# jakepoz/rnnt

Hardware: AMD Instinct MI355X
Metric: RNN-T joint+loss fwd+bwd lattice cells/s (B*T*U/s) (higher is better)
Workload: dtype f32(f16x2); 1 GPU; cfg2: B=32,T=1000,U=200,H=512,V=1024 fp32-class (f16x2 arithmetic) joint+loss fwd+bwd; enc_layout=contiguous (B,T,H), global_batch=32, per_gpu_batch=32, parallelism=dp1, cells_BTU1=6432000

## Files before the change

rnnt_amd/csrc/engine.hip:

```cpp
#include "../../include/rnnt_engine.h"

#include <cfloat>
#include <cmath>
#include <cstdarg>
#include <cstddef>
#include <cstdio>
#include <dlfcn.h>
#include <string>

#include "kernels.hpp"

namespace {

thread_local std::string g_err;
#if defined(RNNT_ABLATE) || defined(RNNT_STAMPS)
int g_flags = 0;
unsigned long long *g_debug = nullptr;
#else
constexpr int g_flags = 0;
constexpr unsigned long long *g_debug = nullptr;
#endif

}

// ... 55 lines not shown
    return RNNT_OK;
}

int check_reg(float fastemit_lambda, float delay_penalty)
{
    if (!(fastemit_lambda >= 0.f && fastemit_lambda <= FLT_MAX))
        return fail(RNNT_ERR_INVALID_ARG, "fastemit_lambda=%g must be finite and >= 0", (double)fastemit_lambda);
    if (!(delay_penalty >= 0.f && delay_penalty <= FLT_MAX))
        return fail(RNNT_ERR_INVALID_ARG, "delay_penalty=%g must be finite and >= 0", (double)delay_penalty);
    return RNNT_OK;
}

int check_restrict(const int32_t *restrict_frames, int restrict_left, int restrict_right)
{
    if (!restrict_frames) return fail(RNNT_ERR_INVALID_ARG, "null pointer argument (restrict_frames)");
    if (restrict_left < 0 || restrict_right < 0)
        return fail(RNNT_ERR_INVALID_ARG, "restrict_left=%d and restrict_right=%d must be >= 0", restrict_left, restrict_right);
    return RNNT_OK;
}

int dw_splits(int B, int T, int H, int V, int dtype)
{
    const long tiles = dtype == RNNT_DTYPE_F32 ? dw_tiles(H, V) : dtype == RNNT_DTYPE_F32_F16X2 ? x2_dw_tiles(H, V) : (long)((V + 255) / 256) * ((H + 255) / 256);
    long s = 256 / tiles;
    if (s < 1) s = 1;
    if (s > (long)B * T) s = (long)B * T;
    return (int)s;
}

long bf16_rows_alloc(size_t rows_pad) { return (long)((rows_pad + 96 + 127) / 128 * 128); }

void layout(int B, int T, int U1, int H, int V, int dtype, rnnt_engine_ws_layout *L)
{
    const size_t D = (size_t)T + U1 - 1;
    const size_t cells = (size_t)B * T * U1;
    const bool bf = dtype == RNNT_DTYPE_BF16, x2 = dtype == RNNT_DTYPE_F32_F16X2, x3 = dtype == RNNT_DTYPE_F32_BF16X3 || x2;
    const size_t rows_pad = (bf || x3) ? (cells + 1 + 31) / 32 * 32 : (cells + 1 + 15) / 16 * 16;
    L->rows_pad = rows_pad;
    L->D = (int)D;
    L->n_ublk = bf ? (U1 + 15) / 16 : x3 ? (U1 + 7) / 8 : (U1 + dhidden_gen_bu(T, U1) - 1) / dhidden_gen_bu(T, U1);
    L->n_ttile = (T + 3) / 4;
    L->n_split = dw_splits(B, T, H, V, dtype);
    L->g_lo = 0; L->aux = 0; L->aux_bytes = 0; L->x2_live = 0;
    size_t o = 0;
    if (bf) {
        const size_t ra = (size_t)bf16_rows_alloc(rows_pad);
        L->logits = o;   o += align_up(ra * V * 2);
        L->hidden = o;   o += align_up(ra * H * 2);
    } else if (x3) {
        const size_t ra = (size_t)bf16_rows_alloc(rows_pad);
        L->logits = o;   o += align_up(ra * V * 4);
        L->hidden = o;   o += align_up((x2 ? 2 : 3) * ra * H * 2);
        if (!x2) { L->g_lo = o; o += align_up(ra * V * 2); }
    } else {
        L->logits = o;   o += align_up((rows_pad + 16) * V * 4);
        L->hidden = o;   o += align_up((rows_pad + 16) * H * 4);
    }
    const LossWs w = carve_loss_ws((void *)o, B, T, U1);
    L->denom_s = (size_t)w.denom_s; L->lpb_s = (size_t)w.lpb_s; L->lpe_s = (size_t)w.lpe_s;
    L->alpha_s = (size_t)w.alpha_s; L->beta_s = (size_t)w.beta_s; L->coef = (size_t)w.coef; o = (size_t)w.err;
    L->wpack = o;
    if (bf) o += align_up(bf16_wpack_fwd_bytes(H, V)) + align_up(bf16_wpack_dh_bytes(H, V));
    else if (x2) o += align_up(x2_wpack_fwd_bytes(H, V)) + align_up(x2_wpack_dh_bytes(H, V));
    else if (x3) o += align_up(x3_wpack_fwd_bytes(H, V)) + align_up(x3_wpack_dh_bytes(H, V));
    else o += align_up(wpack_floats(H, V) * 4);
    L->enc_copy = o; o += align_up((size_t)B * T * H * 4);
    L->ep = 0;
    if (x2) { L->ep = o; o += align_up(x2_ep_bytes(B, T, U1, H)); }
    L->slab_enc = o; o += align_up((size_t)L->n_ublk * B * T * H * 4);
    L->slab_pred = o; o += align_up((size_t)L->n_ttile * B * U1 * H * 4);
    L->slab_w = o;   o += align_up((size_t)L->n_split * V * H * 4);
    L->slab_b = o;   o += align_up((size_t)L->n_split * V * 4);
    const size_t tab = ControlBlock::dw_table_bytes(B), lst = (bf || x3) ? 0 : align_up(dw_list_bytes(B, T, U1, 16));
    L->counters = o; o += sizeof(ControlBlock) + (tab > lst ? tab : lst) + ((bf || x2) ? align_up((size_t)L->n_split * 64) : 0);
    if (x2) { L->x2_live = o; o += align_up(x2_live_bytes(B, T, U1, (long)rows_pad)); }
    L->total = o;
    if (x3) {
        L->aux = o; L->aux_bytes = align_up((rows_pad + 16) * H * 4) + align_up(wpack_floats(H, V) * 4);
    }
}

}

typedef unsigned u32x4 __attribute__((ext_vector_type(4)));

__global__ __launch_bounds__(256) void k_fill32(unsigned *__restrict__ p, unsigned value, size_t n_words, int vec)
{
    const size_t i = (size_t)blockIdx.x * 256 + threadIdx.x;
    if (vec) {
        if (i < n_words / 4) ((u32x4 *)p)[i] = u32x4{value, value, value, value};
    } else if (i < n_words) {
        p[i] = value;
    }
}

__global__ __launch_bounds__(256) void k_copy32(unsigned *__restrict__ d, const unsigned *__restrict__ s, size_t n_words, int vec)
{
    const size_t i = (size_t)blockIdx.x * 256 + threadIdx.x;
    if (vec) {
        if (i < n_words / 4) ((u32x4 *)d)[i] = ((const u32x4 *)s)[i];
    } else if (i < n_words) {
        d[i] = s[i];
    }
}

void launch_fill32(void *p, unsigned value, size_t bytes, hipStream_t st)
{
    const size_t n = bytes / 4;
    if (!n) return;
    const int vec = ((uintptr_t)p % 16 == 0) && (n % 4 == 0);
    const size_t thr = vec ? n / 4 : n;
    hipLaunchKernelGGL(k_fill32, dim3((unsigned)((thr + 255) / 256)), dim3(256), 0, st, (unsigned *)p, value, n, vec);
}

void launch_copy_bytes(void *dst, const void *src, size_t bytes, hipStream_t st)
{
    const size_t n = bytes / 4;
    if (!n) return;
    const int vec = ((uintptr_t)dst % 16 == 0) && ((uintptr_t)src % 16 == 0) && (n % 4 == 0);
    const size_t thr = vec ? n / 4 : n;
    hipLaunchKernelGGL(k_copy32, dim3((unsigned)((thr + 255) / 256)), dim3(256), 0, st, (unsigned *)dst, (const unsigned *)src, n, vec);
}

namespace {

int launch_status(const char *what)
{
    hipError_t e = hipGetLastError();
    if (e != hipSuccess) return fail(RNNT_ERR_LAUNCH, "%s: %s", what, hipGetErrorString(e));
    return RNNT_OK;
}

void resolve_enc(const void *enc, const int64_t s[3], int B, int T, int H, float *copy_buf,
                 hipStream_t st, const float **out, long *sb, long *st_)
{
    const bool direct = s[2] == 1 && (s[1] % 4) == 0 && (s[0] % 4) == 0 && aligned16(enc);
    if (direct) {
        *out = (const float *)enc; *sb = s[0]; *st_ = s[1];
    } else {
        launch_copy_enc((const float *)enc, s[0], s[1], s[2], copy_buf, B, T, H, st);
        *out = copy_buf; *sb = (long)T * H; *st_ = H;
    }
}

enum { ST_PROD = 1, ST_FWD = 2, ST_LATTICE = 4, ST_COEF = 8, ST_DH = 16, ST_DH_RED = 32, ST_DW = 64,
       ST_DW_RED = 128, ST_ALL = 255 };
enum { ABLATE_NO_HIDDEN = 8, ABLATE_SEPARATE_G = 32, ABLATE_SEPARATE_HIDDEN = 64, ABLATE_FWD_LDS_RING = 128, ABLATE_FWD_ONE_WG = 256 };

struct LossCall {
    LossWs w;
    const int32_t *targets, *logit_lens, *target_lens; float *costs;
    int B, T, U1, stages ; float grad_scale, fastemit, delay; hipStream_t st;
    const int32_t *restrict_frames; int restrict_left, restrict_right;
};

struct FusedCall : LossCall {
    int H, V, blank, n_cu;
    const float *enc, *pred, *W, *bias; long enc_sb, enc_st;
    float *grad_enc, *grad_pred, *grad_W, *grad_bias;
    rnnt_engine_ws_layout L;
    char *ws; ControlBlock *cb; float *logits;
    bool separate_g, separate_hidden, fwd_lds_ring, fwd_one_wg_per_tile, no_hidden;
    bool x3_fp32_fwd, x3_fp32_dh;
    bool x2_no_flush;
    int ablate; unsigned long long *debug;
};
float *f32_at(const FusedCall &c, size_t offset) { return (float *)(c.ws + offset); }

JointFwdArgs fwd_args(const FusedCall &c, const float *wpack, const float *hidden, int make_hidden)
{
    JointFwdArgs f{};
    f.enc = c.enc; f.enc_sb = c.enc_sb; f.enc_st = c.enc_st; f.pred = c.pred; f.logit_lens = c.logit_lens; f.target_lens = c.target_lens;
    f.B = c.B; f.T = c.T; f.U1 = c.U1; f.H = c.H; f.V = c.V; f.blank = c.blank; f.ablate = c.ablate; f.debug = c.debug;
    f.wpack = wpack; f.hidden = hidden; f.make_hidden = make_hidden; f.bias = c.bias; f.targets = c.targets; f.logits = c.logits;
    f.denom_s = c.w.denom_s; f.lpb_s = c.w.lpb_s; f.lpe_s = c.w.lpe_s; f.D = c.L.D; f.counter = c.cb ? c.cb->fwd_tile : nullptr; f.n_cu = c.n_cu;
    return f;
}

JointBwdArgs bwd_args(const FusedCall &c)
{
    JointBwdArgs g{};
    g.enc = c.enc; g.enc_sb = c.enc_sb; g.enc_st = c.enc_st; g.pred = c.pred; g.logit_lens = c.logit_lens; g.target_lens = c.target_lens;
    g.B = c.B; g.T = c.T; g.U1 = c.U1; g.H = c.H; g.V = c.V; g.blank = c.blank; g.ablate = c.ablate; g.debug = c.debug;
    g.W = c.W; g.logits = c.logits; g.coef = c.w.coef; g.hidden = f32_at(c, c.L.hidden); g.rows_pad = (long)c.L.rows_pad;
    g.slab_enc = f32_at(c, c.L.slab_enc); g.slab_pred = f32_at(c, c.L.slab_pred);
    g.slab_w = f32_at(c, c.L.slab_w); g.slab_b = f32_at(c, c.L.slab_b);
    g.grad_enc = c.grad_enc; g.grad_pred = c.grad_pred; g.grad_W = c.grad_W; g.grad_bias = c.grad_bias;
    g.n_ublk = c.L.n_ublk; g.n_ttile = c.L.n_ttile; g.n_split = c.L.n_split;
    g.counter = c.cb->queue; g.dw_tab = c.cb->dw_tab(); g.n_cu = c.n_cu;
    g.gen_bu = dhidden_gen_bu(c.T, c.U1);
    return g;
}

template <class Args> Args split_args(const FusedCall &c, size_t wpack_fwd_bytes)
{
    Args h{};
    h.enc = c.enc; h.enc_sb = c.enc_sb; h.enc_st = c.enc_st; h.pred = c.pred; h.logit_lens = c.logit_lens; h.target_lens = c.target_lens;
    h.B = c.B; h.T = c.T; h.U1 = c.U1; h.H = c.H; h.V = c.V; h.blank = c.blank; h.ablate = c.ablate; h.debug = c.debug;
    h.W = c.W; h.bias = c.bias; h.targets = c.targets; h.coef = c.w.coef; h.hidden = (unsigned short *)(c.ws + c.L.hidden);
    h.denom_s = c.w.denom_s; h.lpb_s = c.w.lpb_s; h.lpe_s = c.w.lpe_s; h.D = c.L.D;
    h.slab_enc = f32_at(c, c.L.slab_enc); h.slab_pred = f32_at(c, c.L.slab_pred);
    h.slab_w = f32_at(c, c.L.slab_w); h.slab_b = f32_at(c, c.L.slab_b);
    h.rows_pad = (long)c.L.rows_pad; h.rows_alloc = bf16_rows_alloc(c.L.rows_pad);
    h.n_ublk = c.L.n_ublk; h.n_split = c.L.n_split; h.dw_tab = c.cb->dw_tab();
    h.wpack_fwd = c.ws + c.L.wpack; h.wpack_dh = c.ws + c.L.wpack + align_up(wpack_fwd_bytes);
    return h;
}

Bf16Args bf16_args(const FusedCall &c)
{
    Bf16Args h = split_args<Bf16Args>(c, bf16_wpack_fwd_bytes(c.H, c.V));
    h.logits = (unsigned short *)c.logits; h.dw_prog = c.cb->dw_prog(c.B);
    return h;
}

struct OperandScales { float g_scale, dw_rescale, db_rescale; double flush_log2; float flush_lin; };
OperandScales operand_scales(float grad_scale, float fastemit)
{
    OperandScales s; int e = 0;
    (void)frexpf(grad_scale * (1.0f + fastemit), &e);
    const int k = 13 - e < -100 ? -100 : (13 - e > 100 ? 100 : 13 - e);
    s.g_scale = ldexpf(1.0f, k); s.flush_log2 = (double)(-26 - k); s.flush_lin = ldexpf(1.0f, -26 - k);
    s.dw_rescale = 1.0f / (s.g_scale * 16384.0f); s.db_rescale = 1.0f / s.g_scale;
    return s;
}

X3Args x3_args(const FusedCall &c, size_t wpack_fwd_bytes, const OperandScales &s)
{
    X3Args h = split_args<X3Args>(c, wpack_fwd_bytes);
    h.g_scale = s.g_scale; h.dw_rescale = s.dw_rescale; h.db_rescale = s.db_rescale; h.scales = c.cb->x2_scales;
    h.ep_enc = f32_at(c, c.L.ep); h.ep_pred = h.ep_enc + (size_t)c.B * c.T * c.H; h.ep_flag = c.cb->ep_flag;
    h.logits = c.logits; h.g_lo = (unsigned short *)(c.ws + c.L.g_lo); h.n_ublk16 = (c.U1 + 15) / 16;
    h.plane_stride = h.rows_alloc * (long)c.H; h.counter = c.cb->fwd_tile; h.n_cu = c.n_cu;
    return h;
}

void loss_stages(const LossCall &c, const double *flush_log2 = nullptr, float flush_lin = 0.f)
{
    const LossWs &w = c.w; const int D = c.T + c.U1 - 1;
    if (c.restrict_frames) {
        if (c.stages & ST_LATTICE) {
            launch_restrict(w.lpe_s, c.restrict_frames, c.logit_lens, c.target_lens, c.B, c.T, c.U1, D, c.restrict_left, c.restrict_right,
                            c.delay, c.st);
            launch_lattice(w.lpb_s, w.lpe_s, w.alpha_s, w.beta_s, c.logit_lens, c.target_lens, c.costs, c.B, c.U1, D, w.err, c.st, true);
            if (c.delay > 0.f) launch_delay_cost(w.beta_s, c.logit_lens, c.target_lens, c.costs, c.B, c.T, c.U1, D, c.delay, c.st);
        }
        if (c.stages & ST_COEF)
            launch_coef_restrict(w.alpha_s, w.beta_s, w.denom_s, w.lpb_s, w.lpe_s, c.targets, c.logit_lens, c.target_lens, w.coef,
                                 c.B, c.T, c.U1, D, c.grad_scale, c.fastemit, flush_log2, flush_lin, c.st);
        return;
    }
    if (c.stages & ST_LATTICE) {
        if (c.delay > 0.f) launch_delay_penalty(w.lpe_s, c.logit_lens, c.target_lens, c.B, c.T, c.U1, D, c.delay, c.st);
        launch_lattice(w.lpb_s, w.lpe_s, w.alpha_s, w.beta_s, c.logit_lens, c.target_lens, c.costs, c.B, c.U1, D, w.err, c.st);
        if (c.delay > 0.f) launch_delay_cost(w.beta_s, c.logit_lens, c.target_lens, c.costs, c.B, c.T, c.U1, D, c.delay, c.st);
    }
    if (c.stages & ST_COEF) {
        if (c.fastemit > 0.f)
            launch_coef_fastemit(w.alpha_s, w.beta_s, w.denom_s, w.lpb_s, w.lpe_s, c.targets, c.logit_lens, c.target_lens, w.coef,
                                 c.B, c.T, c.U1, D, c.grad_scale, c.fastemit, c.st);
        else if (flush_log2)
            launch_coef_flush(w.alpha_s, w.beta_s, w.denom_s, w.lpb_s, w.lpe_s, c.targets, c.logit_lens, c.target_lens, w.coef,
                              c.B, c.T, c.U1, D, c.grad_scale, *flush_log2, flush_lin, c.st);
        else
            launch_coef(w.alpha_s, w.beta_s, w.denom_s, w.lpb_s, w.lpe_s, c.targets, c.logit_lens, c.target_lens, w.coef,
                        c.B, c.T, c.U1, D, c.grad_scale, c.st);
    }
}

void zero_unwritten_hidden(const FusedCall &c, float *hidden)
{
    const size_t cells = (size_t)c.B * c.T * c.U1;
    launch_fill32(hidden + cells * c.H, 0u, (c.L.rows_pad + 16 - cells) * c.H * 4, c.st);
    launch_zero_dead_hidden(hidden, c.logit_lens, c.target_lens, c.B, c.T, c.U1, c.H, c.st);
}

int tile_kernel_cols(const FusedCall &c) { return dhidden_gen_ok(c.H, c.V, c.U1) ? 512 * dhidden_gen_groups(c.H) : 0; }

float *aux_hidden(const FusedCall &c) { return f32_at(c, c.L.aux); }
typedef void (*x3_launcher)(const X3Args &, hipStream_t);

void standin_forward(const FusedCall &c, const X3Args &h, x3_launcher make_hidden)
{
    float *wpack = (float *)(c.ws + c.L.aux + align_up((c.L.rows_pad + 16) * (size_t)c.H * 4));
    if (c.stages & ST_PROD) { zero_unwritten_hidden(c, aux_hidden(c)); launch_pack_w_fwd(c.W, wpack, c.H, c.V, c.st); }
    if (c.stages & ST_FWD) {
        JointFwdArgs f = fwd_args(c, wpack, aux_hidden(c), 1);
        f.ablate = 0; f.debug = nullptr;
        launch_joint_fwd(f, c.st); make_hidden(h, c.st);
    }
}

void standin_dhidden(const FusedCall &c, const JointBwdArgs &g, const X3Args &h, x3_launcher split_g)
{
    const bool tile = g.pred_split_col > 0;
    if (!tile) launch_make_g(g, c.st);
    launch_dhidden(g, tile, c.st);
    split_g(h, c.st);
}

int route_fp32(const FusedCall &c)
{
    JointBwdArgs g = bwd_args(c);
    const bool tile = (g.pred_split_col = tile_kernel_cols(c)) > 0, fuse_g = tile && !c.separate_g;
    g.g_ready = tile && !fuse_g;
    const bool fuse_hid = !c.separate_hidden && !c.no_hidden;
    float *wpack = (float *)(c.ws + c.L.wpack);
    if (c.stages & ST_PROD) {
        if (fuse_hid) zero_unwritten_hidden(c, g.hidden);
        else launch_make_hidden(g, c.st);
        launch_pack_w_fwd(c.W, wpack, c.H, c.V, c.st);
    }
    if (c.stages & ST_FWD)
        launch_joint_fwd(fwd_args(c, wpack, c.no_hidden ? nullptr : g.hidden, fuse_hid ? 1 : 0), c.st, c.fwd_lds_ring, c.fwd_one_wg_per_tile);
    loss_stages(c);
    if ((c.stages & ST_COEF) && !fuse_g) launch_make_g(g, c.st);
    if (c.stages & ST_DH) launch_dhidden(g, tile, c.st);
    if (c.stages & ST_DH_RED) launch_dhidden_reduce(g, c.st);
    if (c.stages & ST_DW) launch_dw(g, c.st);
    if (c.stages & ST_DW_RED) launch_dw_reduce(g, c.st);
    return launch_status("rnnt_engine fused pipeline");
}

int route_bf16(const FusedCall &c)
{
    const Bf16Args h = bf16_args(c);
    JointBwdArgs g = bwd_args(c); g.gen_bu = 16; g.pred_split_col = c.H;
    if (c.stages & ST_PROD) launch_bf16_producers(h, c.st);
    if (c.stages & ST_FWD) launch_joint_fwd_bf16(h, c.st);
    loss_stages(c);
    if (c.stages & ST_DH) launch_dhidden_bf16(h, c.st);
    if (c.stages & ST_DH_RED) launch_dhidden_reduce(g, c.st);
    if (c.stages & ST_DW) launch_dw_bf16(h, c.st);
    if (c.stages & ST_DW_RED) launch_dw_reduce(g, c.st);
    return launch_status("rnnt_engine fused pipeline (bf16)");
}

int route_bf16x3(const FusedCall &c)
{
    const X3Args h = x3_args(c, x3_wpack_fwd_bytes(c.H, c.V), operand_scales(c.grad_scale, c.fastemit));
    JointBwdArgs g = bwd_args(c); g.hidden = aux_hidden(c);
    if (c.x3_fp32_dh) g.pred_split_col = tile_kernel_cols(c);
    else { g.gen_bu = 16; g.pred_split_col = c.H; }
    if (c.stages & ST_PROD) { launch_x3_zero_padding(h, 1, c.st); launch_x3_pack_w(h, c.st); }
    if (c.x3_fp32_fwd) standin_forward(c, h, launch_x3_make_hidden);
    else if (c.stages & ST_FWD) launch_joint_fwd_x3(h, c.st);
    loss_stages(c);
    if (c.stages & ST_DH) {
        launch_x3_zero_padding(h, 2, c.st);
        if (c.x3_fp32_dh) standin_dhidden(c, g, h, launch_x3_split_g);
        else launch_dhidden_x3(h, c.st);
    }
    if (c.stages & ST_DH_RED) launch_dhidden_reduce(g, c.st);
    if (c.stages & ST_DW) launch_dw_x3(h, c.st);
    if (c.stages & ST_DW_RED) launch_dw_reduce(g, c.st);
    return launch_status("rnnt_engine fused pipeline (bf16x3)");
}

int route_f16x2(const FusedCall &c)
{
    OperandScales s = operand_scales(c.grad_scale, c.fastemit);
    X3Args h = x3_args(c, x2_wpack_fwd_bytes(c.H, c.V), s);
    h.dw_prog = c.cb->dw_prog(c.B); h.dw_ksteps = x2_dw_walks_ksteps(c.H, c.V) ? 1 : 0;
    x2_live_carve(c.ws + c.L.x2_live, c.B, c.T, c.U1, (long)c.L.rows_pad, h);
    JointBwdArgs g = bwd_args(c); g.hidden = aux_hidden(c);
    if (c.x3_fp32_dh) g.pred_split_col = tile_kernel_cols(c);
    else { g.gen_bu = 16; g.pred_split_col = c.H; }
    if (!c.x3_fp32_dh) { g.tile_flag = h.tile_live; g.flag_ntt = (c.T + 7) / 8; g.flag_nub = h.n_ublk16; }
    if (c.x2_no_flush || c.x3_fp32_dh) { s.flush_log2 = -HUGE_VAL; s.flush_lin = 0.f; }
    if (c.stages & ST_PROD) { launch_x2_zero_padding(h, 1, c.st); launch_x2_pack_w(h, c.cb->x2_scales, c.st); launch_x2_make_ep(h, c.st); }
    if (c.x3_fp32_fwd) standin_forward(c, h, launch_x2_make_hidden);
    else if (c.stages & ST_FWD) launch_joint_fwd_x2(h, c.st);
    loss_stages(c, &s.flush_log2, s.flush_lin);
    if (c.stages & ST_COEF) launch_x2_live(h, c.st);
    if (c.stages & ST_DH) {
        launch_x2_zero_padding(h, 2, c.st);
        if (c.x3_fp32_dh) standin_dhidden(c, g, h, launch_x2_split_g);
        else { launch_x2_dead_rows(h, c.st); launch_dhidden_x2(h, c.st); }
    }
    if (c.stages & ST_DH_RED) launch_dhidden_reduce(g, c.st);
    if (c.stages & ST_DW) launch_dw_x2(h, c.st);
    if (c.stages & ST_DW_RED) launch_dw_reduce_x2(h, c.grad_W, c.grad_bias, c.st);
    return launch_status("rnnt_engine fused pipeline (f16x2)");
}

int run_fused(int stages, int variant, const void *enc, const int64_t enc_strides[3], const void *pred,
              const void *W, const void *bias, const int32_t *targets, const int32_t *logit_lens,
              const int32_t *target_lens, int B, int T, int U1, int H, int V, int blank,
              float clamp, float grad_scale, float fastemit, float delay, int dtype, float *costs,
              void *grad_enc, void *grad_pred, void *grad_W, void *grad_bias, void *workspace,
              size_t ws_bytes, void *stream, const int32_t *restrict_frames = nullptr, int restrict_left = 0,
              int restrict_right = 0)
{
    if (int rc = check_dims(B, T, U1, H, V, dtype, true)) return rc;
    if (!enc || !enc_strides || !pred || !W || !bias || !targets || !logit_lens || !target_lens ||
        !costs || !workspace)
        return fail(RNNT_ERR_INVALID_ARG, "null pointer argument");
    const bool backward = (stages & (ST_DH | ST_DH_RED | ST_DW | ST_DW_RED)) != 0;
    if (backward && (!grad_enc || !grad_pred || !grad_W || !grad_bias))
        return fail(RNNT_ERR_INVALID_ARG, "null gradient pointer");
    if (blank < 0 || blank >= V) return fail(RNNT_ERR_INVALID_ARG, "blank=%d outside [0,%d)", blank, V);
    if (clamp > 0.f) return fail(RNNT_ERR_UNSUPPORTED, "clamp>0 is only supported by rnnt_engine_loss_fwd_bwd");
    if (!(grad_scale > 0.f)) return fail(RNNT_ERR_INVALID_ARG, "grad_scale must be > 0");
    if (!aligned16(pred) || !aligned16(W) || !aligned16(bias) || !aligned16(grad_enc) ||
        !aligned16(grad_pred) || !aligned16(grad_W) || !aligned16(grad_bias) ||
        ((uintptr_t)workspace & 255))
        return fail(RNNT_ERR_INVALID_ARG, "pointers must be 16-byte aligned (workspace 256)");
    if (variant & RNNT_VARIANT_LAB_MASK)
        return fail(RNNT_ERR_UNSUPPORTED, "variant bits 0x%x are reserved: no kernel of librnnt_engine.so answers to them",
                    variant & RNNT_VARIANT_LAB_MASK);
    FusedCall c{};
    layout(B, T, U1, H, V, dtype, &c.L);
    if (ws_bytes < c.L.total)
        return fail(RNNT_ERR_WORKSPACE, "workspace %zu < required %zu bytes", ws_bytes, c.L.total);
    c.ablate = g_flags; c.debug = g_debug;
    const int xp = dtype == RNNT_DTYPE_F32 ? c.ablate : 0;
    c.separate_g = (variant & RNNT_VARIANT_SEPARATE_G) != 0 || (xp & ABLATE_SEPARATE_G) != 0;
    c.separate_hidden = (variant & RNNT_VARIANT_SEPARATE_HIDDEN) != 0 || (xp & ABLATE_SEPARATE_HIDDEN) != 0;
    c.fwd_lds_ring = (variant & RNNT_VARIANT_FWD_LDS_RING) != 0 || (xp & ABLATE_FWD_LDS_RING) != 0;
    c.fwd_one_wg_per_tile = (variant & RNNT_VARIANT_FWD_ONE_WG_PER_TILE) != 0 || (xp & ABLATE_FWD_ONE_WG) != 0;
    c.no_hidden = (xp & ABLATE_NO_HIDDEN) != 0;
    c.x2_no_flush = (variant & RNNT_VARIANT_X2_NO_FLUSH_SKIP) != 0 || fastemit > 0.f || delay > 0.f;
    if (dtype == RNNT_DTYPE_F32_BF16X3 || dtype == RNNT_DTYPE_F32_F16X2) {
        const bool x2 = dtype == RNNT_DTYPE_F32_F16X2;
        c.x3_fp32_dh = (variant & RNNT_VARIANT_X3_FP32_DH) != 0 || !(x2 ? x2_dhidden_ok(U1, H, V) : x3_dhidden_ok(U1, H, V));
        c.x3_fp32_fwd = (variant & RNNT_VARIANT_X3_FP32_FWD) != 0 || !(x2 ? x2_fwd_ok(U1, H, V) : x3_fwd_ok(U1, H, V)) || c.x3_fp32_dh;
        if (c.x3_fp32_fwd && ws_bytes < c.L.total + c.L.aux_bytes)
            return fail(RNNT_ERR_WORKSPACE, "workspace %zu < %zu bytes: a stage on the fp32 route's kernels (RNNT_VARIANT_X3_FP32_*, or a "
                        "shape k_joint_fwd_x3 / k_dhidden_x3 do not cover) needs total + aux_bytes of rnnt_engine_workspace_layout",
                        ws_bytes, c.L.total + c.L.aux_bytes);
    }
    c.B = B; c.T = T; c.U1 = U1; c.H = H; c.V = V; c.blank = blank; c.pred = (const float *)pred; c.W = (const float *)W;
    c.bias = (const float *)bias; c.targets = targets; c.logit_lens = logit_lens; c.target_lens = target_lens; c.costs = costs;
    c.grad_enc = (float *)grad_enc; c.grad_pred = (float *)grad_pred; c.grad_W = (float *)grad_W; c.grad_bias = (float *)grad_bias;
    c.stages = stages; c.grad_scale = grad_scale; c.fastemit = fastemit; c.delay = delay; c.n_cu = device_cus(); c.st = (hipStream_t)stream;
    c.restrict_frames = restrict_frames; c.restrict_left = restrict_left; c.restrict_right = restrict_right;
    c.ws = (char *)workspace; c.cb = (ControlBlock *)(c.ws + c.L.counters); c.logits = f32_at(c, c.L.logits);
    c.w = carve_loss_ws(c.ws + c.L.denom_s, B, T, U1); c.w.err = c.cb->lattice_err;
    resolve_enc(enc, enc_strides, B, T, H, f32_at(c, c.L.enc_copy), c.st, &c.enc, &c.enc_sb, &c.enc_st);
    if (dtype == RNNT_DTYPE_BF16) return route_bf16(c);
    if (dtype == RNNT_DTYPE_F32_BF16X3) return route_bf16x3(c);
    return dtype == RNNT_DTYPE_F32_F16X2 ? route_f16x2(c) : route_fp32(c);
}

}

extern "C" {

int rnnt_engine_version(void) { return RNNT_ENGINE_VERSION; }

#if defined(RNNT_ABLATE) || defined(RNNT_STAMPS)
int rnnt_engine_set_flags(int flags) { int o = g_flags; g_flags = flags; return o; }
void rnnt_engine_set_debug(void *buf) { g_debug = (unsigned long long *)buf; }
#else
int rnnt_engine_set_flags(int) { return 0; }
void rnnt_engine_set_debug(void *) {}
#endif

int rnnt_engine_debug_query(int what) { return fwd_occupancy(what); }

const char *rnnt_engine_last_error(void) { return g_err.c_str(); }

int rnnt_engine_allreduce(void *buf, size_t count, void *comm, void *stream)
{
    if (!buf || !comm) return fail(RNNT_ERR_INVALID_ARG, "null buffer / communicator");
    if (count == 0) return RNNT_OK;
    typedef int (*allreduce_fn)(const void *, void *, size_t, int, int, void *, hipStream_t);
    typedef const char *(*errstr_fn)(int);
    void *sym = dlsym(RTLD_DEFAULT, "ncclAllReduce");
    void *lib = nullptr;
    if (!sym) {
        lib = dlopen("librccl.so.1", RTLD_NOW | RTLD_NOLOAD);
        if (!lib) lib = dlopen("librccl.so.1", RTLD_NOW);
        if (!lib) lib = dlopen("librccl.so", RTLD_NOW);
        if (lib) sym = dlsym(lib, "ncclAllReduce");
    }
    if (!sym) return fail(RNNT_ERR_UNSUPPORTED, "RCCL (librccl.so.1: ncclAllReduce) not found in this process");
    const int ncclFloat32_ = 7, ncclSum_ = 0;
    const int rc = ((allreduce_fn)sym)(buf, buf, count, ncclFloat32_, ncclSum_, comm, (hipStream_t)stream);
    if (rc != 0) {
        void *es = lib ? dlsym(lib, "ncclGetErrorString") : dlsym(RTLD_DEFAULT, "ncclGetErrorString");
        return fail(RNNT_ERR_LAUNCH, "ncclAllReduce failed (%d): %s", rc, es ? ((errstr_fn)es)(rc) : "?");
    }
    return RNNT_OK;
}

int rnnt_engine_workspace_layout(int B, int T, int U1, int H, int V, int dtype,
                                 rnnt_engine_ws_layout *out)
{
    if (!out) return fail(RNNT_ERR_INVALID_ARG, "null layout pointer");
    if (int rc = check_dims(B, T, U1, H, V, dtype, true)) return rc;
    layout(B, T, U1, H, V, dtype, out);
    return RNNT_OK;
}

int rnnt_engine_workspace_bytes(int B, int T, int U1, int H, int V, int dtype, size_t *out)
{
    if (!out) return fail(RNNT_ERR_INVALID_ARG, "null size pointer");
    rnnt_engine_ws_layout L;
    if (int rc = rnnt_engine_workspace_layout(B, T, U1, H, V, dtype, &L)) return rc;
    *out = L.total;
    return RNNT_OK;
}

int rnnt_engine_loss_workspace_bytes(int B, int T, int U1, int V, int dtype, size_t *out)
{
    if (!out) return fail(RNNT_ERR_INVALID_ARG, "null size pointer");
    if (int rc = check_dims(B, T, U1, 4, V, dtype, false)) return rc;
    *out = carve_loss_ws(nullptr, B, T, U1).bytes;
    return RNNT_OK;
}

int rnnt_engine_joint_fwd_workspace_bytes(int B, int T, int U1, int H, int V, int dtype,
                                          size_t *out)
{
    if (!out) return fail(RNNT_ERR_INVALID_ARG, "null size pointer");
    if (int rc = check_dims(B, T, U1, H, V, dtype, true)) return rc;
    *out = align_up(wpack_floats(H, V) * 4) + align_up((size_t)B * T * H * 4);
    return RNNT_OK;
}

int rnnt_engine_joint_fwd(const void *enc, const int64_t enc_strides[3], const void *pred,
                          const void *W, const void *bias, int B, int T, int U1, int H, int V,
                          int dtype, void *logits, void *workspace, size_t ws_bytes, void *stream)
{
    if (int rc = check_dims(B, T, U1, H, V, dtype, true)) return rc;
    if (!enc || !enc_strides || !pred || !W || !bias || !logits || !workspace)
        return fail(RNNT_ERR_INVALID_ARG, "null pointer argument");
    if (!aligned16(pred) || !aligned16(W) || !aligned16(bias) || !aligned16(logits) ||
        ((uintptr_t)workspace & 255))
        return fail(RNNT_ERR_INVALID_ARG, "pointers must be 16-byte aligned (workspace 256)");
    size_t need;
    rnnt_engine_joint_fwd_workspace_bytes(B, T, U1, H, V, dtype, &need);
    if (ws_bytes < need) return fail(RNNT_ERR_WORKSPACE, "workspace %zu < required %zu bytes", ws_bytes, need);
// ... 752 lines not shown
```

rnnt_amd/csrc/joint_bwd.hip:

```cpp
#include "common.hpp"
#include "kernels.hpp"

typedef __attribute__((address_space(3))) void *lds_void_ptr;

#define DH_BT 8
#define DW_KC 16
#define DW_ZERO_SPAN 32
#define DH_BU 16

#define PW_BT 4
struct PwChunk {
    f32x4 x[2];
    f32x4 w[4];
};

template <int BU>
__global__ __launch_bounds__(512, 2) void k_dhidden(JointBwdArgs a, int cb0)
{
    constexpr int IT = 64 / BU;
    const int lane = threadIdx.x & 63;
    const int i = lane & 31, half = lane >> 5;
    const int T = a.T, U1 = a.U1, H = a.H, V = a.V;
    const int n_cb = (H + 127) / 128 - cb0, n_ub = (U1 + BU - 1) / BU, n_tt = (T + IT - 1) / IT;
    const long zero_row = (long)a.B * T * U1;
// ... 377 lines not shown
                }
            }
#pragma unroll
            for (int m = 8; m < 16; ++m) mf(2, m);
#pragma unroll
            for (int m = 0; m < 16; ++m) mf(3, m);
            PIN();
            if (!(j & 1)) {
                asm volatile("s_waitcnt lgkmcnt(0)" ::: "memory");
                __builtin_amdgcn_s_barrier();
            }
            PIN();
            a0 = an0;
            a1 = an1;
        }
    }
#undef PIN
    GSTAMP(2);

    if (RNNT_XP(a.ablate, 8192)) return;
    constexpr int TPM = 32 / BU;
    constexpr int NU = BU / 2;
    constexpr int TB = BU == 16 ? 1 : 2;
    float psum[NU][8];
#pragma unroll
    for (int k = 0; k < NU; ++k)
#pragma unroll
        for (int q = 0; q < 8; ++q) psum[k][q] = 0.f;
    const long BTH = (long)a.B * T * H, BUH = (long)a.B * U1 * H;
    const long rows_utt = (long)(T - t0) * U1 - u0;
    const long hspan = span_rows < rows_utt ? span_rows : rows_utt;
    const __amdgpu_buffer_rsrc_t hrsrc = __builtin_amdgcn_make_buffer_rsrc(
        (void *)(a.hidden + cell0 * H), 0, (int)(hspan * H * 4), 0x00020000);
    const unsigned hvoff[2] = {colok[0] ? (unsigned)(((4 * half) * H + colg[0]) * 4) : 0xfffffff0u,
                               colok[1] ? (unsigned)(((4 * half) * H + colg[1]) * 4) : 0xfffffff0u};
    auto t_of = [&](int mt, int rh, int r7) { return (2 * wm + mt) * TPM + (BU == 16 ? rh : 2 * rh + (r7 >> 2)); };
    auto us_of = [&](int r7) { return BU == 16 ? 8 * (r7 >> 2) + (r7 & 3) : (r7 & 3); };
    auto hload = [&](int k, f32x4 (&hb)[16]) {
        const int mt = k >> 1, rh = k & 1;
#pragma unroll
        for (int r7 = 0; r7 < 8; ++r7) {
            const unsigned soff = (unsigned)((t_of(mt, rh, r7) * U1 + us_of(r7)) * H) * 4u;
#pragma unroll
            for (int g = 0; g < 2; ++g)
                hb[r7 * 2 + g] = __builtin_bit_cast(f32x4, __builtin_amdgcn_raw_buffer_load_b128(hrsrc, hvoff[g], soff, 0));
        }
    };
    auto hcomp = [&](int k, const f32x4 (&hb)[16]) {
        const int mt = k >> 1, rh = k & 1;
        float esum[TB][8];
#pragma unroll
        for (int e = 0; e < TB; ++e)
#pragma unroll
            for (int q = 0; q < 8; ++q) esum[e][q] = 0.f;
#pragma unroll
        for (int r7 = 0; r7 < 8; ++r7)
#pragma unroll
            for (int g = 0; g < 2; ++g) {
                const f32x4 h4 = hb[r7 * 2 + g];
#pragma unroll
                for (int q = 0; q < 4; ++q) {
                    const float d = acc[mt][g * 4 + q][rh * 8 + r7] * (1.f - h4[q] * h4[q]);
                    esum[BU == 16 ? 0 : (r7 >> 2)][g * 4 + q] += d;
                    psum[BU == 16 ? r7 : (r7 & 3)][g * 4 + q] += d;
                }
            }
#pragma unroll
        for (int e = 0; e < TB; ++e) {
#pragma unroll
            for (int q = 0; q < 8; ++q) esum[e][q] += __shfl_xor(esum[e][q], 32, 64);
            const int t = t0 + t_of(mt, rh, 4 * e);
            if (half == 0 && t < Tb) {
#pragma unroll
                for (int g = 0; g < 2; ++g)
                    if (colok[g]) {
                        f32x4 o = {esum[e][g * 4], esum[e][g * 4 + 1], esum[e][g * 4 + 2], esum[e][g * 4 + 3]};
                        *(f32x4 *)(a.slab_enc + (long)ub * BTH + ((long)b * T + t) * H + colg[g]) = o;
                    }
            }
        }
    };
    {
        f32x4 hA[16], hB[16];
        hload(0, hA);
        hload(1, hB);
        __builtin_amdgcn_sched_barrier(0);
        hcomp(0, hA);
        __builtin_amdgcn_sched_barrier(0);
        hload(2, hA);
        __builtin_amdgcn_sched_barrier(0);
        hcomp(1, hB);
        __builtin_amdgcn_sched_barrier(0);
        hload(3, hB);
        __builtin_amdgcn_sched_barrier(0);
        hcomp(2, hA);
        hcomp(3, hB);
    }
    if (wm == 1) {
#pragma unroll
        for (int k = 0; k < NU; ++k)
#pragma unroll
            for (int q = 0; q < 8; ++q) s_red[wn][lane][k * 8 + q] = psum[k][q];
    }
    __syncthreads();
    if (wm == 0) {
#pragma unroll
        for (int k = 0; k < NU; ++k) {
            const int u = u0 + (BU == 16 ? 8 * (k >> 2) + (k & 3) : k) + 4 * half;
            if (u < U1) {
#pragma unroll
                for (int g = 0; g < 2; ++g)
                    if (colok[g]) {
                        f32x4 o;
#pragma unroll
                        for (int q = 0; q < 4; ++q)
                            o[q] = psum[k][g * 4 + q] + s_red[wn][lane][k * 8 + g * 4 + q];
                        *(f32x4 *)(a.slab_pred + (long)tt * BUH + ((long)b * U1 + u) * H + colg[g]) = o;
                    }
            }
        }
    }
    GSTAMP(3);
}

int dhidden_gen_bu(int T, int U1)
{
    const long c16 = (long)((U1 + 15) / 16 * 16) * ((T + 7) / 8 * 8);
    const long c8 = (long)((U1 + 7) / 8 * 8) * ((T + 15) / 16 * 16);
    return c8 < c16 ? 8 : 16;
}
bool dhidden_gen_ok(int H, int V, int U1)
{
    const long span_rows = (long)(16 - 1) * U1 + 16;
    const long wide = V > H ? V : H;
    return (V % 32) == 0 && (long)V * H * 4 < 0xffffffffL && span_rows * wide * 4 < 0x7fffffffL;
}
#define DG_COLS 512
int dhidden_gen_groups(int H) { return H <= DG_COLS ? 1 : H / DG_COLS; }

__device__ __forceinline__ void reduce_flagged(f32x4 &s, const f32x4 *__restrict__ p, long stride, int k0, unsigned m)
{
    const f32x4 z = {0.f, 0.f, 0.f, 0.f};
    while (m) {
        f32x4 v[8];
#pragma unroll
        for (int j = 0; j < 8; ++j) {
            v[j] = z;
            if (m) { v[j] = p[(long)(k0 + __builtin_ctz(m)) * stride]; m &= m - 1; }
        }
#pragma unroll
        for (int j = 0; j < 8; ++j) s += v[j];
    }
}
__global__ __launch_bounds__(256) void k_reduce_enc(const float *__restrict__ slab,
                                                    const int32_t *__restrict__ logit_lens,
                                                    const int32_t *__restrict__ target_lens,
                                                    float *__restrict__ out, int B, int T, int U1,
                                                    int H, int n_ublk, int bu_lo, int col_split,
                                                    const unsigned char *__restrict__ flag, int ntt, int nub_f)
{
    const long idx = (long)blockIdx.x * blockDim.x + threadIdx.x;
    const int H4 = H / 4;
    const long n = (long)B * T * H4;
    if (idx >= n) return;
    const long bt = idx / H4;
    const int t = (int)(bt % T), b = (int)(bt / T);
    f32x4 s = {0.f, 0.f, 0.f, 0.f};
    if (t < len_t(logit_lens, b, T)) {
        const int bu = bu_lo;
        int nub = len_u(target_lens, b, U1) / bu + 1;
        if (nub > n_ublk) nub = n_ublk;
        if (flag) {
            const unsigned char *f = flag + ((long)b * ntt + t / 8) * nub_f;
            for (int k0 = 0; k0 < nub; k0 += 32) {
                const int kn = nub - k0 < 32 ? nub - k0 : 32;
                unsigned m = 0;
                for (int k = 0; k < kn; ++k) m |= (f[k0 + k] ? 1u : 0u) << k;
                reduce_flagged(s, (const f32x4 *)slab + idx, n, k0, m);
            }
        } else {
            for (int k = 0; k < nub; ++k) s += ((const f32x4 *)slab)[(long)k * n + idx];
        }
    }
    ((f32x4 *)out)[idx] = s;
}

__global__ __launch_bounds__(256) void k_reduce_pred(const float *__restrict__ slab,
                                                     const int32_t *__restrict__ logit_lens,
                                                     const int32_t *__restrict__ target_lens,
                                                     float *__restrict__ out, int B, int T, int U1,
                                                     int H, int bt_lo, int bt_hi, int col_split,
                                                     const unsigned char *__restrict__ flag, int ntt_f, int nub_f)
{
    const long idx = (long)blockIdx.x * blockDim.x + threadIdx.x;
    const int H4 = H / 4;
    const long n = (long)B * U1 * H4;
    if (idx >= n) return;
    const int b = (int)(idx / ((long)U1 * H4));
    const int bt = 4 * (int)(idx % H4) < col_split ? bt_lo : bt_hi;
    const int ntt = (len_t(logit_lens, b, T) + bt - 1) / bt;
    const int u = (int)((idx / H4) % U1);
    f32x4 s = {0.f, 0.f, 0.f, 0.f};
    if (u <= len_u(target_lens, b, U1)) {
        if (flag) {
            const unsigned char *f = flag + (long)b * ntt_f * nub_f + u / 16;
            for (int k0 = 0; k0 < ntt; k0 += 32) {
                const int kn = ntt - k0 < 32 ? ntt - k0 : 32;
                unsigned m = 0;
                for (int k = 0; k < kn; ++k) m |= (f[(long)(k0 + k) * nub_f] ? 1u : 0u) << k;
                reduce_flagged(s, (const f32x4 *)slab + idx, n, k0, m);
            }
        } else {
            for (int k = 0; k < ntt; ++k) s += ((const f32x4 *)slab)[(long)k * n + idx];
        }
    }
    ((f32x4 *)out)[idx] = s;
}

void launch_dhidden(const JointBwdArgs &a, bool tile_kernel, hipStream_t st)
{
    int cb0 = 0;
    if (tile_kernel) {
        const long cells = (long)a.B * a.T * a.U1;
        launch_fill32((float *)a.logits + cells * a.V, 0u, (size_t)(a.rows_pad + 16 - cells) * a.V * 4, st);
        const int n_full = dhidden_gen_groups(a.H);
        if (a.gen_bu == 8) {
            dim3 grid((a.U1 + 7) / 8, (a.T + 15) / 16, a.B);
            if (a.g_ready) hipLaunchKernelGGL((k_dhidden_gen<8, false>), grid, dim3(256), 0, st, a, 0);
            else hipLaunchKernelGGL((k_dhidden_gen<8, true>), grid, dim3(256), 0, st, a, 0);
            for (int hp = 1; hp < n_full; ++hp) hipLaunchKernelGGL((k_dhidden_gen<8, false>), grid, dim3(256), 0, st, a, hp * DG_COLS);
        } else {
            dim3 grid((a.U1 + 15) / 16, (a.T + DG_BT - 1) / DG_BT, a.B);
            if (a.g_ready) hipLaunchKernelGGL((k_dhidden_gen<16, false>), grid, dim3(256), 0, st, a, 0);
            else hipLaunchKernelGGL((k_dhidden_gen<16, true>), grid, dim3(256), 0, st, a, 0);
            for (int hp = 1; hp < n_full; ++hp) hipLaunchKernelGGL((k_dhidden_gen<16, false>), grid, dim3(256), 0, st, a, hp * DG_COLS);
        }
        cb0 = n_full * (DG_COLS / 128);
        if (cb0 * 128 >= a.H) return;
    }
    launch_fill32(a.counter, 0u, 8 * 64, st);
    if (a.gen_bu == 8) hipLaunchKernelGGL(k_dhidden<8>, dim3(a.n_cu), dim3(512), 0, st, a, cb0);
    else hipLaunchKernelGGL(k_dhidden<16>, dim3(a.n_cu), dim3(512), 0, st, a, cb0);
}

void launch_dhidden_reduce(const JointBwdArgs &a, hipStream_t st)
{
    const long n4e = (long)a.B * a.T * (a.H / 4);
    hipLaunchKernelGGL(k_reduce_enc, dim3((unsigned)((n4e + 255) / 256)), dim3(256), 0, st,
                       a.slab_enc, a.logit_lens, a.target_lens, a.grad_enc, a.B, a.T, a.U1, a.H, a.n_ublk, a.gen_bu, a.pred_split_col,
                       a.tile_flag, a.flag_ntt, a.flag_nub);
    const long n4p = (long)a.B * a.U1 * (a.H / 4);
    hipLaunchKernelGGL(k_reduce_pred, dim3((unsigned)((n4p + 255) / 256)), dim3(256), 0, st,
                       a.slab_pred, a.logit_lens, a.target_lens, a.grad_pred, a.B, a.T, a.U1, a.H,
                       128 / a.gen_bu, 64 / a.gen_bu, a.pred_split_col, a.tile_flag, a.flag_ntt, a.flag_nub);
}

__global__ __launch_bounds__(256) void k_make_hidden(const float *__restrict__ enc, long sb,
                                                     long st_, const float *__restrict__ pred,
                                                     float *__restrict__ hid, int B, int T, int U1,
                                                     int H, long rows_pad)
{
    const int H4 = H / 4;
    const long idx = (long)blockIdx.x * blockDim.x + threadIdx.x;
    if (idx >= rows_pad * H4) return;
    const long c = idx / H4;
    const int h = (int)(idx - c * H4) * 4;
    f32x4 o = {0.f, 0.f, 0.f, 0.f};
    if (c < (long)B * T * U1) {
        const int u = (int)(c % U1);
        const long bt = c / U1;
        const int t = (int)(bt % T), b = (int)(bt / T);
        const f32x4 e = *(const f32x4 *)(enc + (long)b * sb + (long)t * st_ + h);
        const f32x4 p = *(const f32x4 *)(pred + ((long)b * U1 + u) * H + h);
#pragma unroll
        for (int q = 0; q < 4; ++q) o[q] = fast_tanh(e[q] + p[q]);
    }
    __builtin_nontemporal_store(o, (f32x4 *)(hid + c * H + h));
}

__global__ __launch_bounds__(256) void k_make_g(float *__restrict__ logits,
                                                const CellCoef *__restrict__ coef, long rows,
                                                long rows_pad, int V, int blank)
{
    const int lane = threadIdx.x & 63;
    const long row = (long)blockIdx.x * 4 + (threadIdx.x >> 6);
    if (row >= rows_pad) return;
    float *x = logits + row * V;
    CellCoef c;
    c.c1 = RNNT_NEG_INF; c.sb = 0.f; c.se = 0.f; c.y = -1;
    if (row < rows) c = coef[row];
    const bool live = c.c1 != RNNT_NEG_INF;
    for (int v = lane * 4; v < V; v += 256) {
        f32x4 o = {0.f, 0.f, 0.f, 0.f};
        if (live) {
            const f32x4 q = *(const f32x4 *)(x + v);
#pragma unroll
            for (int s = 0; s < 4; ++s) {
                float e = __builtin_amdgcn_exp2f(fmaf(q[s], RNNT_LOG2E, c.c1));
                if (v + s == blank) e -= c.sb;
                if (v + s == c.y) e -= c.se;
                o[s] = e;
            }
        }
        *(f32x4 *)(x + v) = o;
    }
}

void launch_make_hidden(const JointBwdArgs &a, hipStream_t st)
{
    const long n = a.rows_pad * (a.H / 4);
    hipLaunchKernelGGL(k_make_hidden, dim3((unsigned)((n + 255) / 256)), dim3(256), 0, st, a.enc,
                       a.enc_sb, a.enc_st, a.pred, a.hidden, a.B, a.T, a.U1, a.H, a.rows_pad);
}

void launch_make_g(const JointBwdArgs &a, hipStream_t st)
{
    hipLaunchKernelGGL(k_make_g, dim3((unsigned)((a.rows_pad + 3) / 4)), dim3(256), 0, st,
                       (float *)a.logits, a.coef, (long)a.B * a.T * a.U1, a.rows_pad, a.V, a.blank);
}

#define DW_RING 8

__global__ void k_dw_table(const int32_t *__restrict__ logit_lens, int B, int T, int U1, int gran, long *__restrict__ tab)
{
    if (threadIdx.x != 0 || blockIdx.x != 0) return;
    long prev_end = 0, cum = 0;
    for (int b = 0; b < B; ++b) {
        const long c0 = (long)b * T * U1;
        long s = c0 / gran, e = (c0 + (long)len_t(logit_lens, b, T) * U1 + gran - 1) / gran;
        if (s < prev_end) s = prev_end;
        if (e < s) e = s;
        tab[b] = s;
        tab[B + 1 + b] = cum;
        cum += e - s;
        prev_end = e;
    }
    tab[B] = prev_end;
    tab[2 * B + 1] = cum;
}

void launch_dw_table(const int32_t *logit_lens, int B, int T, int U1, int gran, long *tab, hipStream_t st)
{
    hipLaunchKernelGGL(k_dw_table, dim3(1), dim3(64), 0, st, logit_lens, B, T, U1, gran, tab);
}

__device__ __forceinline__ bool granule_live(long g, int gran, const int32_t *logit_lens,
                                             const int32_t *target_lens, int B, int T, int U1)
{
    const long cells = (long)B * T * U1;
    long c = g * gran;
    if (c >= cells) return false;
    long bt = c / U1;
    int u = (int)(c - bt * U1);
    int t = (int)(bt % T), b = (int)(bt / T);
    int left = gran;
    while (left > 0 && b < B) {
        if (t < len_t(logit_lens, b, T) && u <= len_u(target_lens, b, U1)) return true;
        left -= U1 - u;
        u = 0;
        if (++t == T) { t = 0; ++b; }
    }
    return false;
}
#define DWL_BLK 1024
__global__ __launch_bounds__(DWL_BLK) void k_dw_list_count(const int32_t *__restrict__ logit_lens,
                                                           const int32_t *__restrict__ target_lens, int B, int T,
                                                           int U1, int gran, long n_gran, int *__restrict__ blk)
{
    const long g = (long)blockIdx.x * DWL_BLK + threadIdx.x;
    const bool live = g < n_gran && granule_live(g, gran, logit_lens, target_lens, B, T, U1);
    const int cnt = __syncthreads_count(live);
    if (threadIdx.x == 0) blk[blockIdx.x] = cnt;
}
__global__ __launch_bounds__(1024) void k_dw_list_scan(int *__restrict__ blk, int nblk, long *__restrict__ head,
                                                       const long *__restrict__ tab, int B)
{
    __shared__ int s_w[16];
    __shared__ int s_carry;
    if (threadIdx.x == 0) s_carry = 0;
    __syncthreads();
    for (int base = 0; base < nblk; base += 1024) {
        const int i = base + threadIdx.x;
        const int v = i < nblk ? blk[i] : 0;
        int x = v;
#pragma unroll
        for (int d = 1; d < 64; d <<= 1) { const int y = __shfl_up(x, d, 64); if ((threadIdx.x & 63) >= d) x += y; }
        if ((threadIdx.x & 63) == 63) s_w[threadIdx.x >> 6] = x;
        __syncthreads();
        int off = s_carry;
        for (int w = 0; w < (int)(threadIdx.x >> 6); ++w) off += s_w[w];
        if (i < nblk) blk[i] = off + x - v;
        __syncthreads();
        if (threadIdx.x == 1023) s_carry = off + x;
        __syncthreads();
    }
    if (threadIdx.x == 0) { head[0] = s_carry; head[1] = s_carry < tab[2 * B + 1] ? 1 : 0; }
}
__global__ __launch_bounds__(DWL_BLK) void k_dw_list_write(const int32_t *__restrict__ logit_lens,
                                                           const int32_t *__restrict__ target_lens, int B, int T,
                                                           int U1, int gran, long n_gran, const int *__restrict__ blk,
                                                           int *__restrict__ list)
{
    __shared__ int s_w[DWL_BLK / 64];
    const long g = (long)blockIdx.x * DWL_BLK + threadIdx.x;
    const bool live = g < n_gran && granule_live(g, gran, logit_lens, target_lens, B, T, U1);
    const unsigned long long bal = __ballot(live);
    const int lane = threadIdx.x & 63, wave = threadIdx.x >> 6;
// ... 243 lines not shown
```

rnnt_amd/csrc/kernels.hpp:

```cpp
#pragma once
#include "common.hpp"
#include "../../include/rnnt_engine.h"

int engine_fail(int code, const char *fmt, ...);
void launch_fill32(void *p, unsigned value, size_t bytes, hipStream_t st);
void launch_copy_bytes(void *dst, const void *src, size_t bytes, hipStream_t st);
int device_cus();

void launch_logsoftmax_gather(const float *logits, const int32_t *targets,
                              const int32_t *logit_lens, const int32_t *target_lens,
                              float *denom_s, float *lpb_s, float *lpe_s, int B, int T, int U1,
                              int V, int D, int blank, hipStream_t st);
void launch_lattice(const float *lpb_s, const float *lpe_s, double *alpha_s, double *beta_s,
                    const int32_t *logit_lens, const int32_t *target_lens, float *costs, int B,
                    int U1, int D, unsigned *err , hipStream_t st,
                    bool restricted = false );
void launch_coef(const double *alpha_s, const double *beta_s, const float *denom_s,
                 const float *lpb_s, const float *lpe_s, const int32_t *targets,
                 const int32_t *logit_lens, const int32_t *target_lens, CellCoef *coef, int B,
                 int T, int U1, int D, float scale, hipStream_t st);
void launch_coef_flush(const double *alpha_s, const double *beta_s, const float *denom_s,
                       const float *lpb_s, const float *lpe_s, const int32_t *targets,
                       const int32_t *logit_lens, const int32_t *target_lens, CellCoef *coef, int B,
                       int T, int U1, int D, float scale, double flush_log2, float flush_lin, hipStream_t st);
void launch_coef_fastemit(const double *alpha_s, const double *beta_s, const float *denom_s,
                          const float *lpb_s, const float *lpe_s, const int32_t *targets,
                          const int32_t *logit_lens, const int32_t *target_lens, CellCoef *coef, int B,
                          int T, int U1, int D, float scale, float lambda, hipStream_t st);
void launch_delay_penalty(float *lpe_s, const int32_t *logit_lens, const int32_t *target_lens, int B,
                          int T, int U1, int D, float delay, hipStream_t st);
void launch_delay_cost(const double *beta_s, const int32_t *logit_lens, const int32_t *target_lens,
                       float *costs, int B, int T, int U1, int D, float delay, hipStream_t st);
void launch_restrict(float *lpe_s, const int32_t *frames , const int32_t *logit_lens,
                     const int32_t *target_lens, int B, int T, int U1, int D, int left, int right, float delay,
                     hipStream_t st);
void launch_coef_restrict(const double *alpha_s, const double *beta_s, const float *denom_s,
                          const float *lpb_s, const float *lpe_s, const int32_t *targets,
                          const int32_t *logit_lens, const int32_t *target_lens, CellCoef *coef, int B,
                          int T, int U1, int D, float scale, float lambda, const double *flush_log2, float flush_lin,
                          hipStream_t st);
void launch_grad_logits(const float *logits, const CellCoef *coef, float *grad, long nrows,
                        int V, int blank, float clamp, hipStream_t st);

void launch_align(const float *lpb_s, const float *lpe_s, void *bp, const int32_t *logit_lens,
                  const int32_t *target_lens, float *scores, int32_t *frames, int B, int U1, int D,
                  hipStream_t st);

struct JointFwdArgs {
    const float *enc;
    long enc_sb, enc_st;
    const float *pred;
    const float *wpack;
    const float *hidden;
    int make_hidden;
    const float *bias;
    const int32_t *targets, *logit_lens, *target_lens;
    float *logits;
    float *denom_s, *lpb_s, *lpe_s;
    int B, T, U1, H, V, D, blank;
    int ablate;
    unsigned *counter;
    int n_cu;
    unsigned long long *debug;
};
size_t wpack_floats(int H, int V);
void launch_pack_w_fwd(const float *W, float *wpack, int H, int V, hipStream_t st);
void launch_joint_fwd(const JointFwdArgs &a, hipStream_t st, bool lds_ring = false, bool one_wg_per_tile = false);
int fwd_occupancy(int with_loss);
void launch_zero_dead_hidden(float *hidden, const int32_t *logit_lens, const int32_t *target_lens, int B, int T,
                             int U1, int H, hipStream_t st);
void launch_copy_enc(const float *enc, long sb, long st_, long sh, float *dst, int B, int T, int H,
                     hipStream_t st);

struct JointBwdArgs {
    const float *enc; long enc_sb, enc_st;
    const float *pred;
    const float *W;
    const float *logits;
    float *hidden;
    long rows_pad;
    const CellCoef *coef;
    const int32_t *logit_lens, *target_lens;
    float *slab_enc;
    float *slab_pred;
    float *slab_w;
    float *slab_b;
    float *grad_enc, *grad_pred, *grad_W, *grad_bias;
    int B, T, U1, H, V, blank;
    int n_ublk, n_ttile, n_split;
    unsigned *counter;
    long *dw_tab;
    const int *dw_list;
    int n_cu;
    int ablate;
    int g_ready;
    int gen_bu;
    int pred_split_col;
    const unsigned char *tile_flag;
    int flag_ntt, flag_nub;
    unsigned long long *debug;
};
void launch_dhidden(const JointBwdArgs &a, bool tile_kernel, hipStream_t st);
void launch_dw(const JointBwdArgs &a, hipStream_t st);
int dw_tiles(int H, int V);
void launch_dw_table(const int32_t *logit_lens, int B, int T, int U1, int gran, long *tab, hipStream_t st);
size_t dw_list_bytes(int B, int T, int U1, int gran);
void launch_dhidden_reduce(const JointBwdArgs &a, hipStream_t st);
void launch_dw_reduce(const JointBwdArgs &a, hipStream_t st);
void launch_make_hidden(const JointBwdArgs &a, hipStream_t st);
void launch_make_g(const JointBwdArgs &a, hipStream_t st);
bool dhidden_gen_ok(int H, int V, int U1);
int dhidden_gen_groups(int H);
int dhidden_gen_bu(int T, int U1);

struct Bf16Args {
    const float *enc; long enc_sb, enc_st;
    const float *pred;
    const float *W;
    const float *bias;
    unsigned short *hidden;
    void *wpack_fwd, *wpack_dh;
    unsigned short *logits;
    const CellCoef *coef;
    const int32_t *targets, *logit_lens, *target_lens;
    float *denom_s, *lpb_s, *lpe_s;
    int D;
    float *slab_enc, *slab_pred, *slab_w, *slab_b;
    long rows_alloc;
    long rows_pad;
    int B, T, U1, H, V, blank;
    int n_ublk, n_split;
    int ablate;
    long *dw_tab;
    unsigned long long *debug;
    int *dw_prog;
};
size_t bf16_wpack_fwd_bytes(int H, int V);
size_t bf16_wpack_dh_bytes(int H, int V);
void launch_bf16_producers(const Bf16Args &a, hipStream_t st);
void launch_joint_fwd_bf16(const Bf16Args &a, hipStream_t st);
void launch_dhidden_bf16(const Bf16Args &a, hipStream_t st);
void launch_dw_bf16(const Bf16Args &a, hipStream_t st);

struct X3Args {
    const float *enc; long enc_sb, enc_st;
    const float *pred;
    const float *W;
    const float *bias;
    unsigned short *hidden;
    long plane_stride;
    void *wpack_fwd, *wpack_dh;
    float *logits;
    unsigned short *g_lo;
    const CellCoef *coef;
    const int32_t *targets, *logit_lens, *target_lens;
    float *denom_s, *lpb_s, *lpe_s;
    int D;
    float *slab_enc, *slab_pred, *slab_w, *slab_b;
    long rows_alloc;
    long rows_pad;
    int B, T, U1, H, V, blank;
    int n_ublk, n_split;
    int n_ublk16;
    int ablate;
    long *dw_tab;
    unsigned *counter;
    int n_cu;
    unsigned long long *debug;
    float g_scale;
    float dw_rescale, db_rescale;
    const float *scales;
    int *dw_prog;
    float *ep_enc, *ep_pred;
    unsigned *ep_flag;
    const unsigned char *tile_live;
    const unsigned *ks_bitmap;
    int *ks_list;
    const unsigned *grp_bitmap;
    int *grp_list;
    int *live_stats;
    const int *tile_list;
    int dw_ksteps;
};
size_t x2_live_bytes(int B, int T, int U1, long rows_pad);
void x2_live_carve(void *region, int B, int T, int U1, long rows_pad, X3Args &a);
void launch_x2_live(const X3Args &a, hipStream_t st);
bool x3_fwd_ok(int U1, int H, int V);
bool x3_dhidden_ok(int U1, int H, int V);
size_t x3_wpack_fwd_bytes(int H, int V);
size_t x3_wpack_dh_bytes(int H, int V);
void launch_x3_make_hidden(const X3Args &a, hipStream_t st);
void launch_x3_split_g(const X3Args &a, hipStream_t st);
void launch_x3_zero_padding(const X3Args &a, int what, hipStream_t st);
void launch_x3_pack_w(const X3Args &a, hipStream_t st);
void launch_joint_fwd_x3(const X3Args &a, hipStream_t st);
void launch_dhidden_x3(const X3Args &a, hipStream_t st);
void launch_dw_x3(const X3Args &a, hipStream_t st);
bool x2_fwd_ok(int U1, int H, int V);
bool x2_dhidden_ok(int U1, int H, int V);
size_t x2_wpack_fwd_bytes(int H, int V);
size_t x2_wpack_dh_bytes(int H, int V);
void launch_x2_make_hidden(const X3Args &a, hipStream_t st);
void launch_x2_split_g(const X3Args &a, hipStream_t st);
void launch_x2_zero_padding(const X3Args &a, int what, hipStream_t st);
void launch_x2_pack_w(const X3Args &a, float *scales, hipStream_t st);
void launch_x2_make_ep(const X3Args &a, hipStream_t st);
size_t x2_ep_bytes(int B, int T, int U1, int H);
void launch_joint_fwd_x2(const X3Args &a, hipStream_t st, bool plain_gemm = false);
void launch_x2_dead_rows(const X3Args &a, hipStream_t st);
void launch_dhidden_x2(const X3Args &a, hipStream_t st);
size_t x2_linear_ws_bytes(int M, int K, int N, bool bwd);
bool x2_linear_ok(int M, int K, int N);
void launch_linear_x2_fwd(const float *x, long ldx, const float *W, const float *bias, int M, int K, int N, float *y, void *ws, hipStream_t st);
void launch_linear_x2_bwd(const float *x, long ldx, const float *W, const float *dy, int M, int K, int N, float *dx, float *dW, float *db, void *ws,
                          hipStream_t st);
int x2_dw_tiles(int H, int V);
void launch_dw_reduce_x2(const X3Args &a, float *grad_W, float *grad_bias, hipStream_t st);
bool x2_dw_walks_ksteps(int H, int V);
void launch_dw_x2(const X3Args &a, hipStream_t st, bool zero_prog = true);

void launch_scan_logits(const float *enc, long enc_st, const float *pred, const float *W, const float *bias,
                        float *logits, int K, int H, int V, hipStream_t st);
void launch_argmax_scan(const float *logits, int K, int V, int blank, int t0, int32_t *out, hipStream_t st);

struct DecLoopArgs {
    const float *frames; long frame_stride; int T;
    rnnt_conv_predictor_params p; int S, E, O; float ln_in_eps, ln_eps;
    const float *text_W, *text_b;
    const float *W, *bias; int H, V, blank;
    int max_length, max_per_frame, scan_frames, iterations;
    int init;
    int32_t *host_flag;
    int32_t *state, *tokens;
    void *workspace;
    const void *tables = nullptr;
    const int32_t *sstate = nullptr;
    int stream_cap = 0;
};
size_t dec_loop_workspace_floats(int H, int V, int E, int O, int nframes);
void launch_dec_loop(const DecLoopArgs &a, hipStream_t st);
struct DecPersistArgs {
    unsigned long long *g2g, *zg, *sg, *cg;
    const float *Eenc; int T;
    const float *A0, *A1, *A2, *conv1_b;
    const float *wp2, *conv2_b;
    const float *Wl, *bl;
    const float *M, *dvec, *rvec, *cvec;
    const float *gamma, *beta; float eps;
    const float *W, *bias;
    int S, E, O, H, V, blank, max_length, max_per_frame, has_text, max_iters;
    int32_t *state, *tokens, *host_flag;
    const int32_t *sstate;
    int tok0, lds_toks;
};
int dec_persist_groups(int V);
const char *dec_persist_refusal(int T, int S, int E, int O, int H, int V, int has_text);
size_t dec_persist_workspace_floats(int T, int S, int E, int O, int H, int V, int has_text);
size_t dec_persist_lds_bytes(int E);
int launch_dec_persist(const DecLoopArgs &a, hipStream_t st);
size_t dec_tables_floats(int S, int E, int O, int H, int has_text);
void launch_dec_build_tables(const rnnt_conv_predictor_params &p, int S, int E, int O, float ln_in_eps, const float *text_W, const float *text_b, int H,
                             float *tables, hipStream_t st);
void dec_tables_offsets(int S, int E, int O, int H, int has_text, size_t *tab, size_t *wp2);
void launch_stream_init(int32_t *state, int blank, hipStream_t st);
size_t dec_stream_workspace_bytes(int n, int S, int E, int O, int H, int V, int has_text, int cap, int persistent);
int launch_dec_stream(const DecLoopArgs &a, int persistent, hipStream_t st);

struct BeamArgs {
    DecLoopArgs d;
    int beam;
    double *scores;
    const int32_t *utt = nullptr;
    int n_utt = 1, rows = 0;
    bool streaming = false;
    const rnnt_beam_context *ctx = nullptr;
};
size_t beam_workspace_bytes(int S, int E, int O, int H, int V, int has_text, int max_length, bool ctx = false);
size_t beam_batch_workspace_bytes(int S, int E, int O, int H, int V, int has_text, int max_length, int n_utt, bool ctx = false);
void launch_beam_decode(const BeamArgs &a, hipStream_t st);
size_t beam_stream_block_bytes(int S, int E, int O, int H, int V, int has_text, int max_length, int n_streams);
void launch_beam_stream_init(void *block, int32_t *state, double *scores, int S, int E, int O, int H, int V, int has_text, int max_length,
                             int beam, int blank, int n_streams, int first, int count, hipStream_t st);

enum { BEAM_ST_DONE = 3, BEAM_ST_NEW = 4, BEAM_ST_CUR = 6 };
struct BeamLstmStep {
    const int32_t *state;
    const int *need, *len, *tok;
    float *pvec;
    size_t stride; int n_utt, max_length;
    const int *own, *par; float *pool;
    rnnt_lstm_predictor_params p; int S, E, Hd, O, L, ln; float eps_in, eps_lstm, eps_out;
    const float *text_W, *text_b; int H;
    float *scratch;
};
size_t beam_lstm_step_floats(int n_utt, int E, int Hd, int O, int H);
void launch_beam_lstm_step(const BeamLstmStep &a, hipStream_t st);
struct BeamLstmArgs {
    BeamLstmStep s;
    const float *frames; long frame_stride; int rows; const int32_t *utt;
    const float *W, *bias; int V, blank, max_per_frame, beam, iterations, init;
    int32_t *host_flag, *state, *tokens; double *scores; void *workspace;
};
size_t beam_lstm_workspace_bytes(int n_utt, int E, int Hd, int O, int L, int H, int V, int max_length);
void launch_beam_decode_lstm(const BeamLstmArgs &a, hipStream_t st);
```

rnnt_amd/csrc/lattice.hip:

```cpp
#include "common.hpp"
#include "kernels.hpp"

typedef unsigned u32x2_t __attribute__((ext_vector_type(2)));

__global__ __launch_bounds__(256) void k_logsoftmax_gather(
    const float *__restrict__ logits, const int32_t *__restrict__ targets,
    const int32_t *__restrict__ logit_lens, const int32_t *__restrict__ target_lens,
    float *__restrict__ denom_s, float *__restrict__ lpb_s, float *__restrict__ lpe_s, int B,
    int T, int U1, int V, int D, int blank)
{
    const int lane = threadIdx.x & 63;
    const long row = (long)blockIdx.x * 4 + (threadIdx.x >> 6);
    const long nrows = (long)B * T * U1;
    if (row >= nrows) return;
    const int u = (int)(row % U1);
    const long bt = row / U1;
    const int t = (int)(bt % T);
    const int b = (int)(bt / T);
    if (t >= len_t(logit_lens, b, T) || u > len_u(target_lens, b, U1)) return;
    const float *x = logits + row * V;
    float m = RNNT_NEG_INF;
    for (int v = lane * 4; v < V; v += 256) {
        f32x4 q = *(const f32x4 *)(x + v);
        m = fmaxf(m, fmaxf(fmaxf(q[0], q[1]), fmaxf(q[2], q[3])));
// ... 341 lines not shown
    const int32_t *__restrict__ logit_lens, const int32_t *__restrict__ target_lens,
    CellCoef *__restrict__ coef, int B, int T, int U1, int D, float scale)
{
    coef_cell<false>(alpha_s, beta_s, denom_s, lpb_s, lpe_s, targets, logit_lens, target_lens, coef, B, T, U1, D,
                     scale, 0.f);
}

__global__ __launch_bounds__(256) void k_coef_restrict(
    const double *__restrict__ alpha_s, const double *__restrict__ beta_s,
    const float *__restrict__ denom_s, const float *__restrict__ lpb_s,
    const float *__restrict__ lpe_s, const int32_t *__restrict__ targets,
    const int32_t *__restrict__ logit_lens, const int32_t *__restrict__ target_lens,
    CellCoef *__restrict__ coef, int B, int T, int U1, int D, float scale)
{
    coef_cell<false, false, true>(alpha_s, beta_s, denom_s, lpb_s, lpe_s, targets, logit_lens, target_lens, coef, B, T, U1, D,
                                  scale, 0.f);
}

__global__ __launch_bounds__(256) void k_coef_restrict_flush(
    const double *__restrict__ alpha_s, const double *__restrict__ beta_s,
    const float *__restrict__ denom_s, const float *__restrict__ lpb_s,
    const float *__restrict__ lpe_s, const int32_t *__restrict__ targets,
    const int32_t *__restrict__ logit_lens, const int32_t *__restrict__ target_lens,
    CellCoef *__restrict__ coef, int B, int T, int U1, int D, float scale, double flush_log2, float flush_lin)
{
    coef_cell<false, true, true>(alpha_s, beta_s, denom_s, lpb_s, lpe_s, targets, logit_lens, target_lens, coef, B, T, U1, D,
                                 scale, 0.f, flush_log2, flush_lin);
}

__global__ __launch_bounds__(256) void k_coef_restrict_fastemit(
    const double *__restrict__ alpha_s, const double *__restrict__ beta_s,
    const float *__restrict__ denom_s, const float *__restrict__ lpb_s,
    const float *__restrict__ lpe_s, const int32_t *__restrict__ targets,
    const int32_t *__restrict__ logit_lens, const int32_t *__restrict__ target_lens,
    CellCoef *__restrict__ coef, int B, int T, int U1, int D, float scale, float lambda)
{
    coef_cell<true, false, true>(alpha_s, beta_s, denom_s, lpb_s, lpe_s, targets, logit_lens, target_lens, coef, B, T, U1, D,
                                 scale, lambda);
}

__global__ __launch_bounds__(256) void k_coef_fastemit(
    const double *__restrict__ alpha_s, const double *__restrict__ beta_s,
    const float *__restrict__ denom_s, const float *__restrict__ lpb_s,
    const float *__restrict__ lpe_s, const int32_t *__restrict__ targets,
    const int32_t *__restrict__ logit_lens, const int32_t *__restrict__ target_lens,
    CellCoef *__restrict__ coef, int B, int T, int U1, int D, float scale, float lambda)
{
    coef_cell<true>(alpha_s, beta_s, denom_s, lpb_s, lpe_s, targets, logit_lens, target_lens, coef, B, T, U1, D,
                    scale, lambda);
}

__global__ __launch_bounds__(256) void k_delay_penalty(float *__restrict__ lpe_s,
                                                       const int32_t *__restrict__ logit_lens,
                                                       const int32_t *__restrict__ target_lens,
                                                       int B, int T, int U1, int D, float delay)
{
    const long idx = (long)blockIdx.x * blockDim.x + threadIdx.x;
    const long per = (long)D * U1;
    if (idx >= per * B) return;
    const int b = (int)(idx / per);
    const long rem = idx - (long)b * per;
    const int d = (int)(rem / U1);
    const int u = (int)(rem - (long)d * U1);
    const int t = d - u;
    if (t < 0 || t >= len_t(logit_lens, b, T) || u >= len_u(target_lens, b, U1)) return;
    lpe_s[idx] -= delay * (float)t;
}

__global__ __launch_bounds__(256) void k_restrict(float *__restrict__ lpe_s, const int32_t *__restrict__ frames,
                                                  const int32_t *__restrict__ logit_lens,
                                                  const int32_t *__restrict__ target_lens, int B, int T, int U1,
                                                  int D, int left, int right, float delay)
{
    const long idx = (long)blockIdx.x * blockDim.x + threadIdx.x;
    const long per = (long)D * U1;
    if (idx >= per * B) return;
    const int b = (int)(idx / per);
    const long rem = idx - (long)b * per;
    const int d = (int)(rem / U1);
    const int u = (int)(rem - (long)d * U1);
    const int t = d - u;
    if (t < 0 || t >= len_t(logit_lens, b, T) || u >= len_u(target_lens, b, U1)) return;
    const long f = frames[(long)b * (U1 - 1) + u];
    if (t < f - left || t > f + right) lpe_s[idx] = RNNT_NEG_INF;
    else if (delay > 0.f) lpe_s[idx] -= delay * (float)t;
}

__global__ void k_delay_cost(const double *__restrict__ beta_s, const int32_t *__restrict__ logit_lens,
                             const int32_t *__restrict__ target_lens, float *__restrict__ costs, int B,
                             int T, int U1, int D, float delay)
{
    for (int b = threadIdx.x; b < B; b += blockDim.x) {
        const float c = costs[b];
        if (c != c) continue;
        const int Tb = len_t(logit_lens, b, T), Ub = len_u(target_lens, b, U1);
        costs[b] = (float)(-beta_s[(long)b * D * U1] - (double)Ub * (double)delay * 0.5 * (double)(Tb - 1));
    }
}

__global__ __launch_bounds__(256) void k_grad_logits(const float *__restrict__ logits,
                                                     const CellCoef *__restrict__ coef,
                                                     float *__restrict__ grad, long nrows, int V,
                                                     int blank, float clamp)
{
    const int lane = threadIdx.x & 63;
    const long row = (long)blockIdx.x * 4 + (threadIdx.x >> 6);
    if (row >= nrows) return;
    const CellCoef c = coef[row];
    const float *x = logits + row * V;
    float *g = grad + row * V;
    const bool live = c.c1 != RNNT_NEG_INF;
    for (int v = lane * 4; v < V; v += 256) {
        f32x4 o = {0.f, 0.f, 0.f, 0.f};
        if (live) {
            const f32x4 q = *(const f32x4 *)(x + v);
#pragma unroll
            for (int s = 0; s < 4; ++s) {
                float e = __builtin_amdgcn_exp2f(fmaf(q[s], RNNT_LOG2E, c.c1));
                if (v + s == blank) e -= c.sb;
                if (v + s == c.y) e -= c.se;
                if (clamp > 0.f) e = fminf(fmaxf(e, -clamp), clamp);
                o[s] = e;
            }
        }
        *(f32x4 *)(g + v) = o;
    }
}

void launch_logsoftmax_gather(const float *logits, const int32_t *targets,
                              const int32_t *logit_lens, const int32_t *target_lens,
                              float *denom_s, float *lpb_s, float *lpe_s, int B, int T, int U1,
                              int V, int D, int blank, hipStream_t st)
{
    const long nrows = (long)B * T * U1;
    hipLaunchKernelGGL(k_logsoftmax_gather, dim3((unsigned)((nrows + 3) / 4)), dim3(256), 0, st,
                       logits, targets, logit_lens, target_lens, denom_s, lpb_s, lpe_s, B, T, U1,
                       V, D, blank);
}

__global__ __launch_bounds__(1024) void k_lattice(
    const float *__restrict__ lpb_s, const float *__restrict__ lpe_s,
    double *__restrict__ alpha_s, double *__restrict__ beta_s,
    const int32_t *__restrict__ logit_lens, const int32_t *__restrict__ target_lens,
    float *__restrict__ costs, int U1, int D)
{
    if (blockIdx.y == 0)
        lattice_sweep<0>(lpb_s, lpe_s, alpha_s, logit_lens, target_lens, costs, U1, D);
    else
        lattice_sweep<1>(lpb_s, lpe_s, beta_s, logit_lens, target_lens, costs, U1, D);
}

void launch_lattice(const float *lpb_s, const float *lpe_s, double *alpha_s, double *beta_s,
                    const int32_t *logit_lens, const int32_t *target_lens, float *costs, int B,
                    int U1, int D, unsigned *err, hipStream_t st, bool restricted)
{
    const int NW = (U1 + 63) / 64;
    const size_t mbox = (size_t)(NW - 1) * D * 12;
    if (mbox <= 64 * 1024) {
        if (NW > 1) launch_fill32(err, 0u, 4, st);
        if (restricted)
            hipLaunchKernelGGL(k_lattice_chain_restrict, dim3(B, 2), dim3(64 * NW), (mbox + 15) / 16 * 16, st, lpb_s, lpe_s,
                               alpha_s, beta_s, logit_lens, target_lens, costs, U1, D, err);
        else
            hipLaunchKernelGGL(k_lattice_chain, dim3(B, 2), dim3(64 * NW), (mbox + 15) / 16 * 16, st, lpb_s, lpe_s, alpha_s,
                               beta_s, logit_lens, target_lens, costs, U1, D, err);
        if (NW > 1) hipLaunchKernelGGL(k_lattice_status, dim3(1), dim3(64), 0, st, err, costs, B);
        return;
    }
    const int NT = ((U1 + 63) / 64) * 64;
    const size_t lds = 2 * (size_t)(NT + 2) * sizeof(double);
    hipLaunchKernelGGL(k_lattice, dim3(B, 2), dim3(NT), lds, st, lpb_s, lpe_s, alpha_s, beta_s,
                       logit_lens, target_lens, costs, U1, D);
}

void launch_coef(const double *alpha_s, const double *beta_s, const float *denom_s,
                 const float *lpb_s, const float *lpe_s, const int32_t *targets,
                 const int32_t *logit_lens, const int32_t *target_lens, CellCoef *coef, int B,
                 int T, int U1, int D, float scale, hipStream_t st)
{
    const long n = (long)B * D * U1;
    hipLaunchKernelGGL(k_coef, dim3((unsigned)((n + 255) / 256)), dim3(256), 0, st, alpha_s,
                       beta_s, denom_s, lpb_s, lpe_s, targets, logit_lens, target_lens, coef, B,
                       T, U1, D, scale);
}

void launch_coef_flush(const double *alpha_s, const double *beta_s, const float *denom_s,
                       const float *lpb_s, const float *lpe_s, const int32_t *targets,
                       const int32_t *logit_lens, const int32_t *target_lens, CellCoef *coef, int B,
                       int T, int U1, int D, float scale, double flush_log2, float flush_lin, hipStream_t st)
{
    const long n = (long)B * D * U1;
    hipLaunchKernelGGL(k_coef_flush, dim3((unsigned)((n + 255) / 256)), dim3(256), 0, st, alpha_s,
                       beta_s, denom_s, lpb_s, lpe_s, targets, logit_lens, target_lens, coef, B,
                       T, U1, D, scale, flush_log2, flush_lin);
}

void launch_coef_fastemit(const double *alpha_s, const double *beta_s, const float *denom_s,
                          const float *lpb_s, const float *lpe_s, const int32_t *targets,
                          const int32_t *logit_lens, const int32_t *target_lens, CellCoef *coef, int B,
                          int T, int U1, int D, float scale, float lambda, hipStream_t st)
{
    const long n = (long)B * D * U1;
    hipLaunchKernelGGL(k_coef_fastemit, dim3((unsigned)((n + 255) / 256)), dim3(256), 0, st, alpha_s,
                       beta_s, denom_s, lpb_s, lpe_s, targets, logit_lens, target_lens, coef, B,
                       T, U1, D, scale, lambda);
}

void launch_coef_restrict(const double *alpha_s, const double *beta_s, const float *denom_s,
                          const float *lpb_s, const float *lpe_s, const int32_t *targets,
                          const int32_t *logit_lens, const int32_t *target_lens, CellCoef *coef, int B,
                          int T, int U1, int D, float scale, float lambda, const double *flush_log2, float flush_lin,
                          hipStream_t st)
{
    const long n = (long)B * D * U1;
    const dim3 grid((unsigned)((n + 255) / 256));
    if (lambda > 0.f)
        hipLaunchKernelGGL(k_coef_restrict_fastemit, grid, dim3(256), 0, st, alpha_s, beta_s, denom_s, lpb_s, lpe_s, targets,
                           logit_lens, target_lens, coef, B, T, U1, D, scale, lambda);
    else if (flush_log2)
        hipLaunchKernelGGL(k_coef_restrict_flush, grid, dim3(256), 0, st, alpha_s, beta_s, denom_s, lpb_s, lpe_s, targets,
                           logit_lens, target_lens, coef, B, T, U1, D, scale, *flush_log2, flush_lin);
    else
        hipLaunchKernelGGL(k_coef_restrict, grid, dim3(256), 0, st, alpha_s, beta_s, denom_s, lpb_s, lpe_s, targets,
                           logit_lens, target_lens, coef, B, T, U1, D, scale);
}

void launch_restrict(float *lpe_s, const int32_t *frames, const int32_t *logit_lens, const int32_t *target_lens, int B,
                     int T, int U1, int D, int left, int right, float delay, hipStream_t st)
{
    const long n = (long)B * D * U1;
    hipLaunchKernelGGL(k_restrict, dim3((unsigned)((n + 255) / 256)), dim3(256), 0, st, lpe_s, frames, logit_lens,
                       target_lens, B, T, U1, D, left, right, delay);
}

void launch_delay_penalty(float *lpe_s, const int32_t *logit_lens, const int32_t *target_lens, int B,
                          int T, int U1, int D, float delay, hipStream_t st)
{
    const long n = (long)B * D * U1;
    hipLaunchKernelGGL(k_delay_penalty, dim3((unsigned)((n + 255) / 256)), dim3(256), 0, st, lpe_s,
                       logit_lens, target_lens, B, T, U1, D, delay);
}

void launch_delay_cost(const double *beta_s, const int32_t *logit_lens, const int32_t *target_lens,
                       float *costs, int B, int T, int U1, int D, float delay, hipStream_t st)
{
    hipLaunchKernelGGL(k_delay_cost, dim3(1), dim3(256), 0, st, beta_s, logit_lens, target_lens, costs,
                       B, T, U1, D, delay);
}

void launch_grad_logits(const float *logits, const CellCoef *coef, float *grad, long nrows,
                        int V, int blank, float clamp, hipStream_t st)
{
    hipLaunchKernelGGL(k_grad_logits, dim3((unsigned)((nrows + 3) / 4)), dim3(256), 0, st, logits,
                       coef, grad, nrows, V, blank, clamp);
}
```

rnnt_amd/csrc/x2.hip:

```cpp
#include "kernels.hpp"

typedef __attribute__((ext_vector_type(8))) _Float16 f16x8;
typedef __attribute__((ext_vector_type(2))) _Float16 f16x2;
typedef __attribute__((ext_vector_type(4))) unsigned u32x4;
typedef __attribute__((ext_vector_type(2))) unsigned u32x2;
typedef __attribute__((ext_vector_type(4))) int i32x4;
typedef __attribute__((address_space(3))) void *lds_vptr;
typedef float f2 __attribute__((ext_vector_type(2)));

#ifdef RNNT_STAMPS
#define X2_CLOCK_STAMP(SLOT)                                                                                               \
    do {                                                                                                                   \
        if (a.debug && blockIdx.x == 0 && blockIdx.y == 0 && blockIdx.z == 0 && threadIdx.x == 0) {                        \
            unsigned long long t_, r_;                                                                                     \
            asm volatile("s_memtime %0\n\ts_memrealtime %1\n\ts_waitcnt lgkmcnt(0)" : "=s"(t_), "=s"(r_)::"memory");      \
            a.debug[SLOT] = t_; a.debug[(SLOT) + 1] = r_;                                                                  \
        }                                                                                                                  \
    } while (0)
#else
#define X2_CLOCK_STAMP(SLOT) do {} while (0)
#endif

#define X2_SH 16384.0f
#define X2_INV_SH (1.0f / 16384.0f)
#define X2_F16_MAX 65504.0f

__device__ __forceinline__ unsigned x2_pack(float lo, float hi)
{
    f16x2 v = {(_Float16)lo, (_Float16)hi};
    return __builtin_bit_cast(unsigned, v);
}
struct X2Pieces { unsigned h, m; };
__device__ __forceinline__ X2Pieces x2_split2(float a, float b)
{
    X2Pieces p;
    p.h = x2_pack(a, b);
    float ra, rb;
    asm("v_fma_mix_f32 %0, %1, -1.0, %2 op_sel_hi:[1,0,0]" : "=v"(ra) : "v"(p.h), "v"(a));
    asm("v_fma_mix_f32 %0, %1, -1.0, %2 op_sel:[1,0,0] op_sel_hi:[1,0,0]" : "=v"(rb) : "v"(p.h), "v"(b));
    p.m = x2_pack(ra, rb);
    return p;
}
__device__ __forceinline__ float x2_clamp(float x) { return __builtin_amdgcn_fmed3f(x, -X2_F16_MAX, X2_F16_MAX); }
#define X2_SPLIT4(x4, ph, pm, d)                                      \
    do {                                                              \
        const X2Pieces p0_ = x2_split2((x4)[0], (x4)[1]);             \
        const X2Pieces p1_ = x2_split2((x4)[2], (x4)[3]);             \
        (ph)[d] = p0_.h; (pm)[d] = p0_.m;                             \
        (ph)[(d) + 1] = p1_.h; (pm)[(d) + 1] = p1_.m;                 \
    } while (0)
__device__ __forceinline__ f32x16 x2_mfma(u32x4 a, u32x4 b, f32x16 c)
{
    return __builtin_amdgcn_mfma_f32_32x32x16_f16(__builtin_bit_cast(f16x8, a), __builtin_bit_cast(f16x8, b), c, 0, 0, 0);
}
__device__ __forceinline__ void x2_lds_barrier()
{
    __builtin_amdgcn_sched_barrier(0);
    asm volatile("s_waitcnt lgkmcnt(0)" ::: "memory");
    __builtin_amdgcn_s_barrier();
    __builtin_amdgcn_sched_barrier(0);
}
template <int N> struct X2Int { static constexpr int value = N; };
#define XW2_ROWS 16
#define XG2_BT 8
#define XG2_BU 16

#define X2_F32_MAX 3.4028234663852886e38f
__global__ __launch_bounds__(1024) void k_x2_wscale(const float *__restrict__ W, long n4, float *__restrict__ scales)
{
    __shared__ float s_m[16];
    float m = 0.f;
    bool bad = false;
    long i = threadIdx.x;
    for (; i + 7 * 1024 < n4; i += 8 * 1024) {
        f32x4 w[8];
#pragma unroll
        for (int k = 0; k < 8; ++k) w[k] = ((const f32x4 *)W)[i + 1024 * k];
#pragma unroll
        for (int k = 0; k < 8; ++k) {
            const float mw = fmaxf(fmaxf(fabsf(w[k][0]), fabsf(w[k][1])), fmaxf(fabsf(w[k][2]), fabsf(w[k][3])));
            bad |= (w[k][0] != w[k][0]) | (w[k][1] != w[k][1]) | (w[k][2] != w[k][2]) | (w[k][3] != w[k][3]);
            m = fmaxf(m, mw);
        }
    }
    for (; i < n4; i += 1024) {
        const f32x4 w = ((const f32x4 *)W)[i];
        bad |= (w[0] != w[0]) | (w[1] != w[1]) | (w[2] != w[2]) | (w[3] != w[3]);
        m = fmaxf(fmaxf(m, fmaxf(fabsf(w[0]), fabsf(w[1]))), fmaxf(fabsf(w[2]), fabsf(w[3])));
    }
#pragma unroll
    for (int o = 32; o > 0; o >>= 1) m = fmaxf(m, __shfl_xor(m, o, 64));
    const int any_bad = __syncthreads_or(bad ? 1 : 0);
    if ((threadIdx.x & 63) == 0) s_m[threadIdx.x >> 6] = m;
    __syncthreads();
    if (threadIdx.x == 0) {
        for (int k = 1; k < 16; ++k) m = fmaxf(m, s_m[k]);
        float s = 1.0f;
        const unsigned bits = __float_as_uint(m);
        const int e = (int)(bits >> 23) & 0xff;
        if (e > 0 && e < 255) {
            int k = 14 - (e - 126);
            k = k > 100 ? 100 : (k < -100 ? -100 : k);
            s = __uint_as_float((unsigned)(127 + k) << 23);
        }
        scales[0] = s;
        scales[1] = (any_bad || e == 255) ? __uint_as_float(0x7fc00000u) : 1.0f / s;
    }
}

__global__ __launch_bounds__(256) void k_x2_make_hidden(X3Args a)
{
    const int H8 = a.H / 8;
    const long cells = (long)a.B * a.T * a.U1;
    const long idx = (long)blockIdx.x * 256 + threadIdx.x;
    if (idx >= cells * H8) return;
    const long c = idx / H8;
    const int h = (int)(idx - c * H8) * 8;
    const int u = (int)(c % a.U1);
    const long bt = c / a.U1;
    const int t = (int)(bt % a.T), b = (int)(bt / a.T);
    const float *ep = a.enc + (long)b * a.enc_sb + (long)t * a.enc_st + h;
    const float *pp = a.pred + ((long)b * a.U1 + u) * a.H + h;
    f32x4 t0 = fast_tanh_sum4(*(const f32x4 *)ep, *(const f32x4 *)pp);
    f32x4 t1 = fast_tanh_sum4(*(const f32x4 *)(ep + 4), *(const f32x4 *)(pp + 4));
#pragma unroll
    for (int k = 0; k < 4; ++k) { t0[k] = x2_clamp(t0[k] * X2_SH); t1[k] = x2_clamp(t1[k] * X2_SH); }
    u32x4 ph, pm;
    X2_SPLIT4(t0, ph, pm, 0);
    X2_SPLIT4(t1, ph, pm, 2);
    u32x4 *o = (u32x4 *)(a.hidden + c * a.H + h);
    const long ps = a.plane_stride / 8;
    o[0] = ph; o[ps] = pm;
}

__global__ __launch_bounds__(256) void k_x2_split_g(X3Args a, long rows)
{
    const int VC = a.V / 32;
    const long idx = (long)blockIdx.x * 256 + threadIdx.x;
    if (idx >= rows * VC) return;
    const long r = idx / VC;
    const int c = (int)(idx - r * VC);
    f32x4 *p = (f32x4 *)(a.logits + r * a.V + 32 * c);
    f32x4 x[8];
#pragma unroll
    for (int i = 0; i < 8; ++i) {
        x[i] = p[i];
#pragma unroll
        for (int k = 0; k < 4; ++k) x[i][k] = x2_clamp(x[i][k] * a.g_scale);
    }
    u32x4 ph[4], pm[4];
#pragma unroll
    for (int i = 0; i < 8; ++i) X2_SPLIT4(x[i], ph[i >> 1], pm[i >> 1], 2 * (i & 1));
    u32x4 *o = (u32x4 *)p;
#pragma unroll
    for (int i = 0; i < 4; ++i) { o[i] = ph[i]; o[4 + i] = pm[i]; }
}

void launch_x2_make_hidden(const X3Args &a, hipStream_t st)
{
    const long n = (long)a.B * a.T * a.U1 * (a.H / 8);
    hipLaunchKernelGGL(k_x2_make_hidden, dim3((unsigned)((n + 255) / 256)), dim3(256), 0, st, a);
}
void launch_x2_split_g(const X3Args &a, hipStream_t st)
{
    const long rows = (long)a.B * a.T * a.U1;
    const long n = rows * (a.V / 32);
    hipLaunchKernelGGL(k_x2_split_g, dim3((unsigned)((n + 255) / 256)), dim3(256), 0, st, a, rows);
}
void launch_x2_zero_padding(const X3Args &a, int what, hipStream_t st)
{
    const long cells = (long)a.B * a.T * a.U1;
    const size_t pad = (size_t)(a.rows_alloc - cells);
    if (what & 1)
        for (int p = 0; p < 2; ++p) launch_fill32(a.hidden + p * a.plane_stride + cells * a.H, 0u, pad * a.H * 2, st);
    if (what & 2) launch_fill32(a.logits + cells * a.V, 0u, pad * a.V * 4, st);
}

#define XL2_BLK 1024
__device__ __forceinline__ bool x2_coef_live(const CellCoef &c) { return !(c.c1 == RNNT_NEG_INF && c.sb == 0.f && c.se == 0.f); }
namespace {
#define XL2_GPAD 32
struct X2LiveWs { size_t tiles, bitmap, blk, list, tlist, gbitmap, gblk, glist, total; long nks, ntile; int nblk; };
X2LiveWs x2_live_layout(int B, int T, int U1, long rows_pad)
{
    auto al = [](size_t x) { return (x + 255) & ~(size_t)255; };
    X2LiveWs L{};
    L.nks = rows_pad / XW2_ROWS;
    L.ntile = (long)B * ((T + 7) / 8) * ((U1 + 15) / 16);
    L.nblk = (int)((L.nks + XL2_BLK - 1) / XL2_BLK);
    size_t o = 256;
    L.tiles = o; o += al((size_t)L.ntile);
    L.bitmap = o; o += al((size_t)L.nblk * (XL2_BLK / 8));
    L.blk = o; o += al((size_t)L.nblk * 4);
    L.list = o; o += al((size_t)(L.nks + 8) * 4);
    L.tlist = o; o += al((size_t)L.ntile * 4);
    L.gbitmap = o; o += al((size_t)L.nblk * (XL2_BLK / 2));
    L.gblk = o; o += al((size_t)L.nblk * 16);
    L.glist = o; o += al((size_t)(4 * L.nks + XL2_GPAD) * 4);
    L.total = o;
    return L;
}
}
size_t x2_live_bytes(int B, int T, int U1, long rows_pad) { return x2_live_layout(B, T, U1, rows_pad).total; }
void x2_live_carve(void *region, int B, int T, int U1, long rows_pad, X3Args &a)
{
    const X2LiveWs L = x2_live_layout(B, T, U1, rows_pad);
    char *r = (char *)region;
    a.live_stats = (int *)r; a.tile_live = (const unsigned char *)(r + L.tiles); a.ks_bitmap = (const unsigned *)(r + L.bitmap);
    a.ks_list = (int *)(r + L.list); a.tile_list = (const int *)(r + L.tlist);
    a.grp_bitmap = (const unsigned *)(r + L.gbitmap); a.grp_list = (int *)(r + L.glist);
}
__global__ __launch_bounds__(XL2_BLK) void k_x2_live_count(const CellCoef *__restrict__ coef, long cells,
                                                           unsigned long long *__restrict__ bitmap, int *__restrict__ blk,
                                                           unsigned long long *__restrict__ gbitmap, int *__restrict__ gblk)
{
    __shared__ unsigned short s_nib[16][16];
    __shared__ unsigned short s_grp[16][16];
    const int lane = threadIdx.x & 63, wave = threadIdx.x >> 6;
    const long base = (long)blockIdx.x * XL2_BLK * XW2_ROWS;
    for (int it = 0; it < 16; ++it) {
        const long c = base + (long)it * XL2_BLK + threadIdx.x;
        const bool live = c < cells && x2_coef_live(coef[c]);
        const unsigned long long bal = __ballot(live);
        if (lane == 0)
            s_nib[it][wave] = (unsigned short)(((bal & 0xffffull) ? 1 : 0) | ((bal & 0xffff0000ull) ? 2 : 0) |
                                               ((bal & 0xffff00000000ull) ? 4 : 0) | ((bal & 0xffff000000000000ull) ? 8 : 0));
        unsigned long long x = bal | (bal >> 1);
        x = (x | (x >> 2)) & 0x1111111111111111ull;
        x = (x | (x >> 3)) & 0x0303030303030303ull;
        x = (x | (x >> 6)) & 0x000f000f000f000full;
        x = (x | (x >> 12)) & 0x000000ff000000ffull;
        x = (x | (x >> 24)) & 0xffffull;
        if (lane == 0) s_grp[it][wave] = (unsigned short)x;
    }
    __syncthreads();
    int cnt = 0;
    if (threadIdx.x < 16) {
        unsigned long long w = 0;
        for (int k = 0; k < 16; ++k) w |= (unsigned long long)s_nib[threadIdx.x][k] << (4 * k);
        bitmap[(long)blockIdx.x * 16 + threadIdx.x] = w;
        cnt = __popcll(w);
    }
    if (wave == 0) {
#pragma unroll
        for (int o = 8; o > 0; o >>= 1) cnt += __shfl_xor(cnt, o, 64);
        if (lane == 0) blk[blockIdx.x] = cnt;
        unsigned long long w = 0;
#pragma unroll
        for (int k = 0; k < 4; ++k) w |= (unsigned long long)s_grp[lane >> 2][4 * (lane & 3) + k] << (16 * k);
        gbitmap[(long)blockIdx.x * 64 + lane] = w;
        int gcnt = __popcll(w);
#pragma unroll
        for (int o = 8; o > 0; o >>= 1) gcnt += __shfl_xor(gcnt, o, 64);
        if ((lane & 15) == 0) gblk[(long)blockIdx.x * 4 + (lane >> 4)] = gcnt;
    }
}
#define XL2_TPT 64
__global__ __launch_bounds__(1024) void k_x2_live_scan(int *__restrict__ blk, int nblk, int *__restrict__ stats, int *__restrict__ list,
                                                       long cells, long nks, long ntile, const unsigned char *__restrict__ tile_live,
                                                       int *__restrict__ tile_list, int *__restrict__ gblk, int *__restrict__ glist)
{
    __shared__ int s_w[16];
    __shared__ int s_carry;
    auto scan_counts = [&](int *cnt, int n) {
        if (threadIdx.x == 0) s_carry = 0;
        __syncthreads();
        for (int base = 0; base < n; base += 1024) {
            const int i = base + threadIdx.x;
            const int v = i < n ? cnt[i] : 0;
            int x = v;
#pragma unroll
            for (int d = 1; d < 64; d <<= 1) { const int y = __shfl_up(x, d, 64); if ((threadIdx.x & 63) >= d) x += y; }
            if ((threadIdx.x & 63) == 63) s_w[threadIdx.x >> 6] = x;
            __syncthreads();
            int off = s_carry;
            for (int w = 0; w < (int)(threadIdx.x >> 6); ++w) off += s_w[w];
            if (i < n) cnt[i] = off + x - v;
            __syncthreads();
            if (threadIdx.x == 1023) s_carry = off + x;
            __syncthreads();
        }
        const int sum = s_carry;
        __syncthreads();
        return sum;
    };
    const int total = scan_counts(blk, nblk);
    const int gtotal = scan_counts(gblk, 4 * nblk);
    if (threadIdx.x == 0) s_carry = 0;
    __syncthreads();
    for (long base = 0; base < ntile; base += 1024L * XL2_TPT) {
        const long k0 = base + (long)threadIdx.x * XL2_TPT;
        unsigned long long m = 0;
        if (k0 < ntile) {
            u32x4 f[XL2_TPT / 16];
#pragma unroll
            for (int q = 0; q < XL2_TPT / 16; ++q) f[q] = ((const u32x4 *)(tile_live + k0))[q];
#pragma unroll
            for (int q = 0; q < XL2_TPT / 16; ++q)
#pragma unroll
                for (int j = 0; j < 16; ++j)
                    if ((f[q][j >> 2] >> (8 * (j & 3))) & 0xffu) m |= 1ull << (16 * q + j);
            if (ntile - k0 < XL2_TPT) m &= (1ull << (ntile - k0)) - 1ull;
        }
        const int v = __popcll(m);
        int x = v;
#pragma unroll
        for (int d = 1; d < 64; d <<= 1) { const int y = __shfl_up(x, d, 64); if ((threadIdx.x & 63) >= d) x += y; }
        if ((threadIdx.x & 63) == 63) s_w[threadIdx.x >> 6] = x;
        __syncthreads();
        int off = s_carry;
        for (int w = 0; w < (int)(threadIdx.x >> 6); ++w) off += s_w[w];
        off += x - v;
        for (; m; m &= m - 1) tile_list[off++] = (int)(k0 + __builtin_ctzll(m));
        __syncthreads();
        if (threadIdx.x == 1023) s_carry = off;
        __syncthreads();
    }
    if (threadIdx.x == 0) {
        stats[0] = total; stats[1] = (int)((cells + XW2_ROWS - 1) / XW2_ROWS); stats[2] = s_carry; stats[3] = (int)ntile;
        stats[4] = gtotal; stats[5] = (int)((cells + 3) / 4);
    }
    if (threadIdx.x < 8) list[total + threadIdx.x] = (int)nks;
    if (threadIdx.x < XL2_GPAD) glist[gtotal + threadIdx.x] = (int)(4 * nks);
}
__global__ __launch_bounds__(XL2_BLK) void k_x2_live_write(const unsigned long long *__restrict__ bitmap, int nblk, const int *__restrict__ blk,
                                                           int *__restrict__ list, const unsigned long long *__restrict__ gbitmap,
                                                           const int *__restrict__ gblk, int *__restrict__ glist)
{
    __shared__ int s_w[XL2_BLK / 64];
    int bid = blockIdx.x;
    if (bid >= nblk) { bid -= nblk; bitmap = gbitmap; blk = gblk; list = glist; }
    const long k = (long)bid * XL2_BLK + threadIdx.x;
    const int lane = threadIdx.x & 63, wave = threadIdx.x >> 6;
    const unsigned long long bal = bitmap[k >> 6];
    if (lane == 0) s_w[wave] = __popcll(bal);
    __syncthreads();
    int off = blk[bid];
    for (int w = 0; w < wave; ++w) off += s_w[w];
    if ((bal >> lane) & 1ull) list[off + __popcll(bal & ((1ull << lane) - 1ull))] = (int)k;
}
__global__ __launch_bounds__(256) void k_x2_live_tiles(const CellCoef *__restrict__ coef, int T, int U1, int ntt, int nub, long ntile,
                                                       unsigned char *__restrict__ tile_live)
{
    const int lane = threadIdx.x & 63;
    const long tile = (long)blockIdx.x * 4 + (threadIdx.x >> 6);
    if (tile >= ntile) return;
    const int ub = (int)(tile % nub), tt = (int)((tile / nub) % ntt);
    const long b = tile / ((long)nub * ntt);
    bool live = false;
#pragma unroll
    for (int it = 0; it < 2; ++it) {
        const int r = it * 64 + lane;
        const int t = tt * XG2_BT + (r >> 4), u = ub * XG2_BU + (r & 15);
        if (t < T && u < U1) live = live || x2_coef_live(coef[(b * T + t) * U1 + u]);
    }
    const bool any = __any(live ? 1 : 0) != 0;
    if (lane == 0) tile_live[tile] = any ? 1 : 0;
}
void launch_x2_live(const X3Args &a, hipStream_t st)
{
    const X2LiveWs L = x2_live_layout(a.B, a.T, a.U1, a.rows_pad);
    const long cells = (long)a.B * a.T * a.U1;
    int *blk = (int *)((char *)a.live_stats + L.blk);
    int *gblk = (int *)((char *)a.live_stats + L.gblk);
    unsigned long long *bitmap = (unsigned long long *)a.ks_bitmap, *gbitmap = (unsigned long long *)a.grp_bitmap;
    const int ntt = (a.T + XG2_BT - 1) / XG2_BT, nub = (a.U1 + XG2_BU - 1) / XG2_BU;
    hipLaunchKernelGGL(k_x2_live_tiles, dim3((unsigned)((L.ntile + 3) / 4)), dim3(256), 0, st, a.coef, a.T, a.U1, ntt, nub, L.ntile, (unsigned char *)a.tile_live);
    hipLaunchKernelGGL(k_x2_live_count, dim3(L.nblk), dim3(XL2_BLK), 0, st, a.coef, cells, bitmap, blk, gbitmap, gblk);
    hipLaunchKernelGGL(k_x2_live_scan, dim3(1), dim3(1024), 0, st, blk, L.nblk, a.live_stats, a.ks_list, cells, L.nks, L.ntile, a.tile_live, (int *)a.tile_list, gblk, a.grp_list);
    hipLaunchKernelGGL(k_x2_live_write, dim3(5 * L.nblk), dim3(XL2_BLK), 0, st, bitmap, L.nblk, blk, a.ks_list, gbitmap, gblk, a.grp_list);
}

__global__ __launch_bounds__(256) void k_x2_reduce_slabs(const float *__restrict__ slab, float *__restrict__ out, long n4, int ns)
{
    const long idx = (long)blockIdx.x * blockDim.x + threadIdx.x;
    if (idx >= n4) return;
    double s0 = 0.0, s1 = 0.0, s2 = 0.0, s3 = 0.0;
    for (int k = 0; k < ns; ++k) {
        const f32x4 v = ((const f32x4 *)slab)[(long)k * n4 + idx];
        s0 += (double)v[0]; s1 += (double)v[1]; s2 += (double)v[2]; s3 += (double)v[3];
    }
    ((f32x4 *)out)[idx] = f32x4{(float)s0, (float)s1, (float)s2, (float)s3};
}
void launch_dw_reduce_x2(const X3Args &a, float *grad_W, float *grad_bias, hipStream_t st)
{
    const long n4w = (long)a.V * a.H / 4, n4b = a.V / 4;
    hipLaunchKernelGGL(k_x2_reduce_slabs, dim3((unsigned)((n4w + 255) / 256)), dim3(256), 0, st, a.slab_w, grad_W, n4w, a.n_split);
    hipLaunchKernelGGL(k_x2_reduce_slabs, dim3((unsigned)((n4b + 255) / 256)), dim3(256), 0, st, a.slab_b, grad_bias, n4b, a.n_split);
}

#define XW2_NST 4
#define XW2_PLANE 4096
#define XW2_STAGE (2 * XW2_PLANE)
#define XW2_TILE (XW2_NST * XW2_STAGE)

#define XW2_LOAD_ENT4(ent, ep, WAIT) asm volatile("s_load_dwordx4 %0, %1, 0x0\n\t" WAIT "s_waitcnt lgkmcnt(0)" : "=s"(ent) : "s"(ep) : "memory")
__device__ __forceinline__ __amdgpu_buffer_rsrc_t x2_piece_rsrc(const char *base, int ent, unsigned gbytes, int imm)
{
    return __builtin_amdgcn_make_buffer_rsrc((void *)(base + (unsigned long long)(unsigned)ent * gbytes - imm), 0, (int)gbytes + imm, 0x00020000);
}
struct X2Frag { u32x2 lo[4], hi[4]; };
#define X2_LANDED(f, N)                                                                                          \
    asm volatile("s_waitcnt lgkmcnt(" #N ")"                                                                     \
                 : "+v"(f.lo[0]), "+v"(f.lo[1]), "+v"(f.lo[2]), "+v"(f.lo[3]), "+v"(f.hi[0]), "+v"(f.hi[1]),     \
                   "+v"(f.hi[2]), "+v"(f.hi[3])                                                                  \
                 :: "memory")

__device__ inline int x2_dw_xcd_remap(int id, int total)
{
    const int q8 = total / 8, r8 = total % 8, x = id % 8;
    return (x < r8 ? x * (q8 + 1) : r8 * (q8 + 1) + (x - r8) * q8) + id / 8;
}
__device__ inline int x2_dw_frag_addr(int lds0, int otile, int m, int sec, int lane)
{
    const int g = lane >> 4, q = (lane & 15) >> 2, pp = lane & 3, hh = g >> 1;
    const int row = 8 * hh + 4 * sec + q;
    const int swz = ((row & 3) << 2) | ((row >> 2) & 3);
    const int ch = 4 * m + 2 * (g & 1) + (pp >> 1);
    return lds0 + otile * XW2_TILE + 256 * row + 16 * (ch ^ swz) + 8 * (pp & 1);
}
template <int ST, int P, int NT>
__device__ inline void x2_dw_reads(X2Frag &f, const int (&base)[4][2])
{
    constexpr int off = ST * XW2_STAGE + P * XW2_PLANE;
#pragma unroll
    for (int m = 0; m < NT; ++m) {
        asm volatile("ds_read_b64_tr_b16 %0, %1 offset:%2" : "=v"(f.lo[m]) : "v"(base[m][0]), "n"(off));
        asm volatile("ds_read_b64_tr_b16 %0, %1 offset:%2" : "=v"(f.hi[m]) : "v"(base[m][1]), "n"(off));
    }
}
template <int N0, int CNT, class Piece>
__device__ inline void x2_dw_product(f32x16 (&acc)[4][4], const X2Frag &fa_, const X2Frag &fb_, bool live_n, const Piece &dma_piece)
{
    u32x4 fa[4], fb[4];
#pragma unroll
    for (int m = 0; m < 4; ++m) {
        fa[m] = u32x4{fa_.lo[m][0], fa_.lo[m][1], fa_.hi[m][0], fa_.hi[m][1]};
        fb[m] = u32x4{fb_.lo[m][0], fb_.lo[m][1], fb_.hi[m][0], fb_.hi[m][1]};
    }
#pragma unroll
    for (int qm = 0; qm < 4; ++qm) {
        if (live_n) {
#pragma unroll
            for (int qn = 0; qn < 4; ++qn) acc[qm][qn] = x2_mfma(fa[qm], fb[qn], acc[qm][qn]);
        }
        if (qm == 0 && CNT >= 1) dma_piece(X2Int<N0>{});
        if (qm == 1 && CNT >= 2) dma_piece(X2Int<N0 + (CNT >= 2 ? 1 : 0)>{});
        if (qm == 2 && CNT >= 4) dma_piece(X2Int<N0 + (CNT >= 4 ? 2 : 0)>{});
        if (qm == 3 && CNT >= 3) dma_piece(X2Int<N0 + (CNT >= 3 ? CNT - 1 : 0)>{});
        __builtin_amdgcn_sched_barrier(0);
    }
}
template <int ST, int P>
__device__ inline void x2_dw_bias_read(u32x2 &lo, u32x2 &hi, const int (&sbase)[2])
{
    constexpr int off = ST * XW2_STAGE + P * XW2_PLANE;
    asm volatile("ds_read_b64_tr_b16 %0, %1 offset:%2" : "=v"(lo) : "v"(sbase[0]), "n"(off));
    asm volatile("ds_read_b64_tr_b16 %0, %1 offset:%2" : "=v"(hi) : "v"(sbase[1]), "n"(off));
}
__device__ inline void x2_dw_bias_mfma(u32x2 &lo, u32x2 &hi, f32x16 &dacc, unsigned sv)
{
    asm volatile("s_waitcnt lgkmcnt(0)" : "+v"(lo), "+v"(hi) :: "memory");
    const u32x4 fa = {lo[0], lo[1], hi[0], hi[1]};
    const u32x4 sel = {sv, sv, sv, sv};
    asm volatile("v_mfma_f32_32x32x16_f16 %0, %1, %2, %0" : "+v"(dacc) : "v"(fa), "v"(sel));
}
struct X2DwBias { bool do_b, two_b; unsigned sel0, sel1; int sbase[2][2]; };
template <int ST, int C0, int C1, int C2, class Piece>
__device__ inline void x2_dw_kstep(f32x16 (&acc)[4][4], f32x16 &dacc, const int (&abase)[4][2], const int (&bbase)[4][2], const X2DwBias &b,
                                            bool live_n, const Piece &dma_piece)
{
    x2_lds_barrier();
    X2Frag Ah, Bh, Am, Bm;
    u32x2 dl[2], dh[2];
    x2_dw_reads<ST, 0, 4>(Ah, abase);
    x2_dw_reads<ST, 0, 4>(Bh, bbase);
    x2_dw_reads<ST, 1, 4>(Am, abase);
    X2_LANDED(Ah, 8);
    X2_LANDED(Bh, 8);
    x2_dw_product<0, C0>(acc, Ah, Bh, live_n, dma_piece);
    x2_dw_reads<ST, 1, 4>(Bm, bbase);
    X2_LANDED(Am, 8);
    x2_dw_product<C0, C1>(acc, Am, Bh, live_n, dma_piece);
    X2_LANDED(Bm, 0);
    if (b.do_b) { x2_dw_bias_read<ST, 0>(dl[0], dh[0], b.sbase[0]); x2_dw_bias_read<ST, 1>(dl[1], dh[1], b.sbase[0]); }
    x2_dw_product<C0 + C1, C2>(acc, Ah, Bm, live_n, dma_piece);
    if (b.do_b) {
        x2_dw_bias_mfma(dl[0], dh[0], dacc, b.sel0); x2_dw_bias_mfma(dl[1], dh[1], dacc, b.sel0);
        if (b.two_b) {
            x2_dw_bias_read<ST, 0>(dl[0], dh[0], b.sbase[1]); x2_dw_bias_read<ST, 1>(dl[1], dh[1], b.sbase[1]);
            x2_dw_bias_mfma(dl[0], dh[0], dacc, b.sel1); x2_dw_bias_mfma(dl[1], dh[1], dacc, b.sel1);
        }
    }
}
struct X2DwLockstep {
    int *prog;
    const int *nb;
    int nb_at;
    bool sync_on;
};
__device__ inline X2DwLockstep x2_dw_lockstep_init(int *dw_prog, int split, int tile, int tiles)
{
    X2DwLockstep s;
    s.prog = dw_prog ? dw_prog + split * 16 : nullptr;
    s.sync_on = s.prog != nullptr && tiles > 1 && tiles <= 16;
    s.nb = s.prog ? s.prog + (tile + 1 < tiles ? tile + 1 : 0) : nullptr;
    s.nb_at = 0x7fffffff;
    return s;
}
__device__ inline void x2_dw_lockstep(X2DwLockstep &s, int mine, int tile, int tid)
{
    constexpr int DW_LAG = 6, DW_NAPS = 256;
    asm volatile("s_waitcnt lgkmcnt(0)" : "+s"(s.nb_at) :: "memory");
    int naps = 0;
    while (s.sync_on && s.nb_at + DW_LAG + XW2_NST < mine) {
        if (++naps > DW_NAPS) { s.sync_on = false; break; }
        __builtin_amdgcn_s_sleep(4);
        asm volatile("s_load_dword %0, %1, 0x0 glc\n\ts_waitcnt lgkmcnt(0)" : "=s"(s.nb_at) : "s"(s.nb) : "memory");
    }
    if (s.sync_on) {
        if (tid == 0) __hip_atomic_store(s.prog + tile, mine, __ATOMIC_RELAXED, __HIP_MEMORY_SCOPE_AGENT);
        asm volatile("s_load_dword %0, %1, 0x0 glc" : "=s"(s.nb_at) : "s"(s.nb) : "memory");
    }
}
template <class KStep, class DmaStage>
__device__ inline void x2_dw_ring(int nks, X2DwLockstep &ls, int tile, int tid, const KStep &kstep, const DmaStage &dma_stage)
{
    static_assert(XW2_NST == 4, "prologue and unrolling below");
    int runs = 1;
    asm volatile("" : "+s"(runs));
    for (int run = 0; run < runs; ++run) {
        dma_stage(0, 0);
        dma_stage(1, 1);
        dma_stage(2, 2);
        for (int ks = 0;;) {
            if (ks >= nks) break;
            x2_dw_lockstep(ls, ks, tile, tid);
            kstep(X2Int<0>{}, ks); ++ks;
            if (ks >= nks) break;
            kstep(X2Int<1>{}, ks); ++ks;
            if (ks >= nks) break;
// ... 170 lines not shown
    const int g_lo = __builtin_amdgcn_readfirstlane((int)(nlive * split / a.n_split));
    const int g_hi = __builtin_amdgcn_readfirstlane((int)(nlive * (split + 1) / a.n_split));

    auto body = [&](auto tall_c) {
        constexpr bool TALL = decltype(tall_c)::value != 0;
        const int vb = TALL ? 0 : tile / n_fh, hb = TALL ? n_fh : tile % n_fh, vt = TALL ? tile - n_full : 0;
        const int wm = TALL ? wave : wave >> 1, wn = TALL ? 0 : wave & 1;
        const int v0 = TALL ? vt * 512 + wave * 128 : vb * 256 + wm * 128;
        const int h0 = TALL ? n_fh * 256 : hb * 256 + wn * 128;

        f32x16 acc[4][4];
#pragma unroll
        for (int qm = 0; qm < 4; ++qm)
#pragma unroll
            for (int qn = 0; qn < 4; ++qn)
#pragma unroll
                for (int r = 0; r < 16; ++r) acc[qm][qn][r] = 0.f;
        X2DwBias bias;
        bias.do_b = !TALL && hb < 2;
        bias.two_b = false;
        const int bsel0 = (hb & 1) * 2 + wn;
        f32x16 dacc;
#pragma unroll
        for (int r = 0; r < 16; ++r) dacc[r] = 0.f;
        bias.sel0 = (lane & 31) == 0 ? 0x3c003c00u : 0u; bias.sel1 = 0u;

        if (g_hi > g_lo) {
            const bool is_g = TALL || wave < 2;
            const int col0 = TALL ? v0 : (is_g ? vb : hb) * 256 + 128 * (wave & 1);
            const char *pbase[2];
            long rstride;
            if (is_g) {
                pbase[0] = (const char *)a.logits + 4L * col0;
                pbase[1] = (const char *)a.logits + 4L * col0 + 64;
                rstride = 4L * V;
            } else {
#pragma unroll
                for (int p = 0; p < 2; ++p) pbase[p] = (const char *)(a.hidden + p * a.plane_stride) + 2L * col0;
                rstride = 2L * H;
            }
            int soff[4];
#pragma unroll
            for (int i = 0; i < 4; ++i) {
                const int jg = (lane & 15) ^ (((lane >> 4) << 2) | (i & 3));
                const int cb = is_g ? 128 * (jg >> 2) + 16 * (jg & 3) : 16 * jg;
                soff[i] = (int)((4 * i + (lane >> 4)) * rstride) + cb - 1024 * i;
            }
            const int xp = wave >> 1, xi0 = 2 * (wave & 1);
            const char *xbase = (const char *)(a.hidden + xp * a.plane_stride) + 2L * h0;
            const long xstride = 2L * H;
            int xoff[2];
#pragma unroll
            for (int k = 0; k < 2; ++k) {
                const int i = xi0 + k;
                const int jg = (lane & 15) ^ (((lane >> 4) << 2) | (i & 3));
                xoff[k] = (int)((4 * i + (lane >> 4)) * xstride) + 16 * jg;
            }
            const int *lptr = a.ks_list + g_lo;
            const int lds0 = (int)(size_t)(lds_vptr)s_ring;
            const int own_tile = wave;
            int abase[4][2], bbase[4][2];
#pragma unroll
            for (int m = 0; m < 4; ++m)
#pragma unroll
                for (int sec = 0; sec < 2; ++sec) {
                    abase[m][sec] = x2_dw_frag_addr(lds0, wm, m, sec, lane);
                    bbase[m][sec] = x2_dw_frag_addr(lds0, TALL ? 4 : 2 + wn, m, sec, lane);
                    bias.sbase[1][sec] = bias.sbase[0][sec] = x2_dw_frag_addr(lds0, wm, bsel0 & 3, sec, lane);
                }

            auto kstep = [&](auto st_c, long ks) {
                constexpr int ST = decltype(st_c)::value, DST = (ST + XW2_NST - 1) % XW2_NST;
                int ent;
                const int *ep = lptr + ks + (XW2_NST - 1);
                if (TALL) asm volatile("s_load_dword %0, %1, 0x0\n\t" RNNT_VMCNT(20) "\n\ts_waitcnt lgkmcnt(0)" : "=s"(ent) : "s"(ep) : "memory");
                else asm volatile("s_load_dword %0, %1, 0x0\n\t" RNNT_VMCNT(16) "\n\ts_waitcnt lgkmcnt(0)" : "=s"(ent) : "s"(ep) : "memory");
                __amdgpu_buffer_rsrc_t rs[2];
#pragma unroll
                for (int p = 0; p < 2; ++p)
                    rs[p] = __builtin_amdgcn_make_buffer_rsrc((void *)(pbase[p] + ((long)ent * XW2_ROWS) * rstride), 0,
                                                              (int)(XW2_ROWS * rstride), 0x00020000);
                const __amdgpu_buffer_rsrc_t xrs = __builtin_amdgcn_make_buffer_rsrc(
                    (void *)(xbase + ((long)ent * XW2_ROWS) * xstride), 0, (int)(XW2_ROWS * xstride), 0x00020000);
                auto dma_piece = [&](auto n_c) {
                    constexpr int n = decltype(n_c)::value;
                    if constexpr (n < 8) {
                        constexpr int i = n & 3, p = (n >> 2) & 1;
                        __builtin_amdgcn_raw_ptr_buffer_load_lds(rs[p], (lds_vptr)(s_ring + own_tile * XW2_TILE + DST * XW2_STAGE + p * XW2_PLANE),
                                                                 16, soff[i], 0, 1024 * i, 0);
                    } else {
                        constexpr int k = n - 8;
                        __builtin_amdgcn_raw_ptr_buffer_load_lds(xrs, (lds_vptr)(s_ring + 4 * XW2_TILE + DST * XW2_STAGE + xp * XW2_PLANE + 1024 * (xi0 + k)),
                                                                 16, xoff[k], 0, 0, 0);
                    }
                };
                x2_dw_kstep<ST, (TALL ? 4 : 3), 3, (TALL ? 3 : 2)>(acc, dacc, abase, bbase, bias, true, dma_piece);
            };
            auto dma_stage = [&](long ks, int st) {
                int ent;
                const int *ep = lptr + ks;
                asm volatile("s_load_dword %0, %1, 0x0\n\ts_waitcnt lgkmcnt(0)" : "=s"(ent) : "s"(ep) : "memory");
#pragma unroll
                for (int n = 0; n < 8; ++n) {
                    const int p = n >> 2, i = n & 3;
                    const __amdgpu_buffer_rsrc_t r = __builtin_amdgcn_make_buffer_rsrc(
                        (void *)(pbase[p] + ((long)ent * XW2_ROWS) * rstride), 0, (int)(XW2_ROWS * rstride), 0x00020000);
                    lds_vptr d = (lds_vptr)(s_ring + own_tile * XW2_TILE + st * XW2_STAGE + p * XW2_PLANE);
                    if (i == 0) __builtin_amdgcn_raw_ptr_buffer_load_lds(r, d, 16, soff[i], 0, 0, 0);
                    if (i == 1) __builtin_amdgcn_raw_ptr_buffer_load_lds(r, d, 16, soff[i], 0, 1024, 0);
                    if (i == 2) __builtin_amdgcn_raw_ptr_buffer_load_lds(r, d, 16, soff[i], 0, 2048, 0);
                    if (i == 3) __builtin_amdgcn_raw_ptr_buffer_load_lds(r, d, 16, soff[i], 0, 3072, 0);
                }
                if (TALL) {
                    const __amdgpu_buffer_rsrc_t r = __builtin_amdgcn_make_buffer_rsrc(
                        (void *)(xbase + ((long)ent * XW2_ROWS) * xstride), 0, (int)(XW2_ROWS * xstride), 0x00020000);
#pragma unroll
                    for (int k = 0; k < 2; ++k)
                        __builtin_amdgcn_raw_ptr_buffer_load_lds(r, (lds_vptr)(s_ring + 4 * XW2_TILE + st * XW2_STAGE + xp * XW2_PLANE + 1024 * (xi0 + k)),
                                                                 16, xoff[k], 0, 0, 0);
                }
            };
            X2DwLockstep ls = x2_dw_lockstep_init(a.dw_prog, split, tile, tiles);
            x2_dw_ring(g_hi - g_lo, ls, tile, tid, kstep, dma_stage);
        }
        x2_dw_store<false>(a, split, v0, h0, lane, acc, dacc, bias.do_b, false, bsel0);
    };
    if (tile >= n_full) body(X2Int<1>{});
    else body(X2Int<0>{});
}

bool x2_dw_walks_ksteps(int H, int V) { return x2_dw_mixed_ok(H, V) != 0; }

void launch_dw_x2(const X3Args &a, hipStream_t st, bool zero_prog)
{
    if (a.dw_prog && zero_prog) launch_fill32(a.dw_prog, 0u, (size_t)a.n_split * 64, st);
    const int tiles = x2_dw_tiles(a.H, a.V);
    static bool attr_set[16] = {false};
    int dev = -1;
    if (hipGetDevice(&dev) != hipSuccess || dev < 0 || dev >= 16) dev = -1;
    if (dev < 0 || !attr_set[dev]) {
        (void)hipFuncSetAttribute((const void *)k_dw_x2<4>, hipFuncAttributeMaxDynamicSharedMemorySize, 4 * XW2_TILE);
        (void)hipFuncSetAttribute((const void *)k_dw_x2<4, true>, hipFuncAttributeMaxDynamicSharedMemorySize, 4 * XW2_TILE);
        (void)hipFuncSetAttribute((const void *)k_dw_x2m, hipFuncAttributeMaxDynamicSharedMemorySize, 5 * XW2_TILE);
        if (dev >= 0) attr_set[dev] = true;
    }
    if (x2_dw_mixed_ok(a.H, a.V)) hipLaunchKernelGGL(k_dw_x2m, dim3(tiles * a.n_split), dim3(256), 5 * XW2_TILE, st, a);
    else if (a.H % 256 != 0) hipLaunchKernelGGL((k_dw_x2<4, true>), dim3(((a.V + 255) / 256) * ((a.H + 255) / 256) * a.n_split), dim3(256), 4 * XW2_TILE, st, a);
    else hipLaunchKernelGGL(k_dw_x2<4>, dim3(tiles * a.n_split), dim3(256), 4 * XW2_TILE, st, a);
}

#define XG2_WAIT8(b) asm volatile("s_waitcnt lgkmcnt(0)" : "+v"(b[0]), "+v"(b[1]), "+v"(b[2]), "+v"(b[3]), "+v"(b[4]), "+v"(b[5]), "+v"(b[6]), "+v"(b[7]) :: "memory")
#define XG2_WAIT8_BUT(b, N) asm volatile("s_waitcnt lgkmcnt(" #N ")" : "+v"(b[0]), "+v"(b[1]), "+v"(b[2]), "+v"(b[3]), "+v"(b[4]), "+v"(b[5]), "+v"(b[6]), "+v"(b[7]) :: "memory")

__global__ __launch_bounds__(256) void k_x2_pack_w_dh(const float *__restrict__ W, const float *__restrict__ scales, u32x4 *__restrict__ out, int H, int V, long n)
{
    const long idx = (long)blockIdx.x * 256 + threadIdx.x;
    if (idx >= n) return;
    const int lane = (int)(idx & 63), tile = (int)(idx >> 6) & 15;
    const int VC = V / 16;
    const int c = (int)((idx >> 10) % VC), hp = (int)((idx >> 10) / VC);
    const int h = 512 * hp + 128 * (tile >> 2) + 4 * (lane & 31) + (tile & 3);
    const int v0 = 16 * c + 8 * (lane >> 5);
    const float sw = scales[0];
    u32x4 ph = {0u, 0u, 0u, 0u}, pm = ph;
    if (h < H) {
        const float *w = W + (long)v0 * H + h;
#pragma unroll
        for (int j = 0; j < 4; ++j) {
            const X2Pieces q = x2_split2(x2_clamp(w[(long)(2 * j) * H] * sw), x2_clamp(w[(long)(2 * j + 1) * H] * sw));
            ph[j] = q.h; pm[j] = q.m;
        }
    }
    u32x4 *o = out + ((long)hp * VC + c) * 2048 + tile * 64 + lane;
    o[0] = ph; o[1024] = pm;
}
size_t x2_wpack_dh_bytes(int H, int V) { return (size_t)((H + 511) / 512) * (V / 16) * 2 * 16 * 64 * 16; }

#define XG2_WSLOT 32768
#define XG2_XSLOT 8192
#define XG2_NW 3
template <bool FIRST, bool PART>
__global__ __launch_bounds__(256, 1) void k_dhidden_x2(X3Args a, const int hp)
{
    extern __shared__ __attribute__((aligned(1024))) char s_dh[];
    const int tid = threadIdx.x, lane = tid & 63;
    const int wave = __builtin_amdgcn_readfirstlane(tid >> 6);
    const int wm = wave >> 1, wn = wave & 1;
    const int i = lane & 31, half = lane >> 5;
    const int T = a.T, U1 = a.U1, H = a.H, V = a.V;
    if ((int)blockIdx.x >= a.live_stats[2]) return;
    const int tile = __builtin_amdgcn_readfirstlane(a.tile_list[blockIdx.x]);
    const int nub = a.n_ublk16, ntt = (T + XG2_BT - 1) / XG2_BT;
    const int ub = __builtin_amdgcn_readfirstlane(tile % nub), tt = __builtin_amdgcn_readfirstlane((tile / nub) % ntt);
    const int b = __builtin_amdgcn_readfirstlane(tile / (nub * ntt));
    int Tb, Ub;
    len_tu_uniform(a.logit_lens, a.target_lens, b, a.T, a.U1, Tb, Ub);
    const int t0 = tt * XG2_BT, u0 = ub * XG2_BU;
    const int VC = V / 16;
    const int ngrp = PART ? (H - 512 * hp) / 128 : 4;
    if (FIRST) X2_CLOCK_STAMP(128 + 108);

    const int prow = wave * 32 + i;
    const int pt = t0 + (prow >> 4), pu = u0 + (prow & 15);
    const bool pexists = pt < T && pu < U1;
    const long zrow = (long)a.B * T * U1;
    const long pcell = pexists ? ((long)b * T + pt) * U1 + pu : zrow;


    CellCoef cf = a.coef[pexists ? pcell : 0];
    const bool live = pexists && pt < Tb && cf.c1 != RNNT_NEG_INF;
    if (!live) { cf.c1 = RNNT_NEG_INF; cf.sb = 0.f; cf.se = 0.f; cf.y = -1; }
    const float gs = a.g_scale;
    const float *xsrc = a.logits + ((FIRST ? live : pexists) ? pcell : zrow) * V;
    const int blank = a.blank;
    const int lds0 = (int)(size_t)(lds_vptr)s_dh;
    const int lpiece = lane & 7, lrow = lane >> 3;
    const int xl = lds0 + XG2_NW * XG2_WSLOT + ((lpiece >> 1) & 1) * XG2_XSLOT + wave * 2048 + (lpiece >> 2) * 1024 + 16 * (lrow + 32 * (lpiece & 1));
    const long tile_cell0 = ((long)b * T + t0) * U1 + u0;
    const __amdgpu_buffer_rsrc_t grs = __builtin_amdgcn_make_buffer_rsrc(
        (void *)(a.logits + tile_cell0 * V), 0, (int)((((long)(XG2_BT - 1) * U1 + XG2_BU) * V) * 4), 0x00020000);
    int lvo[4];
#pragma unroll
    for (int n = 0; n < 4; ++n) {
        const int lt = 2 * wave + (n >> 1), lu = 8 * (n & 1) + lrow;
        const bool ex = t0 + lt < T && u0 + lu < U1;
        lvo[n] = ex ? (int)(((long)lt * U1 + lu) * V * 4) + 64 * (lpiece >> 2) + 16 * (lpiece & 3) : 0x7ffffff0;
    }

    f32x16 acc[2][8];
#pragma unroll
    for (int mt = 0; mt < 2; ++mt)
#pragma unroll
        for (int q = 0; q < 8; ++q)
#pragma unroll
            for (int r = 0; r < 16; ++r) acc[mt][q][r] = 0.f;

    const int xw = lds0 + XG2_NW * XG2_WSLOT + wave * 2048 + 16 * lane;
    const int xa = lds0 + XG2_NW * XG2_WSLOT + (2 * wm) * 2048 + 16 * lane;
    const int wb = lds0 + (8 * wn) * 1024 + 16 * lane;
    const __amdgpu_buffer_rsrc_t wrs = __builtin_amdgcn_make_buffer_rsrc((char *)a.wpack_dh + (long)hp * VC * XG2_WSLOT, 0, VC * XG2_WSLOT, 0x00020000);
    const int wvo = lane * 16;

    struct Raw { f32x4 x0, x1; };
    auto xload = [&](Raw &r, int c, int part = 3) {
        const int cc = c < VC ? c : VC - 1;
        if (FIRST) {
            const f32x4 *p = (const f32x4 *)xsrc + 4 * cc + 2 * half;
            if (part & 1) r.x0 = p[0];
            if (part & 2) r.x1 = p[1];
        } else {
            const u32x4 *p = (const u32x4 *)xsrc + 8 * (cc >> 1) + 2 * (cc & 1) + half;
            if (part & 1) r.x0 = __builtin_bit_cast(f32x4, p[0]);
            if (part & 2) r.x1 = __builtin_bit_cast(f32x4, p[4]);
        }
    };
    struct Prod { f32x4 g0, g1; u32x4 ph, pm; };
    auto produce_slice = [&](Prod &P, const Raw &r, int c, int sl) {
        if (!FIRST) {
            if (sl == 0) { P.ph = __builtin_bit_cast(u32x4, r.x0); P.pm = __builtin_bit_cast(u32x4, r.x1); }
        } else if (sl < 4) {
            P.g0[sl] = __builtin_amdgcn_exp2f(fmaf(r.x0[sl], RNNT_LOG2E, cf.c1));
            P.g1[sl] = __builtin_amdgcn_exp2f(fmaf(r.x1[sl], RNNT_LOG2E, cf.c1));
        } else if (sl == 4) {
            const int vb = 16 * c + 8 * half;
            const unsigned dy = (unsigned)(cf.y - vb);
            if (__any(dy < 8u)) {
#pragma unroll
                for (int e = 0; e < 4; ++e) {
                    P.g0[e] = (dy == (unsigned)e) ? P.g0[e] - cf.se : P.g0[e];
                    P.g1[e] = (dy == (unsigned)(e + 4)) ? P.g1[e] - cf.se : P.g1[e];
                }
            }
        } else if (sl == 5) {
            const int vb = 16 * c + 8 * half;
            if ((unsigned)(blank - 16 * c) < 16u) {
#pragma unroll
                for (int e = 0; e < 4; ++e) {
                    P.g0[e] = (vb + e == blank) ? P.g0[e] - cf.sb : P.g0[e];
                    P.g1[e] = (vb + e + 4 == blank) ? P.g1[e] - cf.sb : P.g1[e];
                }
            }
        } else if (sl == 6) {
            const f32x4 s4 = P.g0 * gs;
            X2_SPLIT4(s4, P.ph, P.pm, 0);
        } else if (sl == 7) {
            const f32x4 s4 = P.g1 * gs;
            X2_SPLIT4(s4, P.ph, P.pm, 2);
        }
        if (sl == 8) {
            const int dst = xw + (c & 1) * XG2_XSLOT;
            asm volatile("ds_write_b128 %0, %1" :: "v"(dst), "v"(P.ph) : "memory");
            asm volatile("ds_write_b128 %0, %1 offset:1024" :: "v"(dst), "v"(P.pm) : "memory");
        }
    };
    auto produce = [&](const Raw &r, int c) {
        Prod P;
#pragma unroll
        for (int sl = 0; sl < 9; ++sl) produce_slice(P, r, c, sl);
    };
    auto wdma = [&](int c, int slot, int n) {
        const int cc = c < VC ? c : VC - 1;
        const int vo = (!PART || (((wave * 8 + n) & 15) >> 2) < ngrp) ? wvo : 0x7ffffff0;
        const int g4 = n & 4;
        lds_vptr dst = (lds_vptr)(s_dh + slot * XG2_WSLOT + (wave * 8 + g4) * 1024);
        const int so = (cc * 32 + wave * 8 + g4) * 1024;
        if ((n & 3) == 0) __builtin_amdgcn_raw_ptr_buffer_load_lds(wrs, dst, 16, vo, so, 0, 0);
        if ((n & 3) == 1) __builtin_amdgcn_raw_ptr_buffer_load_lds(wrs, dst, 16, vo, so, 1024, 0);
        if ((n & 3) == 2) __builtin_amdgcn_raw_ptr_buffer_load_lds(wrs, dst, 16, vo, so, 2048, 0);
        if ((n & 3) == 3) __builtin_amdgcn_raw_ptr_buffer_load_lds(wrs, dst, 16, vo, so, 3072, 0);
    };

    Raw xr[4];
    xload(xr[0], 0); xload(xr[1], 1); xload(xr[2], 2); xload(xr[3], 3);
#pragma unroll
    for (int n = 0; n < 8; ++n) wdma(0, 0, n);
#pragma unroll
// ... 214 lines not shown
        lds_vptr dst = (lds_vptr)(s_dr + slot * XR2_WSLOT + (wp * 4 + wt2) * 1024);
        const int so = ((cc * 2 + wp) * 16 + wt2) * 1024;
        __builtin_amdgcn_raw_ptr_buffer_load_lds(wrs, dst, 16, wvo, so, 0, 0);
        __builtin_amdgcn_raw_ptr_buffer_load_lds(wrs, dst, 16, wvo, so, 1024, 0);
    };
    const int lds0 = (int)(size_t)(lds_vptr)s_dr;
    const int wb = lds0 + 16 * lane;

    f32x16 acc[4][4];
#pragma unroll
    for (int m = 0; m < 4; ++m)
#pragma unroll
        for (int n = 0; n < 4; ++n)
#pragma unroll
            for (int r = 0; r < 16; ++r) acc[m][n][r] = 0.f;

    AFrag ar[4];
    aload(ar[0], 0); aload(ar[1], 1); aload(ar[2], 2);
    wdma(0, 0); wdma(1, 1);
    int wsl = 0;
    for (int c0 = 0; c0 < VC; c0 += 4) {
#pragma unroll
        for (int j = 0; j < 4; ++j) {
            const int c = c0 + j;
            asm volatile(RNNT_VMCNT(10) ::: "memory");
            x2_lds_barrier();
            const int ws = wb + wsl * XR2_WSLOT;
            u32x4 bh[4], bm[4];
#pragma unroll
            for (int n = 0; n < 4; ++n) asm volatile("ds_read_b128 %0, %1 offset:%2" : "=v"(bh[n]) : "v"(ws), "n"(n * 1024));
            asm volatile("s_waitcnt lgkmcnt(0)" : "+v"(bh[0]), "+v"(bh[1]), "+v"(bh[2]), "+v"(bh[3]) :: "memory");
            AFrag &ac = ar[j], &an = ar[(j + 3) & 3];
            const int cn = c + 3;
            const int o = 8 * ((cn < VC ? cn : VC - 1) >> 1) + 2 * ((cn < VC ? cn : VC - 1) & 1);
#pragma unroll
            for (int m = 0; m < 4; ++m) {
#pragma unroll
                for (int n = 0; n < 4; ++n) {
                    acc[m][n] = x2_mfma(ac.h[m], bh[n], acc[m][n]);
                    if (m == 0) asm volatile("ds_read_b128 %0, %1 offset:%2" : "=v"(bm[n]) : "v"(ws), "n"(4096 + n * 1024));
                    if (n == 1) an.h[m] = arow[m][o];
                    if (n == 3) an.m[m] = arow[m][o + 4];
                    __builtin_amdgcn_sched_barrier(0);
                }
            }
#pragma unroll
            for (int m = 0; m < 4; ++m)
#pragma unroll
                for (int n = 0; n < 4; ++n) {
                    acc[m][n] = x2_mfma(ac.m[m], bh[n], acc[m][n]);
                    __builtin_amdgcn_sched_barrier(0);
                }
            asm volatile("s_waitcnt lgkmcnt(0)" : "+v"(bm[0]), "+v"(bm[1]), "+v"(bm[2]), "+v"(bm[3]) :: "memory");
#pragma unroll
            for (int m = 0; m < 4; ++m)
#pragma unroll
                for (int n = 0; n < 4; ++n) {
                    acc[m][n] = x2_mfma(ac.h[m], bm[n], acc[m][n]);
                    if (m == 3 && n == 0) wdma(c + 2, (wsl + 2) & 3);
                    __builtin_amdgcn_sched_barrier(0);
                }
            wsl = (wsl + 1) & 3;
        }
    }
    asm volatile("s_waitcnt vmcnt(0)" ::: "memory");
    if (!wlive) return;

    const int colg = 512 * hp + 4 * i;
    const bool colok = colg < H;
    f32x4 pr[8];
#pragma unroll
    for (int r7 = 0; r7 < 8; ++r7) {
        const int u = u0 + 8 * (r7 >> 2) + (r7 & 3) + 4 * half;
        pr[r7] = (u < U1 && colok) ? *(const f32x4 *)(a.pred + ((long)b * U1 + u) * H + colg) : f32x4{0.f, 0.f, 0.f, 0.f};
    }
    const float unscale = 4.0f * a.db_rescale * a.scales[1];
    const long BTH = (long)a.B * T * H, BUH = (long)a.B * U1 * H;
    auto dfac_q = [](f2 x) {
        const f2 av = x * (2.0f * RNNT_LOG2E);
        const f2 w = {__builtin_amdgcn_exp2f(-__builtin_fabsf(av[0])), __builtin_amdgcn_exp2f(-__builtin_fabsf(av[1]))};
        const f2 e1 = w + 1.0f;
        const f2 r = {__builtin_amdgcn_rcpf(e1[0]), __builtin_amdgcn_rcpf(e1[1])};
        return (w * r) * r;
    };
    f2 psum2[8][2];
#pragma unroll
    for (int k = 0; k < 8; ++k) { psum2[k][0] = f2{0.f, 0.f}; psum2[k][1] = f2{0.f, 0.f}; }
#pragma unroll
    for (int m = 0; m < 4; ++m)
#pragma unroll
        for (int rh = 0; rh < 2; ++rh) {
            const int t = t0 + 2 * m + rh;
            const f32x4 er = (t < T && colok) ? *(const f32x4 *)(a.enc + (long)b * a.enc_sb + (long)t * a.enc_st + colg) : f32x4{0.f, 0.f, 0.f, 0.f};
            f2 esum2[2] = {f2{0.f, 0.f}, f2{0.f, 0.f}};
#pragma unroll
            for (int r7 = 0; r7 < 8; ++r7)
#pragma unroll
                for (int qq = 0; qq < 2; ++qq) {
                    const f2 x = {er[2 * qq] + pr[r7][2 * qq], er[2 * qq + 1] + pr[r7][2 * qq + 1]};
                    const f2 av = {acc[m][2 * qq][rh * 8 + r7], acc[m][2 * qq + 1][rh * 8 + r7]};
                    const f2 d = av * dfac_q(x);
                    esum2[qq] += d;
                    psum2[r7][qq] += d;
                }
            f32x4 es = {unscale * esum2[0][0], unscale * esum2[0][1], unscale * esum2[1][0], unscale * esum2[1][1]};
#pragma unroll
            for (int q = 0; q < 4; ++q) es[q] += __shfl_xor(es[q], 32, 64);
            if (half == 0 && t < Tb && colok) *(f32x4 *)(a.slab_enc + (long)ub * BTH + ((long)b * T + t) * H + colg) = es;
        }
#pragma unroll
    for (int k = 0; k < 8; ++k) {
        const int u = u0 + 8 * (k >> 2) + (k & 3) + 4 * half;
        if (u < U1 && colok) {
            const f32x4 o = {unscale * psum2[k][0][0], unscale * psum2[k][0][1], unscale * psum2[k][1][0], unscale * psum2[k][1][1]};
            *(f32x4 *)(a.slab_pred + (long)tt * BUH + ((long)b * U1 + u) * H + colg) = o;
        }
    }
}

#define XZ2_WG_WAVES 4
__global__ __launch_bounds__(64 * XZ2_WG_WAVES) void k_x2_dead_rows(X3Args a, int ntt, int nub)
{
    const int lane = threadIdx.x & 63;
    const long wave = (long)blockIdx.x * XZ2_WG_WAVES + (threadIdx.x >> 6), nwave = (long)gridDim.x * XZ2_WG_WAVES;
    const long cells = (long)a.B * a.T * a.U1;
    const bool by_ks = a.dw_ksteps;
    const int sh = by_ks ? 4 : 2, per = 64 >> sh;
    const int *list = by_ks ? a.ks_list : a.grp_list;
    const long n = a.live_stats[by_ks ? 0 : 4];
    const int V4 = a.V / 4;
    const u32x4 z = {0u, 0u, 0u, 0u};
    for (long k = per * wave; k < n; k += per * nwave) {
        const long kk = k + (lane >> sh);
        int e = 0;
        bool dead = false;
        if (kk < n) {
            e = list[kk];
            const long c = ((long)e << sh) + (lane & ((1 << sh) - 1));
            if (c < cells) {
                const int u = (int)(c % a.U1);
                const long bt = c / a.U1;
                const int t = (int)(bt % a.T);
                const long b = bt / a.T;
                dead = a.tile_live[(b * ntt + t / XG2_BT) * nub + u / XG2_BU] == 0;
            }
        }
        unsigned long long m = __ballot(dead);
        for (; m; m &= m - 1) {
            const int r = __builtin_ctzll(m);
            u32x4 *row = (u32x4 *)(a.logits + (((long)__shfl(e, r, 64) << sh) + (r & ((1 << sh) - 1))) * a.V);
            for (int q = lane; q < V4; q += 64) row[q] = z;
        }
    }
}
void launch_x2_dead_rows(const X3Args &a, hipStream_t st)
{
    const long rounds = ((long)a.B * a.T * a.U1 + 63) / 64;
    const long want = (rounds + XZ2_WG_WAVES - 1) / XZ2_WG_WAVES, cap = (long)(a.n_cu > 0 ? a.n_cu : 256) * 8;
    const int ntt = (a.T + XG2_BT - 1) / XG2_BT;
    hipLaunchKernelGGL(k_x2_dead_rows, dim3((unsigned)(want < cap ? want : cap)), dim3(64 * XZ2_WG_WAVES), 0, st, a, ntt, a.n_ublk16);
}

bool x2_dhidden_ok(int U1, int H, int V)
{
    return (long)((XG2_BT - 1) * (long)U1 + XG2_BU) * V * 4 < 0x7fffffffL && V % 128 == 0 && H % 128 == 0;
}

void launch_dhidden_x2(const X3Args &a, hipStream_t st)
{
    static bool attr_set[16] = {false};
    int dev = -1;
    if (hipGetDevice(&dev) != hipSuccess || dev < 0 || dev >= 16) dev = -1;
    const int lds = XG2_NW * XG2_WSLOT + 2 * XG2_XSLOT;
    if (dev < 0 || !attr_set[dev]) {
        (void)hipFuncSetAttribute((const void *)k_dhidden_x2<true, false>, hipFuncAttributeMaxDynamicSharedMemorySize, lds);
        (void)hipFuncSetAttribute((const void *)k_dhidden_x2<false, false>, hipFuncAttributeMaxDynamicSharedMemorySize, lds);
        (void)hipFuncSetAttribute((const void *)k_dhidden_x2<true, true>, hipFuncAttributeMaxDynamicSharedMemorySize, lds);
        (void)hipFuncSetAttribute((const void *)k_dhidden_x2<false, true>, hipFuncAttributeMaxDynamicSharedMemorySize, lds);
        if (dev >= 0) attr_set[dev] = true;
    }
    dim3 grid((unsigned)((long)a.n_ublk16 * ((a.T + XG2_BT - 1) / XG2_BT) * a.B));
    if (a.H < 512) hipLaunchKernelGGL((k_dhidden_x2<true, true>), grid, dim3(256), lds, st, a, 0);
    else hipLaunchKernelGGL((k_dhidden_x2<true, false>), grid, dim3(256), lds, st, a, 0);
    for (int hp = 1; hp * 512 < a.H; ++hp) {
        if (a.H - 512 * hp == 128) {
            dim3 gr(a.n_ublk16, ((a.T + XG2_BT - 1) / XG2_BT + 3) / 4, a.B);
            hipLaunchKernelGGL(k_dhidden_x2r, gr, dim3(256), XR2_NW * XR2_WSLOT, st, a, hp);
        }
        else if (a.H - 512 * hp < 512) hipLaunchKernelGGL((k_dhidden_x2<false, true>), grid, dim3(256), lds, st, a, hp);
        else hipLaunchKernelGGL((k_dhidden_x2<false, false>), grid, dim3(256), lds, st, a, hp);
    }
}

__global__ __launch_bounds__(256) void k_x2_make_ep(X3Args a)
{
    const int H = a.H, H4 = H / 4, KC = H / 16;
    const long n_enc = (long)a.B * a.T * H4, n_all = n_enc + (long)a.B * a.U1 * H4;
    const long idx = (long)blockIdx.x * 256 + threadIdx.x;
    bool big = false;
    if (idx < n_all) {
        const bool is_enc = idx < n_enc;
        const long j = is_enc ? idx : idx - n_enc;
        const long row = j / H4;
        const int h = (int)(j - row * H4) * 4;
        const int R = is_enc ? a.T : a.U1;
        const int b = (int)(row / R), r = (int)(row - (long)b * R);
        const float *src = is_enc ? a.enc + (long)b * a.enc_sb + (long)r * a.enc_st + h : a.pred + row * H + h;
        const f32x4 x = *(const f32x4 *)src;
        f32x4 y;
#pragma unroll
        for (int k = 0; k < 4; ++k) {
            big = big || !(fabsf(x[k]) <= 43.0f);
            double arg = (double)x[k] * 2.8853900817779268;
            arg = arg > 126.0 ? 126.0 : (arg < -126.0 ? -126.0 : arg);
            y[k] = (float)exp2(arg);
        }
        float *dst = (is_enc ? a.ep_enc : a.ep_pred) + (((long)b * KC + (h >> 4)) * R + r) * 16 + (h & 15);
        *(f32x4 *)dst = y;
    }
    if (__builtin_amdgcn_ballot_w64(big) != 0 && (threadIdx.x & 63) == 0) atomicOr(a.ep_flag, 1u);
}
void launch_x2_make_ep(const X3Args &a, hipStream_t st)
{
    launch_fill32(a.ep_flag, 0u, 4, st);
    const long n = ((long)a.B * a.T + (long)a.B * a.U1) * (a.H / 4);
    hipLaunchKernelGGL(k_x2_make_ep, dim3((unsigned)((n + 255) / 256)), dim3(256), 0, st, a);
}
size_t x2_ep_bytes(int B, int T, int U1, int H) { return ((size_t)B * T + (size_t)B * U1) * H * 4; }

__global__ __launch_bounds__(256) void k_x2_pack_w_fwd(const float *__restrict__ W, const float *__restrict__ scales, u32x4 *__restrict__ out, int H, int V, long n)
{
    const long idx = (long)blockIdx.x * 256 + threadIdx.x;
    if (idx >= n) return;
    const int lane = (int)(idx & 63), tile = (int)(idx >> 6) & 15;
    const int KC = H / 16;
    const int c = (int)((idx >> 10) % KC), pass = (int)((idx >> 10) / KC);
    const int v = 512 * pass + 128 * (tile >> 2) + 4 * (lane & 31) + (tile & 3);
    const int h0 = 16 * c + 8 * (lane >> 5);
    const float sw = scales[0];
    u32x4 ph = {0u, 0u, 0u, 0u}, pm = ph;
    if (v < V) {
        const float *w = W + (long)v * H + h0;
        f32x4 w0 = *(const f32x4 *)w, w1 = *(const f32x4 *)(w + 4);
#pragma unroll
        for (int k = 0; k < 4; ++k) { w0[k] = x2_clamp(w0[k] * sw); w1[k] = x2_clamp(w1[k] * sw); }
        X2_SPLIT4(w0, ph, pm, 0);
        X2_SPLIT4(w1, ph, pm, 2);
    }
    u32x4 *o = out + ((long)pass * KC + c) * 2048 + tile * 64 + lane;
    o[0] = ph; o[1024] = pm;
}
size_t x2_wpack_fwd_bytes(int H, int V) { return (size_t)((V + 511) / 512) * (H / 16) * 2 * 16 * 64 * 16; }

#define XF2_WSLOT 32768
#define XF2_ASLOT 8192
#define XF2_NW 3
#ifdef RNNT_STAMPS
#ifndef X2S_WAVE
#define X2S_WAVE 0
#endif
#define X2STAMP(slot)                                                                                       \
    do {                                                                                                    \
        if (a.debug && blockIdx.x == 0 && wave == X2S_WAVE && lane == 0 && it == 1 && cs >= 8 && cs < 24) {  \
            unsigned long long t_;                                                                          \
            asm volatile("s_memtime %0\n\ts_waitcnt lgkmcnt(0)" : "=s"(t_)::"memory");                       \
            a.debug[(cs - 8) * 8 + (slot)] = t_;                                                            \
        }                                                                                                   \
    } while (0)
#else
#define X2STAMP(slot) do {} while (0)
#endif
template <int MODE>
__global__ __launch_bounds__(256, 1) void k_joint_fwd_x2(X3Args a, const int ntiles)
{
    constexpr bool EP = MODE == 1, LIN = MODE == 2;
    if (!LIN && (*a.ep_flag != 0) == EP) return;
    extern __shared__ __attribute__((aligned(1024))) char s_fw[];
    float *s_den = (float *)(s_fw + XF2_NW * XF2_WSLOT + 2 * XF2_ASLOT);
    float *s_part = s_den + 128;
    int *s_next = (int *)(s_part + 512);
    const int tid = threadIdx.x, lane = tid & 63;
    const int wave = __builtin_amdgcn_readfirstlane(tid >> 6);
    const int wm = wave >> 1, wn = wave & 1;
    const int i = lane & 31, half = lane >> 5;
    const int H = a.H, V = a.V, KC = H / 16, U1 = a.U1, T = a.T;
    const int npass = (V + 511) / 512;
    const int NS = LIN ? KC : npass * KC;
    const long cells = (long)a.B * T * U1;
    const float unscale = (LIN ? a.scales[3] : X2_INV_SH) * a.scales[1];
    const float sx = LIN ? a.scales[2] : 1.0f;

    const int lds0 = (int)(size_t)(lds_vptr)s_fw;
    const int xa = lds0 + XF2_NW * XF2_WSLOT + (2 * wm) * 2048 + 16 * lane;
    const int xw = lds0 + XF2_NW * XF2_WSLOT + wave * 2048 + 16 * lane;
    const int wb = lds0 + (8 * wn) * 1024 + 16 * lane;
    const __amdgpu_buffer_rsrc_t wrs = __builtin_amdgcn_make_buffer_rsrc(a.wpack_fwd, 0, npass * KC * XF2_WSLOT, 0x00020000);
    const int wvo = lane * 16;

    X2_CLOCK_STAMP(128 + 100);
    if (tid == 0) s_next[0] = (int)atomicAdd(a.counter, 1u);
    __syncthreads();
    int tile = s_next[0];
    for (int it = 1; tile < ntiles; ++it) {
        if (tid == 0) s_next[it & 1] = (int)atomicAdd(a.counter, 1u);
        const long row0 = (long)(LIN ? tile / npass : tile) * 128;
        const int pass0 = LIN ? tile % npass : 0, cs0 = pass0 * KC;
        __syncthreads();
        const int next = s_next[it & 1];
        bool dead = false;
        if (!LIN) {
            const long per = (long)T * U1, c_last = row0 + 127;
            const long b_first = row0 / per;
            dead = c_last < cells && c_last / per == b_first && (row0 - b_first * per) / U1 >= len_t(a.logit_lens, (int)b_first, T);
        }

        const long prow = row0 + 32 * wave + i;
        const long pc_ = prow < cells ? prow : cells - 1;
        const int pu = (int)(pc_ % U1);
        const long pbt = pc_ / U1;
        const int pt = (int)(pbt % T), pb = (int)(pbt / T);
        const float *ep = EP ? a.ep_enc + ((long)pb * KC * T + pt) * 16 + 8 * half : a.enc + (long)pb * a.enc_sb + (long)pt * a.enc_st + 8 * half;
        const float *pp = LIN ? ep : EP ? a.ep_pred + ((long)pb * KC * U1 + pu) * 16 + 8 * half : a.pred + ((long)pb * U1 + pu) * H + 8 * half;
        const long ek = EP ? (long)T * 16 : 16, pk = EP ? (long)U1 * 16 : 16;
        u32x4 *hdst = (u32x4 *)a.hidden + pc_ * (H / 8) + half;
        const long ps = a.plane_stride / 8;
        struct Opd { f32x4 e0, e1, p0, p1; };
        struct Prod { f2 w[4]; float ra, rb; u32x4 ph, pm; };
        auto op_load1 = [&](Opd &o, int kcs, int k) {
            const float *e = ep + ek * kcs, *q = pp + pk * kcs;
            if (k == 0) o.e0 = *(const f32x4 *)e;
            else if (k == 1) o.e1 = *(const f32x4 *)(e + 4);
            else if (LIN) return;
            else if (k == 2) o.p0 = *(const f32x4 *)q;
            else o.p1 = *(const f32x4 *)(q + 4);
        };
        auto op_load = [&](Opd &o, int kcs) {
#pragma unroll
            for (int k = 0; k < 4; ++k) op_load1(o, kcs, k);
        };
        auto prod_piece = [&](Prod &P, const Opd &o, auto off_c, int k) {
            if (k < 8) {
                const int j = k >> 1;
                const f32x4 &e = j < 2 ? o.e0 : o.e1, &pv = j < 2 ? o.p0 : o.p1;
                const int q = 2 * (j & 1);
                if (LIN) {
                    if (!(k & 1)) P.w[j] = f2{x2_clamp(e[q] * sx), x2_clamp(e[q + 1] * sx)};
                } else if (EP) {
                    if (!(k & 1)) {
                        P.w[j] = f2{__builtin_amdgcn_rcpf(fmaf(e[q], pv[q], 1.0f)), __builtin_amdgcn_rcpf(fmaf(e[q + 1], pv[q + 1], 1.0f))};
                    } else {
                        P.w[j] = f2{fmaf(-2.0f * X2_SH, P.w[j][0], X2_SH), fmaf(-2.0f * X2_SH, P.w[j][1], X2_SH)};
                    }
                } else if (!(k & 1)) {
                    const f2 x = {e[q] + pv[q], e[q + 1] + pv[q + 1]};
                    const f2 av = x * (2.0f * RNNT_LOG2E);
                    P.w[j] = f2{__builtin_amdgcn_exp2f(av[0]), __builtin_amdgcn_exp2f(av[1])};
                } else {
                    const f2 ex = P.w[j] + 1.0f;
                    const f2 rr = {__builtin_amdgcn_rcpf(ex[0]), __builtin_amdgcn_rcpf(ex[1])};
                    P.w[j] = X2_SH - (2.0f * X2_SH) * rr;
                }
            } else if (k < 16) {
                const int j = (k - 8) >> 1;
                if (!(k & 1)) {
                    const unsigned hh = x2_pack(P.w[j][0], P.w[j][1]);
                    P.ph[j] = hh;
                    asm("v_fma_mix_f32 %0, %1, -1.0, %2 op_sel_hi:[1,0,0]" : "=v"(P.ra) : "v"(hh), "v"(P.w[j][0]));
                    asm("v_fma_mix_f32 %0, %1, -1.0, %2 op_sel:[1,0,0] op_sel_hi:[1,0,0]" : "=v"(P.rb) : "v"(hh), "v"(P.w[j][1]));
                } else {
                    P.pm[j] = x2_pack(P.ra, P.rb);
                }
            } else {
                const int dst = xw;
                asm volatile("ds_write_b128 %0, %1 offset:%2" :: "v"(dst), "v"(P.ph), "n"(decltype(off_c)::value) : "memory");
                asm volatile("ds_write_b128 %0, %1 offset:%2" :: "v"(dst), "v"(P.pm), "n"(decltype(off_c)::value + 1024) : "memory");
            }
        };
        auto hid_store = [&](const Prod &P, int kcs) { hdst[2 * kcs] = P.ph; hdst[2 * kcs + ps] = P.pm; };
        auto wdma = [&](int cs, int slot, int n) {
            const int g4 = n & 4;
            if ((n & 3) == 0) __builtin_amdgcn_raw_ptr_buffer_load_lds(wrs, (lds_vptr)(s_fw + slot * XF2_WSLOT + (wave * 8 + g4) * 1024), 16, wvo, (cs * 32 + wave * 8 + g4) * 1024, 0, 0);
            if ((n & 3) == 1) __builtin_amdgcn_raw_ptr_buffer_load_lds(wrs, (lds_vptr)(s_fw + slot * XF2_WSLOT + (wave * 8 + g4) * 1024), 16, wvo, (cs * 32 + wave * 8 + g4) * 1024, 1024, 0);
            if ((n & 3) == 2) __builtin_amdgcn_raw_ptr_buffer_load_lds(wrs, (lds_vptr)(s_fw + slot * XF2_WSLOT + (wave * 8 + g4) * 1024), 16, wvo, (cs * 32 + wave * 8 + g4) * 1024, 2048, 0);
            if ((n & 3) == 3) __builtin_amdgcn_raw_ptr_buffer_load_lds(wrs, (lds_vptr)(s_fw + slot * XF2_WSLOT + (wave * 8 + g4) * 1024), 16, wvo, (cs * 32 + wave * 8 + g4) * 1024, 3072, 0);
        };

        if (dead) {
            for (int kc = 0; kc < KC; ++kc) {
                Opd o; Prod P;
                op_load(o, kc);
#pragma unroll
                for (int pc = 0; pc < 16; ++pc) prod_piece(P, o, X2Int<0>{}, pc);
                hid_store(P, kc);
            }
            tile = next;
            continue;
        }

        f32x16 acc[2][8];
        float m_run = RNNT_NEG_INF, s_run = 0.f;
        auto acc_init = [&]() {
#pragma unroll
            for (int mt = 0; mt < 2; ++mt)
// ... 105 lines not shown
          for (int kc0 = 0; kc0 < KC; kc0 += 2) { kstep(X2Int<0>{}, kc0); kstep(X2Int<1>{}, kc0 + 1); }
          if (STORE) asm volatile(RNNT_VMCNT(2) ::: "memory");
          else asm volatile("s_waitcnt vmcnt(0)" ::: "memory");
          {
            const int cw = 512 * pass + 256 * wn;
            const unsigned lane_off = (unsigned)(((4 * half) * V + 4 * i) * 4);
            char *tile_base = (char *)(a.logits + row0 * V + cw);
            const bool has_b = !LIN || a.bias != nullptr;
            const f32x4 b0 = has_b && cw + 4 * i < V ? *(const f32x4 *)(a.bias + cw + 4 * i) : f32x4{0.f, 0.f, 0.f, 0.f};
            const f32x4 b1 = has_b && cw + 128 + 4 * i < V ? *(const f32x4 *)(a.bias + cw + 128 + 4 * i) : f32x4{0.f, 0.f, 0.f, 0.f};
            auto epilogue = [&](auto both_c) {
                constexpr bool BOTH = decltype(both_c)::value != 0;
                auto read_slot = [&](int mt, int r, f32x4 &o0, f32x4 &o1) {
#pragma unroll
                    for (int q = 0; q < 4; ++q) {
                        float x0, x1;
                        asm volatile("v_accvgpr_read_b32 %0, %1" : "=v"(x0) : "a"(acc[mt][q][r]));
                        asm volatile("v_accvgpr_read_b32 %0, %1" : "=v"(x1) : "a"(acc[mt][4 + q][r]));
                        o0[q] = fmaf(x0, unscale, b0[q]); o1[q] = fmaf(x1, unscale, b1[q]);
                    }
                };
                auto row_of = [&](int mt, int r) { return 32 * (2 * wm + mt) + (r & 3) + 8 * (r >> 2); };
                if constexpr (LIN) {
                    auto slot = [&](int mt, int r) {
                        f32x4 o0, o1;
#pragma unroll
                        for (int q = 0; q < 4; ++q) {
                            float x0, x1;
                            asm volatile("v_accvgpr_read_b32 %0, %1" : "=v"(x0) : "a"(acc[mt][q][r]));
                            asm volatile("v_accvgpr_read_b32 %0, %1" : "=v"(x1) : "a"(acc[mt][4 + q][r]));
                            o0[q] = fmaf(x0, unscale, b0[q]); o1[q] = fmaf(x1, unscale, b1[q]);
                        }
                        char *rowp = tile_base + (long)(32 * (2 * wm + mt) + (r & 3) + 8 * (r >> 2)) * V * 4;
                        if (row0 + 32 * (2 * wm + mt) + (r & 3) + 8 * (r >> 2) + 4 * half < cells) {
                            *(f32x4 *)(rowp + lane_off) = o0;
                            if (BOTH) *(f32x4 *)(rowp + lane_off + 512) = o1;
                        }
                    };
#pragma unroll
                    for (int mt = 0; mt < 2; ++mt)
#pragma unroll
                        for (int r = 0; r < 16; r += 2) {
                            slot(mt, r);
                            slot(mt, r + 1);
                            __builtin_amdgcn_sched_barrier(0);
                        }
                } else {
                    int m_pass = 0, s_pass = 0;
#pragma unroll
                    for (int mt = 0; mt < 2; ++mt)
#pragma unroll
                        for (int r0 = 0; r0 < 16; r0 += 4) {
                            f32x4 o0[4], o1[4];
                            float mx[4], sm[4];
#pragma unroll
                            for (int g = 0; g < 4; ++g) {
                                read_slot(mt, r0 + g, o0[g], o1[g]);
                                char *rowp = tile_base + (long)row_of(mt, r0 + g) * V * 4;
                                __builtin_nontemporal_store(o0[g], (f32x4 *)(rowp + lane_off));
                                if (BOTH) __builtin_nontemporal_store(o1[g], (f32x4 *)(rowp + lane_off + 512));
                                float m8 = fmaxf(fmaxf(o0[g][0], o0[g][1]), fmaxf(o0[g][2], o0[g][3]));
                                if (BOTH) m8 = fmaxf(m8, fmaxf(fmaxf(o1[g][0], o1[g][1]), fmaxf(o1[g][2], o1[g][3])));
                                mx[g] = m8;
                            }
                            half_max_dpp_x4(mx[0], mx[1], mx[2], mx[3]);
#pragma unroll
                            for (int g = 0; g < 4; ++g) {
                                const int lo = __builtin_amdgcn_readlane(__float_as_int(mx[g]), 31), hi = __builtin_amdgcn_readlane(__float_as_int(mx[g]), 63);
                                asm("v_writelane_b32 %0, %1, %2" : "+v"(m_pass) : "s"(lo), "n"(16 * mt + r0 + g));
                                asm("v_writelane_b32 %0, %1, %2" : "+v"(m_pass) : "s"(hi), "n"(32 + 16 * mt + r0 + g));
                                const float M = __int_as_float(half ? hi : lo);
                                const float nm2 = -M * RNNT_LOG2E;
                                float e = (__builtin_amdgcn_exp2f(fmaf(o0[g][0], RNNT_LOG2E, nm2)) + __builtin_amdgcn_exp2f(fmaf(o0[g][1], RNNT_LOG2E, nm2))) +
                                          (__builtin_amdgcn_exp2f(fmaf(o0[g][2], RNNT_LOG2E, nm2)) + __builtin_amdgcn_exp2f(fmaf(o0[g][3], RNNT_LOG2E, nm2)));
                                if (BOTH)
                                    e += (__builtin_amdgcn_exp2f(fmaf(o1[g][0], RNNT_LOG2E, nm2)) + __builtin_amdgcn_exp2f(fmaf(o1[g][1], RNNT_LOG2E, nm2))) +
                                         (__builtin_amdgcn_exp2f(fmaf(o1[g][2], RNNT_LOG2E, nm2)) + __builtin_amdgcn_exp2f(fmaf(o1[g][3], RNNT_LOG2E, nm2)));
                                sm[g] = e;
                            }
                            half_sum_dpp_x4(sm[0], sm[1], sm[2], sm[3]);
#pragma unroll
                            for (int g = 0; g < 4; ++g) {
                                const int lo = __builtin_amdgcn_readlane(__float_as_int(sm[g]), 31), hi = __builtin_amdgcn_readlane(__float_as_int(sm[g]), 63);
                                asm("v_writelane_b32 %0, %1, %2" : "+v"(s_pass) : "s"(lo), "n"(16 * mt + r0 + g));
                                asm("v_writelane_b32 %0, %1, %2" : "+v"(s_pass) : "s"(hi), "n"(32 + 16 * mt + r0 + g));
                            }
                            __builtin_amdgcn_sched_barrier(0);
                        }
                    const float M = __int_as_float(m_pass), S_ = __int_as_float(s_pass);
                    const float m_o = m_run, s_o = s_run;
                    const float mn = fmaxf(m_o, M);
                    m_run = mn;
                    s_run = fmaf(s_o, __builtin_amdgcn_exp2f((m_o - mn) * RNNT_LOG2E), S_ * __builtin_amdgcn_exp2f((M - mn) * RNNT_LOG2E));
                }
            };
            if (cw + 128 < V) epilogue(X2Int<1>{});
            else if (cw < V) epilogue(X2Int<0>{});
          }
        };
        run_pass(X2Int<(LIN ? 0 : 1)>{}, pass0);
        if (!LIN)
            for (int pass = 1; pass < npass; ++pass) run_pass(X2Int<0>{}, pass);

        if (!LIN) {
            float *sp = s_part + (wn * 128 + 32 * (2 * wm + (i >> 4)) + (i & 3) + 8 * ((i & 15) >> 2) + 4 * half) * 2;
            sp[0] = m_run;
            sp[1] = s_run;
        }
        asm volatile("s_waitcnt vmcnt(0)" ::: "memory");
        __syncthreads();
        if (LIN) { tile = next; continue; }
        if (tid < 128) {
            const float m0 = s_part[tid * 2], s0 = s_part[tid * 2 + 1];
            const float m1 = s_part[(128 + tid) * 2], s1 = s_part[(128 + tid) * 2 + 1];
            const float M = fmaxf(m0, m1);
            const float S_ = s0 * __builtin_amdgcn_exp2f((m0 - M) * RNNT_LOG2E) + s1 * __builtin_amdgcn_exp2f((m1 - M) * RNNT_LOG2E);
            s_den[tid] = M + __logf(S_);
        }
        __syncthreads();
        {
            const int row = tid & 127, which = tid >> 7;
            const long cell = row0 + row;
            if (cell < cells) {
                const int u = (int)(cell % U1);
                const long bt = cell / U1;
                const int t = (int)(bt % T), b = (int)(bt / T);
                const int Ub = len_u(a.target_lens, b, U1);
                if (t < len_t(a.logit_lens, b, T) && u <= Ub) {
                    const float den = s_den[row];
                    const float *lrow = a.logits + cell * V;
                    const long si = skew_index(b, t, u, a.D, U1);
                    if (which == 0) {
                        const float lb = __hip_atomic_load(lrow + a.blank, __ATOMIC_RELAXED, __HIP_MEMORY_SCOPE_AGENT);
                        a.denom_s[si] = den;
                        a.lpb_s[si] = lb - den;
                    } else {
                        float le = 0.f;
                        if (u < Ub) {
                            const int y = a.targets[(long)b * (U1 - 1) + u];
                            le = __hip_atomic_load(lrow + y, __ATOMIC_RELAXED, __HIP_MEMORY_SCOPE_AGENT) - den;
                        }
                        a.lpe_s[si] = le;
                    }
                }
            }
        }
        tile = next;
    }
    X2_CLOCK_STAMP(128 + 102);
}

bool x2_fwd_ok(int U1, int H, int V) { return H % 128 == 0 && V % 128 == 0 && (long)128 * H * 2 < 0x7fffffffL; }

void launch_joint_fwd_x2(const X3Args &a, hipStream_t st, bool lin )
{
    static bool attr_set[16] = {false};
    int dev = -1;
    if (hipGetDevice(&dev) != hipSuccess || dev < 0 || dev >= 16) dev = -1;
    const int lds = XF2_NW * XF2_WSLOT + 2 * XF2_ASLOT + 128 * 4 + 2 * 128 * 2 * 4 + 16;
    if (dev < 0 || !attr_set[dev]) {
        (void)hipFuncSetAttribute((const void *)k_joint_fwd_x2<1>, hipFuncAttributeMaxDynamicSharedMemorySize, lds);
        (void)hipFuncSetAttribute((const void *)k_joint_fwd_x2<0>, hipFuncAttributeMaxDynamicSharedMemorySize, lds);
        (void)hipFuncSetAttribute((const void *)k_joint_fwd_x2<2>, hipFuncAttributeMaxDynamicSharedMemorySize, lds);
        if (dev >= 0) attr_set[dev] = true;
    }
    const long cells = (long)a.B * a.T * a.U1;
    const int ntiles = (int)((cells + 127) / 128) * (lin ? (a.V + 511) / 512 : 1);
    if (!lin) launch_fill32(a.counter, 0u, 4, st);
    const int nwg = ntiles < a.n_cu ? ntiles : a.n_cu;
    if (lin) { hipLaunchKernelGGL(k_joint_fwd_x2<2>, dim3((unsigned)nwg), dim3(256), lds, st, a, ntiles); return; }
    hipLaunchKernelGGL(k_joint_fwd_x2<1>, dim3((unsigned)nwg), dim3(256), lds, st, a, ntiles);
    hipLaunchKernelGGL(k_joint_fwd_x2<0>, dim3((unsigned)nwg), dim3(256), lds, st, a, ntiles);
}

void launch_x2_pack_w(const X3Args &a, float *scales, hipStream_t st)
{
    hipLaunchKernelGGL(k_x2_wscale, dim3(1), dim3(1024), 0, st, a.W, (long)a.V * a.H / 4, scales);
    const long nd = (long)((a.H + 511) / 512) * (a.V / 16) * 16 * 64;
    hipLaunchKernelGGL(k_x2_pack_w_dh, dim3((unsigned)((nd + 255) / 256)), dim3(256), 0, st, a.W, (const float *)scales, (u32x4 *)a.wpack_dh, a.H, a.V, nd);
    const long nf = (long)((a.V + 511) / 512) * (a.H / 16) * 16 * 64;
    hipLaunchKernelGGL(k_x2_pack_w_fwd, dim3((unsigned)((nf + 255) / 256)), dim3(256), 0, st, a.W, (const float *)scales, (u32x4 *)a.wpack_fwd, a.H, a.V, nf);
}


struct X2AbsArgs { const float *x[3]; long ld[3], rows[3]; int cols4[3]; };
__global__ __launch_bounds__(256) void k_x2_absmax(X2AbsArgs a, float *__restrict__ partial)
{
    __shared__ float s_m[4];
    const int t = blockIdx.y;
    const float *x = a.x[t];
    const long ld = a.ld[t], n = a.rows[t] * a.cols4[t];
    const int cols4 = a.cols4[t];
    float m = 0.f;
    bool bad = false;
    for (long idx = (long)blockIdx.x * 256 + threadIdx.x; idx < n; idx += (long)gridDim.x * 256) {
        const long r = idx / cols4;
        const int c = (int)(idx - r * cols4);
        const f32x4 w = *(const f32x4 *)(x + r * ld + 4 * c);
        const float mw = fmaxf(fmaxf(fabsf(w[0]), fabsf(w[1])), fmaxf(fabsf(w[2]), fabsf(w[3])));
        bad = bad || !(fabsf(w[0]) <= X2_F32_MAX) || !(fabsf(w[1]) <= X2_F32_MAX) || !(fabsf(w[2]) <= X2_F32_MAX) || !(fabsf(w[3]) <= X2_F32_MAX);
        m = fmaxf(m, mw);
    }
#pragma unroll
    for (int o = 32; o > 0; o >>= 1) m = fmaxf(m, __shfl_xor(m, o, 64));
    const int any_bad = __syncthreads_or(bad ? 1 : 0);
    if ((threadIdx.x & 63) == 0) s_m[threadIdx.x >> 6] = m;
    __syncthreads();
    if (threadIdx.x == 0) partial[t * 256 + blockIdx.x] = any_bad ? __uint_as_float(0x7fc00000u) : fmaxf(fmaxf(s_m[0], s_m[1]), fmaxf(s_m[2], s_m[3]));
}
__global__ __launch_bounds__(256) void k_x2_lin_scales(const float *__restrict__ partial, float *__restrict__ scales, int n, unsigned *__restrict__ zero0,
                                                       int nzero0, unsigned *__restrict__ zero1, int nzero1, long nks,
                                                       int *__restrict__ list, int *__restrict__ stats, int *__restrict__ glist)
{
    __shared__ float s_m[4];
    for (int i = 0; i < n; ++i) {
        float m = partial[i * 256 + threadIdx.x];
        const int nonfinite = __syncthreads_or(m != m ? 1 : 0);
#pragma unroll
        for (int o = 32; o > 0; o >>= 1) m = fmaxf(m, __shfl_xor(m, o, 64));
        __syncthreads();
        if ((threadIdx.x & 63) == 0) s_m[threadIdx.x >> 6] = m;
        __syncthreads();
        if (threadIdx.x == 0 && nonfinite) {
            scales[2 * i] = 1.0f;
            scales[2 * i + 1] = __uint_as_float(0x7fc00000u);
        } else if (threadIdx.x == 0) {
            const unsigned bits = __float_as_uint(fmaxf(fmaxf(s_m[0], s_m[1]), fmaxf(s_m[2], s_m[3])));
            float s = 1.0f;
            const int e = (int)(bits >> 23) & 0xff;
            if (e > 0 && e < 255) {
                int k = 14 - (e - 126);
                k = k > 100 ? 100 : (k < -100 ? -100 : k);
                s = __uint_as_float((unsigned)(127 + k) << 23);
            }
            scales[2 * i] = s;
            scales[2 * i + 1] = 1.0f / s;
        }
    }
    for (int j = threadIdx.x; j < nzero0; j += 256) zero0[j] = 0u;
    for (int j = threadIdx.x; j < nzero1; j += 256) zero1[j] = 0u;
    if (list) {
        const long ngrp = 4 * nks;
        for (long j = threadIdx.x; j < nks + 8; j += 256) list[j] = (int)(j < nks ? j : nks);
        for (long j = threadIdx.x; j < ngrp + XL2_GPAD; j += 256) glist[j] = (int)(j < ngrp ? j : ngrp);
        if (threadIdx.x == 0) { stats[0] = (int)nks; stats[1] = (int)nks; stats[2] = 0; stats[3] = 0; stats[4] = (int)ngrp; stats[5] = (int)ngrp; }
    }
}
template <bool INTER>
__global__ __launch_bounds__(256) void k_x2_split_rows(const float *__restrict__ x, long ld, long rows, long rows_out, int cols,
                                                       const float *__restrict__ scale, void *__restrict__ dst, long plane_stride)
{
    const float s = scale[0];
    const long idx = (long)blockIdx.x * 256 + threadIdx.x;
    if (INTER) {
        const int VC = cols / 32;
        if (idx >= rows_out * VC) return;
        const long r = idx / VC;
        const int c = (int)(idx - r * VC);
        const f32x4 *p = (const f32x4 *)(x + (r < rows ? r : 0) * ld + 32 * c);
        u32x4 ph[4], pm[4];
#pragma unroll
        for (int i = 0; i < 8; ++i) {
            f32x4 v = r < rows ? p[i] : f32x4{0.f, 0.f, 0.f, 0.f};
#pragma unroll
            for (int k = 0; k < 4; ++k) v[k] = x2_clamp(v[k] * s);
            X2_SPLIT4(v, ph[i >> 1], pm[i >> 1], 2 * (i & 1));
        }
        u32x4 *o = (u32x4 *)((float *)dst + r * cols + 32 * c);
#pragma unroll
        for (int i = 0; i < 4; ++i) { o[i] = ph[i]; o[4 + i] = pm[i]; }
    } else {
        const int H8 = cols / 8;
        if (idx >= rows_out * H8) return;
        const long r = idx / H8;
        const int h = (int)(idx - r * H8) * 8;
        const float *xr = x + (r < rows ? r : 0) * ld + h;
        f32x4 t0 = *(const f32x4 *)xr, t1 = *(const f32x4 *)(xr + 4);
        if (r >= rows) t0 = t1 = f32x4{0.f, 0.f, 0.f, 0.f};
#pragma unroll
        for (int k = 0; k < 4; ++k) { t0[k] = x2_clamp(t0[k] * s); t1[k] = x2_clamp(t1[k] * s); }
        u32x4 ph, pm;
        X2_SPLIT4(t0, ph, pm, 0);
        X2_SPLIT4(t1, ph, pm, 2);
        u32x4 *o = (u32x4 *)((unsigned short *)dst + r * cols + h);
        o[0] = ph; o[plane_stride / 8] = pm;
    }
}
__global__ __launch_bounds__(256) void k_x2_reduce_scaled(const float *__restrict__ slab, float *__restrict__ out, long n4, long stride4, int nsplit,
                                                          const float *__restrict__ sa, const float *__restrict__ sb)
{
    const long i = (long)blockIdx.x * 256 + threadIdx.x;
    if (i >= n4) return;
    f32x4 acc = ((const f32x4 *)slab)[i];
    for (int s = 1; s < nsplit; ++s) acc += ((const f32x4 *)slab)[i + s * stride4];
    const float r = sa[0] * (sb ? sb[0] : 1.0f);
    ((f32x4 *)out)[i] = acc * r;
}

int device_cus()
{
    static thread_local int cus[16] = {0};
    int dev = 0;
    if (hipGetDevice(&dev) != hipSuccess || dev < 0 || dev >= 16) dev = 0;
    if (!cus[dev]) {
        hipDeviceProp_t p;
        if (hipGetDeviceProperties(&p, dev) == hipSuccess) cus[dev] = p.multiProcessorCount;
        if (cus[dev] <= 0) cus[dev] = 256;
    }
    return cus[dev];
}

namespace {
struct LinWs { size_t wt, pack, pa, pb, slab_w, slab_b, prog, list, glist, total; long rows_pad, rows_alloc; int n_split; };
LinWs lin_layout(int M, int K, int N, bool bwd)
{
    auto al = [](size_t x) { return (x + 255) & ~(size_t)255; };
    LinWs L{};
    size_t o = 4096;
    if (!bwd) { L.pack = o; o += al(x2_wpack_fwd_bytes(K, N)); L.total = o; return L; }
    L.rows_pad = ((long)M + 1 + 31) / 32 * 32;
    L.rows_alloc = (L.rows_pad + 96 + 127) / 128 * 128;
    const long tiles = x2_dw_tiles(K, N);
    long ns = 256 / tiles;
    if (ns < 1) ns = 1;
    if (ns > L.rows_pad / 32) ns = L.rows_pad / 32;
    L.n_split = (int)ns;
    L.wt = o; o += al((size_t)N * K * 4);
    L.pack = o; o += al(x2_wpack_fwd_bytes(N, K));
    L.pa = o; o += al((size_t)L.rows_alloc * N * 4);
    L.pb = o; o += al((size_t)L.rows_alloc * K * 4);
    L.slab_w = o; o += al((size_t)L.n_split * N * K * 4);
    L.slab_b = o; o += al((size_t)L.n_split * N * 4);
    L.prog = o; o += al((size_t)L.n_split * 64);
    L.list = o; o += al(64 + (size_t)(L.rows_pad / XW2_ROWS + 8) * 4);
// ... 75 lines not shown
```

Before: 168.4 million cells/s.

## Merge f16x2 prologue, pack, reduce and status launches into fewer fused kernels

Collapses the many small setup launches of the f16x2 pipeline into two kernels: a prologue that computes per-block weight absmax partials while zeroing padding, counters and flags, and a combined weight-pack plus ep kernel that reduces the scale inline. The enc/pred dhidden reductions and the dW/bias slab reductions each become a single launch. Redundant fills of the lattice error and forward counter are skipped when the prologue already zeroed them, and the lattice status check is folded into the live kernel. The aim is lower launch and serialization overhead. In exchange, every block of the pack kernel recomputes the scale reduction, and the correctness of the zeroing now depends on stage flags.

Measured after the change: 168.4 million cells/s, median of 6. No clear change (+0.0%).

```diff
diff --git a/rnnt_amd/csrc/engine.hip b/rnnt_amd/csrc/engine.hip
--- a/rnnt_amd/csrc/engine.hip
+++ b/rnnt_amd/csrc/engine.hip
@@ -231,6 +231,7 @@
     const int32_t *targets, *logit_lens, *target_lens; float *costs;
     int B, T, U1, stages ; float grad_scale, fastemit, delay; hipStream_t st;
     const int32_t *restrict_frames; int restrict_left, restrict_right;
+    bool err_zeroed, fold_status;
 };
 
 struct FusedCall : LossCall {
@@ -321,7 +322,8 @@
         if (c.stages & ST_LATTICE) {
             launch_restrict(w.lpe_s, c.restrict_frames, c.logit_lens, c.target_lens, c.B, c.T, c.U1, D, c.restrict_left, c.restrict_right,
                             c.delay, c.st);
-            launch_lattice(w.lpb_s, w.lpe_s, w.alpha_s, w.beta_s, c.logit_lens, c.target_lens, c.costs, c.B, c.U1, D, w.err, c.st, true);
+            launch_lattice(w.lpb_s, w.lpe_s, w.alpha_s, w.beta_s, c.logit_lens, c.target_lens, c.costs, c.B, c.U1, D, w.err, c.st, true,
+                           c.err_zeroed, c.fold_status);
             if (c.delay > 0.f) launch_delay_cost(w.beta_s, c.logit_lens, c.target_lens, c.costs, c.B, c.T, c.U1, D, c.delay, c.st);
         }
         if (c.stages & ST_COEF)
@@ -331,7 +333,8 @@
     }
     if (c.stages & ST_LATTICE) {
         if (c.delay > 0.f) launch_delay_penalty(w.lpe_s, c.logit_lens, c.target_lens, c.B, c.T, c.U1, D, c.delay, c.st);
-        launch_lattice(w.lpb_s, w.lpe_s, w.alpha_s, w.beta_s, c.logit_lens, c.target_lens, c.costs, c.B, c.U1, D, w.err, c.st);
+        launch_lattice(w.lpb_s, w.lpe_s, w.alpha_s, w.beta_s, c.logit_lens, c.target_lens, c.costs, c.B, c.U1, D, w.err, c.st, false,
+                       c.err_zeroed, c.fold_status);
         if (c.delay > 0.f) launch_delay_cost(w.beta_s, c.logit_lens, c.target_lens, c.costs, c.B, c.T, c.U1, D, c.delay, c.st);
     }
     if (c.stages & ST_COEF) {
@@ -436,8 +439,12 @@
     return launch_status("rnnt_engine fused pipeline (bf16x3)");
 }
 
-int route_f16x2(const FusedCall &c)
-{
+int route_f16x2(const FusedCall &c0)
+{
+    FusedCall c = c0;
+    const bool prod = (c.stages & ST_PROD) != 0;
+    c.err_zeroed = prod;
+    c.fold_status = prod && (c.stages & ST_LATTICE) && (c.stages & ST_COEF) && !(c.delay > 0.f);
     OperandScales s = operand_scales(c.grad_scale, c.fastemit);
     X3Args h = x3_args(c, x2_wpack_fwd_bytes(c.H, c.V), s);
     h.dw_prog = c.cb->dw_prog(c.B); h.dw_ksteps = x2_dw_walks_ksteps(c.H, c.V) ? 1 : 0;
@@ -447,18 +454,17 @@
     else { g.gen_bu = 16; g.pred_split_col = c.H; }
     if (!c.x3_fp32_dh) { g.tile_flag = h.tile_live; g.flag_ntt = (c.T + 7) / 8; g.flag_nub = h.n_ublk16; }
     if (c.x2_no_flush || c.x3_fp32_dh) { s.flush_log2 = -HUGE_VAL; s.flush_lin = 0.f; }
-    if (c.stages & ST_PROD) { launch_x2_zero_padding(h, 1, c.st); launch_x2_pack_w(h, c.cb->x2_scales, c.st); launch_x2_make_ep(h, c.st); }
+    if (prod) launch_x2_producers(h, c.cb->x2_scales, (float *)c.cb->queue, c.cb->lattice_err, c.st);
     if (c.x3_fp32_fwd) standin_forward(c, h, launch_x2_make_hidden);
-    else if (c.stages & ST_FWD) launch_joint_fwd_x2(h, c.st);
+    else if (c.stages & ST_FWD) launch_joint_fwd_x2(h, c.st, false, prod);
     loss_stages(c, &s.flush_log2, s.flush_lin);
-    if (c.stages & ST_COEF) launch_x2_live(h, c.st);
+    if (c.stages & ST_COEF) launch_x2_live(h, prod, c.fold_status ? c.cb->lattice_err : nullptr, c.costs, c.st);
     if (c.stages & ST_DH) {
-        launch_x2_zero_padding(h, 2, c.st);
-        if (c.x3_fp32_dh) standin_dhidden(c, g, h, launch_x2_split_g);
+        if (c.x3_fp32_dh) { launch_x2_zero_g_padding(h, c.st); standin_dhidden(c, g, h, launch_x2_split_g); }
         else { launch_x2_dead_rows(h, c.st); launch_dhidden_x2(h, c.st); }
     }
     if (c.stages & ST_DH_RED) launch_dhidden_reduce(g, c.st);
-    if (c.stages & ST_DW) launch_dw_x2(h, c.st);
+    if (c.stages & ST_DW) launch_dw_x2(h, c.st, !prod);
     if (c.stages & ST_DW_RED) launch_dw_reduce_x2(h, c.grad_W, c.grad_bias, c.st);
     return launch_status("rnnt_engine fused pipeline (f16x2)");
 }
diff --git a/rnnt_amd/csrc/joint_bwd.hip b/rnnt_amd/csrc/joint_bwd.hip
--- a/rnnt_amd/csrc/joint_bwd.hip
+++ b/rnnt_amd/csrc/joint_bwd.hip
@@ -553,14 +553,13 @@
         for (int j = 0; j < 8; ++j) s += v[j];
     }
 }
-__global__ __launch_bounds__(256) void k_reduce_enc(const float *__restrict__ slab,
-                                                    const int32_t *__restrict__ logit_lens,
-                                                    const int32_t *__restrict__ target_lens,
-                                                    float *__restrict__ out, int B, int T, int U1,
-                                                    int H, int n_ublk, int bu_lo, int col_split,
-                                                    const unsigned char *__restrict__ flag, int ntt, int nub_f)
-{
-    const long idx = (long)blockIdx.x * blockDim.x + threadIdx.x;
+__device__ __forceinline__ void reduce_enc(const float *__restrict__ slab,
+                                           const int32_t *__restrict__ logit_lens,
+                                           const int32_t *__restrict__ target_lens,
+                                           float *__restrict__ out, int B, int T, int U1,
+                                           int H, int n_ublk, int bu_lo,
+                                           const unsigned char *__restrict__ flag, int ntt, int nub_f, long idx)
+{
     const int H4 = H / 4;
     const long n = (long)B * T * H4;
     if (idx >= n) return;
@@ -586,14 +585,13 @@
     ((f32x4 *)out)[idx] = s;
 }
 
-__global__ __launch_bounds__(256) void k_reduce_pred(const float *__restrict__ slab,
-                                                     const int32_t *__restrict__ logit_lens,
-                                                     const int32_t *__restrict__ target_lens,
-                                                     float *__restrict__ out, int B, int T, int U1,
-                                                     int H, int bt_lo, int bt_hi, int col_split,
-                                                     const unsigned char *__restrict__ flag, int ntt_f, int nub_f)
-{
-    const long idx = (long)blockIdx.x * blockDim.x + threadIdx.x;
+__device__ __forceinline__ void reduce_pred(const float *__restrict__ slab,
+                                            const int32_t *__restrict__ logit_lens,
+                                            const int32_t *__restrict__ target_lens,
+                                            float *__restrict__ out, int B, int T, int U1,
+                                            int H, int bt_lo, int bt_hi, int col_split,
+                                            const unsigned char *__restrict__ flag, int ntt_f, int nub_f, long idx)
+{
     const int H4 = H / 4;
     const long n = (long)B * U1 * H4;
     if (idx >= n) return;
@@ -618,6 +616,16 @@
     ((f32x4 *)out)[idx] = s;
 }
 
+__global__ __launch_bounds__(256) void k_reduce_hidden(JointBwdArgs a, unsigned nb_enc)
+{
+    if (blockIdx.x < nb_enc)
+        reduce_enc(a.slab_enc, a.logit_lens, a.target_lens, a.grad_enc, a.B, a.T, a.U1, a.H, a.n_ublk, a.gen_bu, a.tile_flag, a.flag_ntt,
+                   a.flag_nub, (long)blockIdx.x * 256 + threadIdx.x);
+    else
+        reduce_pred(a.slab_pred, a.logit_lens, a.target_lens, a.grad_pred, a.B, a.T, a.U1, a.H, 128 / a.gen_bu, 64 / a.gen_bu, a.pred_split_col,
+                    a.tile_flag, a.flag_ntt, a.flag_nub, (long)(blockIdx.x - nb_enc) * 256 + threadIdx.x);
+}
+
 void launch_dhidden(const JointBwdArgs &a, bool tile_kernel, hipStream_t st)
 {
     int cb0 = 0;
@@ -646,14 +654,9 @@
 
 void launch_dhidden_reduce(const JointBwdArgs &a, hipStream_t st)
 {
-    const long n4e = (long)a.B * a.T * (a.H / 4);
-    hipLaunchKernelGGL(k_reduce_enc, dim3((unsigned)((n4e + 255) / 256)), dim3(256), 0, st,
-                       a.slab_enc, a.logit_lens, a.target_lens, a.grad_enc, a.B, a.T, a.U1, a.H, a.n_ublk, a.gen_bu, a.pred_split_col,
-                       a.tile_flag, a.flag_ntt, a.flag_nub);
-    const long n4p = (long)a.B * a.U1 * (a.H / 4);
-    hipLaunchKernelGGL(k_reduce_pred, dim3((unsigned)((n4p + 255) / 256)), dim3(256), 0, st,
-                       a.slab_pred, a.logit_lens, a.target_lens, a.grad_pred, a.B, a.T, a.U1, a.H,
-                       128 / a.gen_bu, 64 / a.gen_bu, a.pred_split_col, a.tile_flag, a.flag_ntt, a.flag_nub);
+    const long n4e = (long)a.B * a.T * (a.H / 4), n4p = (long)a.B * a.U1 * (a.H / 4);
+    const unsigned nbe = (unsigned)((n4e + 255) / 256), nbp = (unsigned)((n4p + 255) / 256);
+    hipLaunchKernelGGL(k_reduce_hidden, dim3(nbe + nbp), dim3(256), 0, st, a, nbe);
 }
 
 __global__ __launch_bounds__(256) void k_make_hidden(const float *__restrict__ enc, long sb,
diff --git a/rnnt_amd/csrc/kernels.hpp b/rnnt_amd/csrc/kernels.hpp
--- a/rnnt_amd/csrc/kernels.hpp
+++ b/rnnt_amd/csrc/kernels.hpp
@@ -14,7 +14,9 @@
 void launch_lattice(const float *lpb_s, const float *lpe_s, double *alpha_s, double *beta_s,
                     const int32_t *logit_lens, const int32_t *target_lens, float *costs, int B,
                     int U1, int D, unsigned *err , hipStream_t st,
-                    bool restricted = false );
+                    bool restricted = false ,
+                    bool err_zeroed = false ,
+                    bool fold_status = false );
 void launch_coef(const double *alpha_s, const double *beta_s, const float *denom_s,
                  const float *lpb_s, const float *lpe_s, const int32_t *targets,
                  const int32_t *logit_lens, const int32_t *target_lens, CellCoef *coef, int B,
@@ -184,7 +186,7 @@
 };
 size_t x2_live_bytes(int B, int T, int U1, long rows_pad);
 void x2_live_carve(void *region, int B, int T, int U1, long rows_pad, X3Args &a);
-void launch_x2_live(const X3Args &a, hipStream_t st);
+void launch_x2_live(const X3Args &a, bool tiles_zeroed, const unsigned *status_err, float *costs, hipStream_t st);
 bool x3_fwd_ok(int U1, int H, int V);
 bool x3_dhidden_ok(int U1, int H, int V);
 size_t x3_wpack_fwd_bytes(int H, int V);
@@ -202,11 +204,10 @@
 size_t x2_wpack_dh_bytes(int H, int V);
 void launch_x2_make_hidden(const X3Args &a, hipStream_t st);
 void launch_x2_split_g(const X3Args &a, hipStream_t st);
-void launch_x2_zero_padding(const X3Args &a, int what, hipStream_t st);
-void launch_x2_pack_w(const X3Args &a, float *scales, hipStream_t st);
-void launch_x2_make_ep(const X3Args &a, hipStream_t st);
+void launch_x2_zero_g_padding(const X3Args &a, hipStream_t st);
+void launch_x2_producers(const X3Args &a, float *scales, float *wmax, unsigned *lattice_err, hipStream_t st);
 size_t x2_ep_bytes(int B, int T, int U1, int H);
-void launch_joint_fwd_x2(const X3Args &a, hipStream_t st, bool plain_gemm = false);
+void launch_joint_fwd_x2(const X3Args &a, hipStream_t st, bool plain_gemm = false, bool counter_zeroed = false);
 void launch_x2_dead_rows(const X3Args &a, hipStream_t st);
 void launch_dhidden_x2(const X3Args &a, hipStream_t st);
 size_t x2_linear_ws_bytes(int M, int K, int N, bool bwd);
diff --git a/rnnt_amd/csrc/lattice.hip b/rnnt_amd/csrc/lattice.hip
--- a/rnnt_amd/csrc/lattice.hip
+++ b/rnnt_amd/csrc/lattice.hip
@@ -517,19 +517,19 @@
 
 void launch_lattice(const float *lpb_s, const float *lpe_s, double *alpha_s, double *beta_s,
                     const int32_t *logit_lens, const int32_t *target_lens, float *costs, int B,
-                    int U1, int D, unsigned *err, hipStream_t st, bool restricted)
+                    int U1, int D, unsigned *err, hipStream_t st, bool restricted, bool err_zeroed, bool fold_status)
 {
     const int NW = (U1 + 63) / 64;
     const size_t mbox = (size_t)(NW - 1) * D * 12;
     if (mbox <= 64 * 1024) {
-        if (NW > 1) launch_fill32(err, 0u, 4, st);
+        if (NW > 1 && !err_zeroed) launch_fill32(err, 0u, 4, st);
         if (restricted)
             hipLaunchKernelGGL(k_lattice_chain_restrict, dim3(B, 2), dim3(64 * NW), (mbox + 15) / 16 * 16, st, lpb_s, lpe_s,
                                alpha_s, beta_s, logit_lens, target_lens, costs, U1, D, err);
         else
             hipLaunchKernelGGL(k_lattice_chain, dim3(B, 2), dim3(64 * NW), (mbox + 15) / 16 * 16, st, lpb_s, lpe_s, alpha_s,
                                beta_s, logit_lens, target_lens, costs, U1, D, err);
-        if (NW > 1) hipLaunchKernelGGL(k_lattice_status, dim3(1), dim3(64), 0, st, err, costs, B);
+        if (NW > 1 && !fold_status) hipLaunchKernelGGL(k_lattice_status, dim3(1), dim3(64), 0, st, err, costs, B);
         return;
     }
     const int NT = ((U1 + 63) / 64) * 64;
diff --git a/rnnt_amd/csrc/x2.hip b/rnnt_amd/csrc/x2.hip
--- a/rnnt_amd/csrc/x2.hip
+++ b/rnnt_amd/csrc/x2.hip
@@ -66,16 +66,31 @@
 #define XG2_BU 16
 
 #define X2_F32_MAX 3.4028234663852886e38f
-__global__ __launch_bounds__(1024) void k_x2_wscale(const float *__restrict__ W, long n4, float *__restrict__ scales)
-{
-    __shared__ float s_m[16];
+#define XP2_NMAX 64
+__device__ __forceinline__ void x2_wscale(float m, bool any_bad, float *s_out, float *inv_out)
+{
+    float s = 1.0f;
+    const unsigned bits = __float_as_uint(m);
+    const int e = (int)(bits >> 23) & 0xff;
+    if (e > 0 && e < 255) {
+        int k = 14 - (e - 126);
+        k = k > 100 ? 100 : (k < -100 ? -100 : k);
+        s = __uint_as_float((unsigned)(127 + k) << 23);
+    }
+    *s_out = s;
+    *inv_out = (any_bad || e == 255) ? __uint_as_float(0x7fc00000u) : 1.0f / s;
+}
+__device__ __forceinline__ void x2_wmax_partial(const float *__restrict__ W, long n4, float *__restrict__ part)
+{
+    __shared__ float s_m[4];
+    constexpr long S = 256L * XP2_NMAX;
     float m = 0.f;
     bool bad = false;
-    long i = threadIdx.x;
-    for (; i + 7 * 1024 < n4; i += 8 * 1024) {
+    long i = (long)blockIdx.x * 256 + threadIdx.x;
+    for (; i + 7 * S < n4; i += 8 * S) {
         f32x4 w[8];
 #pragma unroll
-        for (int k = 0; k < 8; ++k) w[k] = ((const f32x4 *)W)[i + 1024 * k];
+        for (int k = 0; k < 8; ++k) w[k] = ((const f32x4 *)W)[i + S * k];
 #pragma unroll
         for (int k = 0; k < 8; ++k) {
             const float mw = fmaxf(fmaxf(fabsf(w[k][0]), fabsf(w[k][1])), fmaxf(fabsf(w[k][2]), fabsf(w[k][3])));
@@ -83,7 +98,7 @@
             m = fmaxf(m, mw);
         }
     }
-    for (; i < n4; i += 1024) {
+    for (; i < n4; i += S) {
         const f32x4 w = ((const f32x4 *)W)[i];
         bad |= (w[0] != w[0]) | (w[1] != w[1]) | (w[2] != w[2]) | (w[3] != w[3]);
         m = fmaxf(fmaxf(m, fmaxf(fabsf(w[0]), fabsf(w[1]))), fmaxf(fabsf(w[2]), fabsf(w[3])));
@@ -94,17 +109,42 @@
     if ((threadIdx.x & 63) == 0) s_m[threadIdx.x >> 6] = m;
     __syncthreads();
     if (threadIdx.x == 0) {
-        for (int k = 1; k < 16; ++k) m = fmaxf(m, s_m[k]);
-        float s = 1.0f;
-        const unsigned bits = __float_as_uint(m);
-        const int e = (int)(bits >> 23) & 0xff;
-        if (e > 0 && e < 255) {
-            int k = 14 - (e - 126);
-            k = k > 100 ? 100 : (k < -100 ? -100 : k);
-            s = __uint_as_float((unsigned)(127 + k) << 23);
-        }
-        scales[0] = s;
-        scales[1] = (any_bad || e == 255) ? __uint_as_float(0x7fc00000u) : 1.0f / s;
+        for (int k = 1; k < 4; ++k) m = fmaxf(m, s_m[k]);
+        part[blockIdx.x] = m;
+        part[XP2_NMAX + blockIdx.x] = any_bad ? 1.0f : 0.0f;
+    }
+}
+__device__ __forceinline__ float x2_wscale_reduce(const float *__restrict__ part, float *__restrict__ scales)
+{
+    __shared__ float s_sw;
+    if (threadIdx.x < 64) {
+        float m = part[threadIdx.x];
+        static_assert(XP2_NMAX == 64, "one partial per lane of the first wave");
+        const bool any_bad = __ballot(part[XP2_NMAX + threadIdx.x] != 0.0f) != 0ull;
+#pragma unroll
+        for (int o = 32; o > 0; o >>= 1) m = fmaxf(m, __shfl_xor(m, o, 64));
+        if (threadIdx.x == 0) {
+            float s, inv;
+            x2_wscale(m, any_bad, &s, &inv);
+            s_sw = s;
+            if (scales) { scales[0] = s; scales[1] = inv; }
+        }
+    }
+    __syncthreads();
+    return s_sw;
+}
+struct X2ZeroList { u32x4 *p[8]; unsigned n[8]; };
+__global__ __launch_bounds__(256) void k_x2_prologue(const float *__restrict__ W, long n4, float *__restrict__ part, X2ZeroList z, unsigned n_zero)
+{
+    if (blockIdx.x < XP2_NMAX) { x2_wmax_partial(W, n4, part); return; }
+    const unsigned stride = (gridDim.x - XP2_NMAX) * 256u;
+    for (unsigned i = (blockIdx.x - XP2_NMAX) * 256u + threadIdx.x; i < n_zero; i += stride) {
+        u32x4 *dst = nullptr;
+        unsigned j = i;
+#pragma unroll
+        for (int r = 0; r < 8; ++r)
+            if (!dst) { if (j < z.n[r]) dst = z.p[r] + j; else j -= z.n[r]; }
+        if (dst) *dst = u32x4{0u, 0u, 0u, 0u};
     }
 }
 
@@ -167,13 +207,10 @@
     const long n = rows * (a.V / 32);
     hipLaunchKernelGGL(k_x2_split_g, dim3((unsigned)((n + 255) / 256)), dim3(256), 0, st, a, rows);
 }
-void launch_x2_zero_padding(const X3Args &a, int what, hipStream_t st)
+void launch_x2_zero_g_padding(const X3Args &a, hipStream_t st)
 {
     const long cells = (long)a.B * a.T * a.U1;
-    const size_t pad = (size_t)(a.rows_alloc - cells);
-    if (what & 1)
-        for (int p = 0; p < 2; ++p) launch_fill32(a.hidden + p * a.plane_stride + cells * a.H, 0u, pad * a.H * 2, st);
-    if (what & 2) launch_fill32(a.logits + cells * a.V, 0u, pad * a.V * 4, st);
+    launch_fill32(a.logits + cells * a.V, 0u, (size_t)(a.rows_alloc - cells) * a.V * 4, st);
 }
 
 #define XL2_BLK 1024
@@ -212,15 +249,27 @@
 }
 __global__ __launch_bounds__(XL2_BLK) void k_x2_live_count(const CellCoef *__restrict__ coef, long cells,
                                                            unsigned long long *__restrict__ bitmap, int *__restrict__ blk,
-                                                           unsigned long long *__restrict__ gbitmap, int *__restrict__ gblk)
+                                                           unsigned long long *__restrict__ gbitmap, int *__restrict__ gblk,
+                                                           int T, int U1, int ntt, int nub, unsigned char *__restrict__ tile_live,
+                                                           const unsigned *__restrict__ err, float *__restrict__ costs, int B)
 {
     __shared__ unsigned short s_nib[16][16];
     __shared__ unsigned short s_grp[16][16];
     const int lane = threadIdx.x & 63, wave = threadIdx.x >> 6;
     const long base = (long)blockIdx.x * XL2_BLK * XW2_ROWS;
+    if (err && blockIdx.x == 0 && *err != 0u)
+        for (int b = threadIdx.x; b < B; b += XL2_BLK) costs[b] = __builtin_nanf("");
     for (int it = 0; it < 16; ++it) {
         const long c = base + (long)it * XL2_BLK + threadIdx.x;
         const bool live = c < cells && x2_coef_live(coef[c]);
+        int tile = -1;
+        if (live) {
+            const int u = (int)(c % U1);
+            const long bt = c / U1;
+            tile = (int)(((bt / T) * ntt + (int)(bt % T) / XG2_BT) * nub + u / XG2_BU);
+        }
+        const int left = __shfl_up(tile, 1, 64);
+        if (live && (lane == 0 || left != tile)) tile_live[tile] = 1;
         const unsigned long long bal = __ballot(live);
         if (lane == 0)
             s_nib[it][wave] = (unsigned short)(((bal & 0xffffull) ? 1 : 0) | ((bal & 0xffff0000ull) ? 2 : 0) |
@@ -339,25 +388,8 @@
     for (int w = 0; w < wave; ++w) off += s_w[w];
     if ((bal >> lane) & 1ull) list[off + __popcll(bal & ((1ull << lane) - 1ull))] = (int)k;
 }
-__global__ __launch_bounds__(256) void k_x2_live_tiles(const CellCoef *__restrict__ coef, int T, int U1, int ntt, int nub, long ntile,
-                                                       unsigned char *__restrict__ tile_live)
-{
-    const int lane = threadIdx.x & 63;
-    const long tile = (long)blockIdx.x * 4 + (threadIdx.x >> 6);
-    if (tile >= ntile) return;
-    const int ub = (int)(tile % nub), tt = (int)((tile / nub) % ntt);
-    const long b = tile / ((long)nub * ntt);
-    bool live = false;
-#pragma unroll
-    for (int it = 0; it < 2; ++it) {
-        const int r = it * 64 + lane;
-        const int t = tt * XG2_BT + (r >> 4), u = ub * XG2_BU + (r & 15);
-        if (t < T && u < U1) live = live || x2_coef_live(coef[(b * T + t) * U1 + u]);
-    }
-    const bool any = __any(live ? 1 : 0) != 0;
-    if (lane == 0) tile_live[tile] = any ? 1 : 0;
-}
-void launch_x2_live(const X3Args &a, hipStream_t st)
+size_t x2_tile_flag_bytes(int B, int T, int U1) { return (x2_live_layout(B, T, U1, 0).ntile + 255) & ~(size_t)255; }
+void launch_x2_live(const X3Args &a, bool tiles_zeroed, const unsigned *status_err, float *costs, hipStream_t st)
 {
     const X2LiveWs L = x2_live_layout(a.B, a.T, a.U1, a.rows_pad);
     const long cells = (long)a.B * a.T * a.U1;
@@ -365,15 +397,19 @@
     int *gblk = (int *)((char *)a.live_stats + L.gblk);
     unsigned long long *bitmap = (unsigned long long *)a.ks_bitmap, *gbitmap = (unsigned long long *)a.grp_bitmap;
     const int ntt = (a.T + XG2_BT - 1) / XG2_BT, nub = (a.U1 + XG2_BU - 1) / XG2_BU;
-    hipLaunchKernelGGL(k_x2_live_tiles, dim3((unsigned)((L.ntile + 3) / 4)), dim3(256), 0, st, a.coef, a.T, a.U1, ntt, nub, L.ntile, (unsigned char *)a.tile_live);
-    hipLaunchKernelGGL(k_x2_live_count, dim3(L.nblk), dim3(XL2_BLK), 0, st, a.coef, cells, bitmap, blk, gbitmap, gblk);
+    if (!tiles_zeroed) launch_fill32((void *)a.tile_live, 0u, x2_tile_flag_bytes(a.B, a.T, a.U1), st);
+    hipLaunchKernelGGL(k_x2_live_count, dim3(L.nblk), dim3(XL2_BLK), 0, st, a.coef, cells, bitmap, blk, gbitmap, gblk, a.T, a.U1, ntt, nub,
+                       (unsigned char *)a.tile_live, status_err, costs, a.B);
     hipLaunchKernelGGL(k_x2_live_scan, dim3(1), dim3(1024), 0, st, blk, L.nblk, a.live_stats, a.ks_list, cells, L.nks, L.ntile, a.tile_live, (int *)a.tile_list, gblk, a.grp_list);
     hipLaunchKernelGGL(k_x2_live_write, dim3(5 * L.nblk), dim3(XL2_BLK), 0, st, bitmap, L.nblk, blk, a.ks_list, gbitmap, gblk, a.grp_list);
 }
 
-__global__ __launch_bounds__(256) void k_x2_reduce_slabs(const float *__restrict__ slab, float *__restrict__ out, long n4, int ns)
-{
-    const long idx = (long)blockIdx.x * blockDim.x + threadIdx.x;
+__global__ __launch_bounds__(256) void k_x2_reduce_slabs(const float *__restrict__ slab, float *__restrict__ out, long n4, int ns, unsigned nbw,
+                                                         const float *__restrict__ slab_b, float *__restrict__ out_b, long n4b)
+{
+    unsigned bid = blockIdx.x;
+    if (bid >= nbw) { bid -= nbw; slab = slab_b; out = out_b; n4 = n4b; }
+    const long idx = (long)bid * 256 + threadIdx.x;
     if (idx >= n4) return;
     double s0 = 0.0, s1 = 0.0, s2 = 0.0, s3 = 0.0;
     for (int k = 0; k < ns; ++k) {
@@ -385,8 +421,8 @@
 void launch_dw_reduce_x2(const X3Args &a, float *grad_W, float *grad_bias, hipStream_t st)
 {
     const long n4w = (long)a.V * a.H / 4, n4b = a.V / 4;
-    hipLaunchKernelGGL(k_x2_reduce_slabs, dim3((unsigned)((n4w + 255) / 256)), dim3(256), 0, st, a.slab_w, grad_W, n4w, a.n_split);
-    hipLaunchKernelGGL(k_x2_reduce_slabs, dim3((unsigned)((n4b + 255) / 256)), dim3(256), 0, st, a.slab_b, grad_bias, n4b, a.n_split);
+    const unsigned nbw = (unsigned)((n4w + 255) / 256), nbb = (unsigned)((n4b + 255) / 256);
+    hipLaunchKernelGGL(k_x2_reduce_slabs, dim3(nbw + nbb), dim3(256), 0, st, a.slab_w, grad_W, n4w, a.n_split, nbw, a.slab_b, grad_bias, n4b);
 }
 
 #define XW2_NST 4
@@ -863,16 +899,14 @@
 #define XG2_WAIT8(b) asm volatile("s_waitcnt lgkmcnt(0)" : "+v"(b[0]), "+v"(b[1]), "+v"(b[2]), "+v"(b[3]), "+v"(b[4]), "+v"(b[5]), "+v"(b[6]), "+v"(b[7]) :: "memory")
 #define XG2_WAIT8_BUT(b, N) asm volatile("s_waitcnt lgkmcnt(" #N ")" : "+v"(b[0]), "+v"(b[1]), "+v"(b[2]), "+v"(b[3]), "+v"(b[4]), "+v"(b[5]), "+v"(b[6]), "+v"(b[7]) :: "memory")
 
-__global__ __launch_bounds__(256) void k_x2_pack_w_dh(const float *__restrict__ W, const float *__restrict__ scales, u32x4 *__restrict__ out, int H, int V, long n)
-{
-    const long idx = (long)blockIdx.x * 256 + threadIdx.x;
+__device__ __forceinline__ void x2_pack_w_dh(const float *__restrict__ W, float sw, u32x4 *__restrict__ out, int H, int V, long n, long idx)
+{
     if (idx >= n) return;
     const int lane = (int)(idx & 63), tile = (int)(idx >> 6) & 15;
     const int VC = V / 16;
     const int c = (int)((idx >> 10) % VC), hp = (int)((idx >> 10) / VC);
     const int h = 512 * hp + 128 * (tile >> 2) + 4 * (lane & 31) + (tile & 3);
     const int v0 = 16 * c + 8 * (lane >> 5);
-    const float sw = scales[0];
     u32x4 ph = {0u, 0u, 0u, 0u}, pm = ph;
     if (h < H) {
         const float *w = W + (long)v0 * H + h;
@@ -1393,6 +1427,9 @@
             for (int q = lane; q < V4; q += 64) row[q] = z;
         }
     }
+    u32x4 *pad = (u32x4 *)(a.logits + cells * a.V);
+    const long npad = (a.rows_alloc - cells) * V4;
+    for (long q = (long)blockIdx.x * (64 * XZ2_WG_WAVES) + threadIdx.x; q < npad; q += (long)gridDim.x * (64 * XZ2_WG_WAVES)) pad[q] = z;
 }
 void launch_x2_dead_rows(const X3Args &a, hipStream_t st)
 {
@@ -1433,11 +1470,10 @@
     }
 }
 
-__global__ __launch_bounds__(256) void k_x2_make_ep(X3Args a)
+__device__ __forceinline__ void x2_make_ep(const X3Args &a, long idx)
 {
     const int H = a.H, H4 = H / 4, KC = H / 16;
     const long n_enc = (long)a.B * a.T * H4, n_all = n_enc + (long)a.B * a.U1 * H4;
-    const long idx = (long)blockIdx.x * 256 + threadIdx.x;
     bool big = false;
     if (idx < n_all) {
         const bool is_enc = idx < n_enc;
@@ -1461,24 +1497,16 @@
     }
     if (__builtin_amdgcn_ballot_w64(big) != 0 && (threadIdx.x & 63) == 0) atomicOr(a.ep_flag, 1u);
 }
-void launch_x2_make_ep(const X3Args &a, hipStream_t st)
-{
-    launch_fill32(a.ep_flag, 0u, 4, st);
-    const long n = ((long)a.B * a.T + (long)a.B * a.U1) * (a.H / 4);
-    hipLaunchKernelGGL(k_x2_make_ep, dim3((unsigned)((n + 255) / 256)), dim3(256), 0, st, a);
-}
 size_t x2_ep_bytes(int B, int T, int U1, int H) { return ((size_t)B * T + (size_t)B * U1) * H * 4; }
 
-__global__ __launch_bounds__(256) void k_x2_pack_w_fwd(const float *__restrict__ W, const float *__restrict__ scales, u32x4 *__restrict__ out, int H, int V, long n)
-{
-    const long idx = (long)blockIdx.x * 256 + threadIdx.x;
+__device__ __forceinline__ void x2_pack_w_fwd(const float *__restrict__ W, float sw, u32x4 *__restrict__ out, int H, int V, long n, long idx)
+{
     if (idx >= n) return;
     const int lane = (int)(idx & 63), tile = (int)(idx >> 6) & 15;
     const int KC = H / 16;
     const int c = (int)((idx >> 10) % KC), pass = (int)((idx >> 10) / KC);
     const int v = 512 * pass + 128 * (tile >> 2) + 4 * (lane & 31) + (tile & 3);
     const int h0 = 16 * c + 8 * (lane >> 5);
-    const float sw = scales[0];
     u32x4 ph = {0u, 0u, 0u, 0u}, pm = ph;
     if (v < V) {
         const float *w = W + (long)v * H + h0;
@@ -1490,6 +1518,19 @@
     }
     u32x4 *o = out + ((long)pass * KC + c) * 2048 + tile * 64 + lane;
     o[0] = ph; o[1024] = pm;
+}
+__global__ __launch_bounds__(256) void k_x2_pack_w_fwd(const float *__restrict__ W, const float *__restrict__ scales, u32x4 *__restrict__ out, int H, int V, long n)
+{
+    x2_pack_w_fwd(W, scales[0], out, H, V, n, (long)blockIdx.x * 256 + threadIdx.x);
+}
+__global__ __launch_bounds__(256) void k_x2_pack_ep(X3Args a, const float *__restrict__ part, float *__restrict__ scales, unsigned nbd, unsigned nbf,
+                                                    long nd, long nf)
+{
+    const unsigned bid = blockIdx.x;
+    if (bid >= nbd + nbf) { x2_make_ep(a, (long)(bid - nbd - nbf) * 256 + threadIdx.x); return; }
+    const float sw = x2_wscale_reduce(part, bid == 0 ? scales : nullptr);
+    if (bid < nbd) x2_pack_w_dh(a.W, sw, (u32x4 *)a.wpack_dh, a.H, a.V, nd, (long)bid * 256 + threadIdx.x);
+    else x2_pack_w_fwd(a.W, sw, (u32x4 *)a.wpack_fwd, a.H, a.V, nf, (long)(bid - nbd) * 256 + threadIdx.x);
 }
 size_t x2_wpack_fwd_bytes(int H, int V) { return (size_t)((V + 511) / 512) * (H / 16) * 2 * 16 * 64 * 16; }
 
@@ -1901,7 +1942,8 @@
 
 bool x2_fwd_ok(int U1, int H, int V) { return H % 128 == 0 && V % 128 == 0 && (long)128 * H * 2 < 0x7fffffffL; }
 
-void launch_joint_fwd_x2(const X3Args &a, hipStream_t st, bool lin )
+void launch_joint_fwd_x2(const X3Args &a, hipStream_t st, bool lin ,
+                         bool counter_zeroed )
 {
     static bool attr_set[16] = {false};
     int dev = -1;
@@ -1915,20 +1957,30 @@
     }
     const long cells = (long)a.B * a.T * a.U1;
     const int ntiles = (int)((cells + 127) / 128) * (lin ? (a.V + 511) / 512 : 1);
-    if (!lin) launch_fill32(a.counter, 0u, 4, st);
+    if (!lin && !counter_zeroed) launch_fill32(a.counter, 0u, 4, st);
     const int nwg = ntiles < a.n_cu ? ntiles : a.n_cu;
     if (lin) { hipLaunchKernelGGL(k_joint_fwd_x2<2>, dim3((unsigned)nwg), dim3(256), lds, st, a, ntiles); return; }
     hipLaunchKernelGGL(k_joint_fwd_x2<1>, dim3((unsigned)nwg), dim3(256), lds, st, a, ntiles);
     hipLaunchKernelGGL(k_joint_fwd_x2<0>, dim3((unsigned)nwg), dim3(256), lds, st, a, ntiles);
 }
 
-void launch_x2_pack_w(const X3Args &a, float *scales, hipStream_t st)
-{
-    hipLaunchKernelGGL(k_x2_wscale, dim3(1), dim3(1024), 0, st, a.W, (long)a.V * a.H / 4, scales);
-    const long nd = (long)((a.H + 511) / 512) * (a.V / 16) * 16 * 64;
-    hipLaunchKernelGGL(k_x2_pack_w_dh, dim3((unsigned)((nd + 255) / 256)), dim3(256), 0, st, a.W, (const float *)scales, (u32x4 *)a.wpack_dh, a.H, a.V, nd);
-    const long nf = (long)((a.V + 511) / 512) * (a.H / 16) * 16 * 64;
-    hipLaunchKernelGGL(k_x2_pack_w_fwd, dim3((unsigned)((nf + 255) / 256)), dim3(256), 0, st, a.W, (const float *)scales, (u32x4 *)a.wpack_fwd, a.H, a.V, nf);
+void launch_x2_producers(const X3Args &a, float *scales, float *wmax, unsigned *lattice_err, hipStream_t st)
+{
+    const long cells = (long)a.B * a.T * a.U1;
+    X2ZeroList z{};
+    unsigned n_zero = 0;
+    int r = 0;
+    auto add = [&](void *p, size_t bytes) { z.p[r] = (u32x4 *)p; z.n[r] = (unsigned)(bytes / 16); n_zero += z.n[r]; ++r; };
+    for (int p = 0; p < 2; ++p) add(a.hidden + p * a.plane_stride + cells * a.H, (size_t)(a.rows_alloc - cells) * a.H * 2);
+    add(a.counter, 16); add(a.ep_flag, 16); add(lattice_err, 16);
+    if (a.dw_prog) add(a.dw_prog, (size_t)a.n_split * 64);
+    add((void *)a.tile_live, x2_tile_flag_bytes(a.B, a.T, a.U1));
+    const unsigned nbz = (n_zero + 255) / 256;
+    hipLaunchKernelGGL(k_x2_prologue, dim3(XP2_NMAX + (nbz < 1024u ? nbz : 1024u)), dim3(256), 0, st, a.W, (long)a.V * a.H / 4, wmax, z, n_zero);
+    const long nd = (long)((a.H + 511) / 512) * (a.V / 16) * 16 * 64, nf = (long)((a.V + 511) / 512) * (a.H / 16) * 16 * 64;
+    const long ne = ((long)a.B * a.T + (long)a.B * a.U1) * (a.H / 4);
+    const unsigned nbd = (unsigned)((nd + 255) / 256), nbf = (unsigned)((nf + 255) / 256);
+    hipLaunchKernelGGL(k_x2_pack_ep, dim3(nbd + nbf + (unsigned)((ne + 255) / 256)), dim3(256), 0, st, a, (const float *)wmax, scales, nbd, nbf, nd, nf);
 }
 
 
```
